# hpcaitech/CachedEmbedding

Hardware: AMD Instinct MI355X
Metric: embedding lookups/sec (cache op + EmbeddingBag fwd + bwd/SGD), Criteo-1TB table @1% cache (higher is better)
Workload: dtype f32

## Files before the change

### cachedembedding_amd/_lib.py

```python
from __future__ import annotations

import ctypes
import os
from ctypes import POINTER, Structure, c_char_p, c_double, c_float, c_int, c_int32, c_int64, c_size_t, c_uint64, c_void_p
from pathlib import Path

import torch

_PKG = Path(__file__).resolve().parent
LIB_PATH = Path(os.environ["CE_LIBRARY"]) if os.environ.get("CE_LIBRARY") else _PKG / "libce_hip.so"

CE_OK = 0
CE_ERR_INVALID = 1
CE_ERR_HIP = 2
CE_ERR_CAPACITY = 3
CE_ERR_NOMEM = 4
CE_ERR_UNSUPPORTED = 5
CE_ERR_RANGE = 6
CE_EVICT_DATASET = 0
CE_EVICT_LFU = 1
CE_MODE_SUM = 0
CE_MODE_MEAN = 1
CE_ACT_F32 = 0
CE_ACT_BF16 = 1
CE_ACT_F16 = 2
CE_TRANSPORT_ZEROCOPY = 0
CE_TRANSPORT_STAGED = 1
CE_TRANSPORT_WORKER = 2
CE_CALL_PREPARE = 0
CE_CALL_PRELOAD = 1
CE_CALL_FLUSH = 2


class CeCacheConfig(Structure):
    _fields_ = [
        ("num_embeddings", c_int64),
        ("cuda_row_num", c_int64),
        ("embedding_dim", c_int32),
        ("evict_strategy", c_int32),
        ("transport", c_int32),
        ("protect_depth", c_int32),
        ("max_ids_per_call", c_int64),
        ("host_weight", c_void_p),
        ("host_weight_dev", c_void_p),
        ("cache_weight", c_void_p),
        ("idx_map", c_void_p),
        ("inverted_cached_idx", c_void_p),
        ("cached_idx_map", c_void_p),
        ("freq_cnter", c_void_p),
        ("workspace", c_void_p),
        ("workspace_bytes", c_size_t),
    ]


class CeCallStats(Structure):
    _fields_ = [
        ("seq", c_int64),
        ("n_ids", c_int64),
        ("n_unique", c_int64),
        ("n_miss", c_int64),
        ("n_evict", c_int64),
        ("miss_lookups", c_int64),
        ("n_free_after", c_int64),
        ("status", c_int32),
        ("kind", c_int32),
    ]


_BAG_COMMON = [c_void_p, c_int32, c_int64, c_int32, c_void_p, c_int32, c_int64]
SIGNATURES = {
    "ce_version": (c_int, []),
    "ce_cpu_budget": (c_int32, []),
    "ce_last_error": (c_char_p, []),
    "ce_stream_create_cu_mask": (c_int, [c_void_p, c_int32, POINTER(c_void_p)]),
    "ce_stream_destroy": (c_int, [c_void_p]),
    "ce_host_alloc": (c_int, [c_size_t, c_int, POINTER(c_void_p), POINTER(c_void_p)]),
    "ce_host_free": (c_int, [c_void_p]),
    "ce_host_register": (c_int, [c_void_p, c_size_t, POINTER(c_void_p)]),
    "ce_host_unregister": (c_int, [c_void_p]),
    "ce_host_fill_uniform": (c_int, [c_void_p, c_int64, c_float, c_float, c_uint64, c_int]),
    "ce_host_fill_uniform_rows": (c_int, [c_void_p, c_int64, c_int32, c_float, c_float, c_uint64, c_void_p, c_void_p]),
    "ce_host_rows_gather": (c_int, [c_void_p, c_int64, c_int32, c_void_p, c_int64, c_void_p, c_void_p]),
    "ce_box_probe": (c_int, [c_void_p, c_size_t, c_int32, POINTER(c_double), POINTER(c_double), c_void_p]),
    "ce_probe_rows": (c_int, [c_void_p, c_int64, c_int32, c_int64, c_int32, POINTER(c_double), POINTER(c_double), c_void_p]),
    "ce_bag_forward": (c_int, [c_void_p, c_int64, c_int32, c_void_p, c_int64, c_void_p, c_int32, c_int64,
                               c_int32, c_void_p, c_int32, c_int64, c_void_p, c_void_p]),
    "ce_bag_backward_dense": (c_int, [c_void_p, c_int64, c_int32, c_void_p, c_int64, c_void_p, c_int32, c_int64,
                                      c_int32, c_void_p, c_int32, c_int64, c_void_p, c_void_p]),
    "ce_bag_backward_dense_presorted": (c_int, [c_void_p, c_int64, c_int32, c_void_p, c_int64, c_void_p, c_int32, c_int64,
                                      c_int32, c_void_p, c_int32, c_int64, c_void_p, c_void_p, c_void_p]),
    "ce_bag_backward_rows": (c_int, [c_void_p, c_void_p, c_int32, c_int64, c_void_p, c_int32, c_int64, c_int32, c_void_p,
                                     c_int32, c_int64, c_void_p, c_void_p]),
    "ce_bag_backward_sgd": (c_int, [c_void_p, c_int64, c_int32, c_void_p, c_int64, c_void_p, c_int32, c_int64,
                                    c_int32, c_void_p, c_int32, c_int64, c_void_p, c_float, c_void_p]),
    "ce_bag_presort_len": (c_int64, [c_int64]),
    "ce_bag_presort": (c_int, [c_void_p, c_int64, c_int64, c_void_p, c_void_p]),
    "ce_bag_backward_sgd_presorted": (c_int, [c_void_p, c_int64, c_int32, c_void_p, c_int64, c_void_p, c_int32,
                                              c_int64, c_int32, c_void_p, c_int32, c_int64, c_void_p, c_float,
                                              c_void_p, c_void_p]),
    "ce_bag_presort_window": (c_int, [c_void_p, c_int64, c_int64, c_int64, c_void_p, c_void_p]),
    "ce_bag_presort_window_src": (c_int, [c_void_p, c_int64, c_int64, c_int64, c_void_p, c_int32, c_int64, c_int64,
                                          c_int32, c_int64, c_void_p, c_void_p]),
    "ce_bag_forward_src_keys": (c_int, [c_void_p, c_int64, c_int32, c_int64, c_void_p, c_void_p, c_void_p]),
    "ce_bag_backward_sgd_presorted_src": (c_int, [c_void_p, c_int64, c_int32, c_int64, c_void_p, c_float, c_void_p,
                                                  c_void_p]),
    "ce_bag_presort_window_src_excl": (c_int, [c_void_p, c_int64, c_int64, c_int64, c_void_p, c_int32, c_int64,
                                               c_int64, c_int32, c_int64, c_void_p, c_void_p, c_void_p, c_void_p]),
    "ce_bag_backward_sgd_presorted_src_excl": (c_int, [c_void_p, c_int64, c_int32, c_int64, c_void_p, c_float,
                                                       c_void_p, c_void_p, c_void_p]),
    "ce_bag_backward_dense_presorted_src": (c_int, [c_void_p, c_int64, c_int32, c_int64, c_void_p, c_void_p,
                                                    c_void_p]),
    "ce_bag_backward_sgd_sorted_workspace": (c_size_t, [c_int64, c_int64]),
    "ce_bag_backward_sgd_sorted": (c_int, [c_void_p, c_int64, c_int32, c_void_p, c_int64, c_void_p, c_int32,
                                           c_int64, c_int32, c_void_p, c_int32, c_int64, c_void_p, c_float,
                                           c_void_p, c_size_t, c_void_p]),
    "ce_bag_backward_rowwise_adagrad_workspace": (c_size_t, [c_int64, c_int32]),
    "ce_bag_backward_rowwise_adagrad": (c_int, [c_void_p, c_int64, c_int32, c_void_p, c_int64, c_void_p, c_int32,
                                                c_int64, c_int32, c_void_p, c_int32, c_int64, c_void_p, c_void_p,
                                                c_void_p, c_void_p, c_int64, c_float, c_float, c_void_p, c_size_t,
                                                c_void_p]),
    "ce_bag_backward_rowwise_adagrad_src": (c_int, [c_void_p, c_int64, c_int32, c_int64, c_void_p, c_void_p, c_void_p,
                                                    c_void_p, c_int64, c_float, c_float, c_void_p, c_size_t,
                                                    c_void_p]),
    "ce_bag_forward_act": (c_int, [c_void_p, c_int64, c_int32, c_void_p, c_int64, c_void_p, c_int32, c_int64,
                                   c_int32, c_void_p, c_int32, c_int64, c_void_p, c_int32, c_void_p]),
    "ce_bag_forward_src_keys_act": (c_int, [c_void_p, c_int64, c_int32, c_int64, c_void_p, c_void_p, c_int32,
                                            c_void_p]),
    "ce_bag_backward_dense_act": (c_int, [c_void_p, c_int64, c_int32, c_void_p, c_int64, c_void_p, c_int32, c_int64,
                                          c_int32, c_void_p, c_int32, c_int64, c_void_p, c_int32, c_void_p,
                                          c_void_p]),
    "ce_bag_backward_sgd_act": (c_int, [c_void_p, c_int64, c_int32, c_void_p, c_int64, c_void_p, c_int32, c_int64,
                                        c_int32, c_void_p, c_int32, c_int64, c_void_p, c_int32, c_float, c_void_p,
                                        c_void_p]),
    "ce_bag_backward_sgd_src_act": (c_int, [c_void_p, c_int64, c_int32, c_int64, c_void_p, c_int32, c_float, c_void_p,
                                            c_void_p, c_void_p]),
    "ce_bag_backward_dense_src_act": (c_int, [c_void_p, c_int64, c_int32, c_int64, c_void_p, c_int32, c_void_p,
                                              c_void_p]),
    "ce_bag_backward_rowwise_adagrad_act": (c_int, [c_void_p, c_int64, c_int32, c_void_p, c_int64, c_void_p, c_int32,
                                                    c_int64, c_int32, c_void_p, c_int32, c_int64, c_void_p, c_int32,
                                                    c_void_p, c_void_p, c_void_p, c_int64, c_float, c_float,
                                                    c_void_p, c_size_t, c_void_p]),
    "ce_bag_backward_rowwise_adagrad_src_act": (c_int, [c_void_p, c_int64, c_int32, c_int64, c_void_p, c_int32,
                                                        c_void_p, c_void_p, c_void_p, c_int64, c_float, c_float,
                                                        c_void_p, c_size_t, c_void_p]),
    "ce_cache_workspace_bytes": (c_size_t, [c_int64, c_int64, c_int64, c_int32]),
    "ce_cache_create": (c_int, [POINTER(CeCacheConfig), c_void_p, POINTER(c_void_p)]),
    "ce_cache_destroy": (c_int, [c_void_p]),
    "ce_cache_preload": (c_int, [c_void_p, c_void_p, c_void_p, c_int64, c_void_p]),
    "ce_cache_set_freq_bound": (c_int, [c_void_p, c_int64]),
    "ce_cache_prepare_ids": (c_int, [c_void_p, c_void_p, c_int64, c_void_p, c_void_p]),
    "ce_cache_prepare_ids_keys": (c_int, [c_void_p, c_void_p, c_int64, c_int64, c_void_p, c_int32, c_void_p, c_int32,
                                          c_int64, c_int64, c_int32, c_int64, c_void_p, c_void_p]),
    "ce_cache_prepare_ids_begin": (c_int, [c_void_p, c_void_p, c_int64, c_int64, c_void_p, c_int32, c_void_p, c_int32,
                                           c_int64, c_int64, c_int32, c_int64, c_void_p, c_void_p]),
    "ce_cache_prepare_ids_finish": (c_int, [c_void_p, c_void_p]),
    "ce_cache_prepare_ids_padded": (c_int, [c_void_p, c_void_p, c_int64, c_void_p, c_void_p]),
    "ce_cache_prepare_ids_begin_padded": (c_int, [c_void_p, c_void_p, c_int64, c_void_p, c_void_p]),
    "ce_cache_set_deferred_rows": (c_int, [c_void_p, c_int32]),
    "ce_cache_rows_ticket": (c_int64, [c_void_p]),
    "ce_cache_wait_rows": (c_int, [c_void_p, c_int64, c_void_p]),
    "ce_cache_last_stats": (c_int, [c_void_p, POINTER(CeCallStats)]),
    "ce_cache_totals": (c_int, [c_void_p, POINTER(c_int64), POINTER(c_int64), POINTER(c_int64),
                                POINTER(c_int64), POINTER(c_int64)]),
    "ce_cache_history": (c_int64, [c_void_p, c_int64, POINTER(CeCallStats), c_int64]),
    "ce_cache_lookup_slots": (c_int, [c_void_p, c_void_p, c_int64, c_void_p, c_void_p]),
    "ce_cache_flush": (c_int, [c_void_p, c_void_p]),
    "ce_cache_set_protect_depth": (c_int, [c_void_p, c_int32]),
    "ce_cache_set_transport": (c_int, [c_void_p, c_int32]),
    "ce_cache_get_transport": (c_int32, [c_void_p]),
    "ce_cache_set_cache_weight": (c_int, [c_void_p, c_void_p]),
    "ce_cache_graph_replayed": (c_int, [c_void_p, c_int64, c_int64, c_void_p]),
    "ce_cache_set_buffer_rows": (c_int, [c_void_p, c_int64]),
    "ce_cache_set_profiling": (c_int, [c_void_p, c_int32]),
    "ce_cache_phase_count": (c_int32, []),
    "ce_cache_phase_name": (c_char_p, [c_int32]),
    "ce_cache_phase_times": (c_int, [c_void_p, POINTER(c_double), c_int32, POINTER(c_int64), c_int32]),
    "ce_cache_writeback_wait": (c_int, [c_void_p]),
    "ce_cache_swap_stats": (c_int, [c_void_p, POINTER(c_double), POINTER(c_int64)]),
    "ce_cache_failures": (c_int, [c_void_p, POINTER(c_int64), POINTER(c_int32), POINTER(c_int64)]),
    "ce_cache_free_rows": (c_int, [c_void_p, POINTER(c_int64)]),
    "ce_bucketize_workspace": (c_size_t, [c_int64, c_int32]),
    "ce_bucketize_rows": (c_int, [c_void_p, c_int64, c_void_p, c_int32, c_void_p, c_void_p, c_void_p, c_void_p,
                                  c_size_t, c_void_p]),
    "ce_dedupe_bucket_rows": (c_int, [c_void_p, c_int64, c_void_p, c_int64, c_int32, c_void_p, c_void_p,
                                      c_void_p, c_void_p, c_void_p, c_void_p, c_void_p]),
    "ce_dedupe_bucket_rows_padded": (c_int, [c_void_p, c_int64, c_void_p, c_int64, c_int32, c_int64, c_void_p, c_void_p,
                                             c_void_p, c_void_p, c_void_p, c_void_p, c_void_p, c_void_p]),
    "ce_dedupe_bucket_rows_padded_window": (c_int, [c_void_p, c_int64, c_int64, c_void_p, c_int64, c_int32, c_int64,
                                                    c_void_p, c_void_p, c_void_p, c_void_p, c_void_p, c_void_p,
                                                    c_void_p, c_void_p]),
    "ce_exchange_local_index": (c_int, [c_void_p, c_int64, c_int64, c_void_p, c_int64, c_int64, c_int64, c_int64,
                                        c_void_p, c_void_p]),
    "ce_split_classify": (c_int, [c_void_p, c_int32, c_int32, c_int64, c_int64, c_void_p, c_int64, c_void_p, c_void_p,
                                  c_void_p]),
    "ce_split_places": (c_int, [c_void_p, c_void_p, c_int32, c_int32, c_int64, c_int32, c_void_p, c_void_p, c_void_p,
                                c_void_p, c_void_p, c_void_p]),
    "ce_exchange_local_index_split": (c_int, [c_void_p, c_int64, c_int64, c_void_p, c_void_p, c_void_p, c_int64, c_int64,
                                              c_int64, c_int64, c_int64, c_void_p, c_int32, c_int64, c_int64, c_int64,
                                              c_void_p, c_void_p, c_void_p]),
    "ce_bag_forward_max": (c_int, [c_void_p, c_int64, c_int32, c_void_p, c_int64, c_void_p, c_int32, c_int64, c_int32,
                                   c_int64, c_void_p, c_void_p, c_void_p]),
    "ce_bag_backward_max": (c_int, [c_void_p, c_int64, c_int32, c_void_p, c_int64, c_int64, c_int64, c_void_p, c_void_p,
                                    c_float, c_void_p]),
    "ce_bag_backward_psw": (c_int, [c_void_p, c_int64, c_int32, c_void_p, c_int64, c_void_p, c_int32, c_int64, c_int32,
                                    c_int64, c_void_p, c_void_p, c_void_p]),
    "ce_rows_renorm_workspace": (c_size_t, [c_int64]),
    "ce_rows_renorm": (c_int, [c_void_p, c_int64, c_int32, c_void_p, c_int64, c_float, c_float, c_void_p, c_size_t,
                               c_void_p]),
    "ce_rows_axpy": (c_int, [c_void_p, c_int64, c_int32, c_void_p, c_int64, c_void_p, c_float, c_void_p]),
}


class CeError(RuntimeError):
    def __init__(self, code: int, msg: str):
        super().__init__(f"libce_hip error {code}: {msg}")
        self.code = code


def _load() -> ctypes.CDLL:
    if not LIB_PATH.exists():
        raise ImportError(
            f"{LIB_PATH} is missing: the HIP extension has not been built. Run "
            "`python -c 'import __graft_entry__ as g; g.build()'` (needs hipcc). There is no CPU fallback.")
    lib = ctypes.CDLL(str(LIB_PATH), mode=os.RTLD_NOW | os.RTLD_LOCAL)
    for name, (res, args) in SIGNATURES.items():
        fn = getattr(lib, name)
        fn.restype = res
        fn.argtypes = args
    return lib


lib = _load()


def last_error() -> str:
    m = lib.ce_last_error()
    return m.decode("utf-8", "replace") if m else ""


def check(rc: int) -> None:
    if rc != CE_OK:
        raise CeError(rc, last_error())


def require_gpu() -> None:
    if not torch.cuda.is_available():
        raise RuntimeError("cachedembedding_amd needs a HIP device (MI355X); no GPU is visible and there is "
                           "no CPU fallback for the product path")


_RAW_STREAM = getattr(torch._C, "_cuda_getCurrentRawStream", None)


def stream_ptr() -> int:
    if _RAW_STREAM is not None:
        return _RAW_STREAM(torch.cuda.current_device())
    return torch.cuda.current_stream().cuda_stream


ACT_DTYPES = {torch.float32: CE_ACT_F32, torch.bfloat16: CE_ACT_BF16, torch.float16: CE_ACT_F16}


def act_code(dtype) -> int:
    if dtype is None:
        return CE_ACT_F32
    try:
        return ACT_DTYPES[dtype]
    except (KeyError, TypeError):
        raise NotImplementedError(f"output_dtype={dtype!r}: torch.float32, torch.bfloat16 and torch.float16 are "
                                  "implemented") from None


def ptr(t) -> int:
    return 0 if t is None else t.data_ptr()
```

### cachedembedding_amd/cache_mgr.py

```python
from __future__ import annotations

import ctypes
import math
import weakref
from enum import Enum
from typing import List, Optional

import numpy as np
import torch

from . import _lib
from ._lib import CeCacheConfig, CeCallStats, check, lib, ptr, stream_ptr


class EvictionStrategy(Enum):
    LFU = 1
    DATASET = 2


class _PinnedBlock:

    def __init__(self, host_ptr: int):
        self._fin = weakref.finalize(self, _PinnedBlock._free, host_ptr)

# ... 284 lines not shown
                self.wait_rows()
            self._strict_check()
        return out

    def graph_replayed(self, n_calls: int, ids_per_call: int) -> None:
        with torch.cuda.device(self.device):
            check(lib.ce_cache_graph_replayed(self._handle, int(n_calls), int(ids_per_call), stream_ptr()))

    def _id_to_cached_cuda_id(self, ids: torch.Tensor) -> torch.Tensor:
        flat = ids.reshape(-1).long().contiguous()
        slots = torch.empty_like(flat)
        check(lib.ce_cache_lookup_slots(self._handle, ptr(flat), flat.numel(), ptr(slots), stream_ptr()))
        return slots.view(ids.shape)

    @torch.no_grad()
    def flush(self):
        with torch.cuda.device(self.device):
            check(lib.ce_cache_flush(self._handle, stream_ptr()))
            st = CeCallStats()
            check(lib.ce_cache_last_stats(self._handle, ctypes.byref(st)))
        self._pull_history()
        assert self.cuda_available_row_num == self.cuda_row_num

    def sync_stats(self) -> CeCallStats:
        st = CeCallStats()
        rc = lib.ce_cache_last_stats(self._handle, ctypes.byref(st))
        self._pull_history()
        if rc not in (_lib.CE_OK, _lib.CE_ERR_CAPACITY, _lib.CE_ERR_RANGE):
            check(rc)
        return st

    def _pull_history(self):
        cap = 4096
        buf = (CeCallStats * cap)()
        while True:
            n = lib.ce_cache_history(self._handle, self._hist_seen + 1, buf, cap)
            for i in range(n):
                r = buf[i]
                self._hist_seen = max(self._hist_seen, r.seq)
                if r.kind != _lib.CE_CALL_PREPARE:
                    continue
                self.num_hits_history.append(int(r.n_unique - r.n_miss))
                self.num_miss_history.append(int(r.n_miss))
                self.num_write_back_history.append(int(r.n_evict) if r.status == _lib.CE_OK else 0)
            if n < cap:
                break

    def totals(self):
        a, b, c, d, e = (ctypes.c_int64() for _ in range(5))
        check(lib.ce_cache_totals(self._handle, ctypes.byref(a), ctypes.byref(b), ctypes.byref(c), ctypes.byref(d),
                                  ctypes.byref(e)))
        return dict(cpu_to_cuda_numel=a.value, cuda_to_cpu_numel=b.value, cache_miss=c.value,
                    total_cache=d.value, calls=e.value)

    def print_comm_stats(self):
        self.sync_stats()
        t = self.totals()
        esz = 4
        msg = (f"CUDA->CPU {t['cuda_to_cpu_numel'] * esz / 1e6:.2f} MB, CPU->CUDA "
               f"{t['cpu_to_cuda_numel'] * esz / 1e6:.2f} MB, cache miss {t['cache_miss']} / {t['total_cache']} "
               f"lookups ({100.0 * t['cache_miss'] / max(1, t['total_cache']):.2f} %)")
        wb = self.writeback_stats()
        if wb["jobs"]:
            row_b = self.embedding_dim * esz
            def rate(nbytes, busy_s):
                return f"{nbytes / busy_s / 1e9:.1f} GB/s" if busy_s > 0 else "a rate no worker thread timed"
            msg += (f"; swap workers: out {wb['jobs']} jobs {wb['rows'] * row_b / 1e6:.2f} MB at "
                    f"{rate(wb['rows'] * row_b, wb['out_busy_s'])}, in {wb['in_jobs']} jobs "
                    f"{wb['in_rows'] * row_b / 1e6:.2f} MB at {rate(wb['in_rows'] * row_b, wb['in_busy_s'])}")
        print(msg)
        return msg

    def set_protect_depth(self, depth: int):
        check(lib.ce_cache_set_protect_depth(self._handle, int(depth)))

    def set_async_copy(self, flag: bool):
        self._async_copy = bool(flag)
        self.set_transport("staged" if flag else "zerocopy")

    _TRANSPORTS = {"zerocopy": _lib.CE_TRANSPORT_ZEROCOPY, "staged": _lib.CE_TRANSPORT_STAGED,
                   "worker": _lib.CE_TRANSPORT_WORKER}

    def set_transport(self, name: str):
        with torch.cuda.device(self.device):
            rc = lib.ce_cache_set_transport(self._handle, self._TRANSPORTS[name])
            if rc == _lib.CE_ERR_UNSUPPORTED and name == "worker":
                import warnings
                warnings.warn(f"worker transport unavailable ({_lib.last_error()}); using zerocopy")
                name = "zerocopy"
                rc = lib.ce_cache_set_transport(self._handle, self._TRANSPORTS[name])
            check(rc)
        self._transport = self._TRANSPORTS[name]

    def reserve_tail(self, rows: int) -> torch.Tensor:
        rows = int(rows)
        C, D = self.cuda_row_num, self.embedding_dim
        full = getattr(self, "_cache_full", None)
        if full is None or full.shape[0] < C + rows:
            with torch.cuda.device(self.device):
                torch.cuda.synchronize(self.device)
                full = torch.empty(C + rows, D, device=self.device, dtype=torch.float32)
                full[:C].copy_(self.cuda_cached_weight.data)
                full[C:].zero_()
                check(lib.ce_cache_set_cache_weight(self._handle, full.data_ptr()))
            self.cuda_cached_weight.data = full[:C]
            self._cache_full = full
        return self._cache_full[C:C + rows]

    @property
    def cache_with_tail(self) -> torch.Tensor:
        return self._cache_full

    @property
    def transport_name(self) -> str:
        code = lib.ce_cache_get_transport(self._handle)
        return {v: k for k, v in self._TRANSPORTS.items()}.get(code, "zerocopy")

    def set_profiling(self, on: bool = True):
        check(lib.ce_cache_set_profiling(self._handle, int(bool(on))))

    def phase_times(self, reset: bool = False) -> dict:
        n = lib.ce_cache_phase_count()
        buf = (ctypes.c_double * n)()
        calls = ctypes.c_int64()
        check(lib.ce_cache_phase_times(self._handle, buf, n, ctypes.byref(calls), int(reset)))
        out = {lib.ce_cache_phase_name(i).decode(): buf[i] for i in range(n)}
        out["calls"] = calls.value
        return out

    def writeback_wait(self):
        check(lib.ce_cache_writeback_wait(self._handle))

    def set_deferred_rows(self, on: bool = True):
        check(lib.ce_cache_set_deferred_rows(self._handle, int(bool(on))))
        self._deferred_rows = bool(on)

    def rows_ticket(self) -> int:
        return int(lib.ce_cache_rows_ticket(self._handle))

    def wait_rows(self, ticket: int = 0):
        if torch.cuda.current_device() == self.device.index:
            check(lib.ce_cache_wait_rows(self._handle, int(ticket), stream_ptr()))
        else:
            with torch.cuda.device(self.device):
                check(lib.ce_cache_wait_rows(self._handle, int(ticket), stream_ptr()))

    def writeback_stats(self) -> dict:
        sec = (ctypes.c_double * 6)()
        cnt = (ctypes.c_int64 * 4)()
        check(lib.ce_cache_swap_stats(self._handle, sec, cnt))
        return dict(out_wait_s=sec[0], out_busy_s=sec[1], in_wait_s=sec[2], in_busy_s=sec[3], in_gather_s=sec[4],
                    rows=cnt[0], jobs=cnt[1], in_rows=cnt[2], in_jobs=cnt[3], in_jobs_before_writeback_landed=int(sec[5]))

    def raise_on_failed_calls(self):
        n, st, sq = ctypes.c_int64(), ctypes.c_int32(), ctypes.c_int64()
        check(lib.ce_cache_failures(self._handle, ctypes.byref(n), ctypes.byref(st), ctypes.byref(sq)))
        if n.value > self._failures_seen:
            self._failures_seen = n.value
            if st.value == _lib.CE_ERR_CAPACITY:
                raise AssertionError(
                    f"cache op #{sq.value} needed more unique rows than the {self.cuda_row_num} rows available on "
                    "CUDA (with an overlapped window: unique(window k U window k+1)). Please increase cuda_row_num "
                    "or decrease the training batch size.")
            if st.value == _lib.CE_ERR_RANGE:
                raise IndexError(f"cache op #{sq.value}: an id is outside [0, {self.num_embeddings}) -- every slot of "
                                 "that call is -1.  (Since API 4 an id of -1 is a bad id on prepare_ids / "
                                 "ce_cache_prepare_ids too; padded id lists go through prepare_ids(..., padded=True) / "
                                 "ce_cache_prepare_ids_padded.)")
            raise _lib.CeError(st.value, f"cache op #{sq.value} failed")

    def acknowledge_failures(self) -> int:
        n, st, sq = ctypes.c_int64(), ctypes.c_int32(), ctypes.c_int64()
        self.sync_stats()
        check(lib.ce_cache_failures(self._handle, ctypes.byref(n), ctypes.byref(st), ctypes.byref(sq)))
        self._failures_seen = n.value
        return n.value

    def cuda_weight_data(self, slot: int) -> torch.Tensor:
        return self.cuda_cached_weight.data[slot]

    def cpu_weight_data(self, row_idx: int) -> torch.Tensor:
        return self.weight[row_idx]
```

### cachedembedding_amd/csrc/ce_cache.hip

```cpp
#include <sched.h>
#include <stdlib.h>
#include <string.h>
#include <sys/prctl.h>

#include <algorithm>
#include <atomic>
#include <chrono>
#include <condition_variable>
#include <functional>
#include <mutex>
#include <thread>
#include <vector>

#include "ce_common.h"

#include "ce_cache_index.h"
#include "ce_cache_select.h"
#include "ce_cache_rows.h"
#include "ce_cache_fused.h"
#include "ce_cache_worker.h"


struct ce_cache {
  ce_cache_config_t cfg;
  ce::Layout L;
  char* ws;
  ce::Ctl* ctl;
  uint32_t* bitmap;
  int32_t *blk_unique, *blk_miss, *coarse, *miss_list, *slot_epoch, *victims, *blk_free, *free_list;
  int32_t* miss_list_b[2];
  int32_t* free_list_b[2];
  ce::ChainWords* chain;
  unsigned long long *lb_emit, *lb_remap;
  unsigned lb_tag;
  ce::FrontWords* front;
  int32_t *fine_cnt, *coarse_cnt;
  long long front_calls;
  bool front_cleanup_pending;
  unsigned long long* keys;
  uint32_t* hist;
  ce_call_stats_t* ring;
  ce_call_stats_t* ring_dev;
  hipEvent_t ev;
  float* stage;
  int32_t* stage_idx;
  long long seq;
  long long drained;
  std::vector<ce_call_stats_t> history;
  int64_t cpu_to_cuda_numel, cuda_to_cpu_numel, cache_miss, total_cache;
  int vec;
  int rowlen, g_log2, slot_bits, word_bits;
  int host_threads;
  float* stage_dev;
  float* stage_host;
  int32_t* list_host;
  ce::Ctl* ctl_host;
  int64_t stage_rows;
  int64_t list_rows;
  int64_t buffer_rows;
  ce::RowPool* pool;
  ce::SwapEngine* wb;
  unsigned long long* evt_keys[2];
  int32_t* evt_pos[2];
  uint32_t evt_mask;
  float* stage2;
  int32_t* stage_idx2;
  float* in_stage;
  long long hist_base;
  ce::PhaseProf* prof;
  uint64_t freq_bound;
  uint64_t graph_freq_limit;
  bool freq_bound_known;
  long long n_failed;
  int last_fail_status;
  long long last_fail_seq;
  bool free_zero;
  long long free_reset_seq;
  bool deferred_rows;
  struct Pending {
    bool active = false;
    int64_t n = 0;
    int64_t* slots_out = nullptr;
    hipStream_t s = nullptr;
    bool worker = false, capturing = false, has_tail = false;
    long long in_job = 0, seq_arg = 0;
    int cap_groups = 1, swap_threads = 256, pslot = 0, pmark = 0;
    bool chained = false;
    long long call = 0;
    int parity = 0;
    bool sel_pending = false;
    hipStream_t sel_s = nullptr;
    int64_t sel_n = 0;
    bool sel_steady = false;
    long long sel_out_job = 0;
    int sel_wbuf = 0, sel_n_vblocks = 0;
    const void* prof = nullptr;
    struct {
      int64_t n_batches, nnz_per_batch;
      int32_t src_keys;
      const void* offsets;
      int32_t offsets_are_i64;
      int64_t offsets_batch_stride, num_bags;
      int32_t include_last_offset;
      int64_t hook_features;
      uint64_t* keys_out;
    } tail;
  } pend;
};

using namespace ce;

static int ensure_writeback(ce_cache* h);

static void drain(ce_cache* h) {
  while (h->drained < h->seq) {
    const long long s = h->drained + 1;
    const ce_call_stats_t& r = h->ring[s % kRing];
    if (r.seq != s) break;
    if (h->history.empty()) h->hist_base = s;
    h->history.push_back(r);
    if (h->history.size() > (size_t)2 * kHistoryKeep) {
      h->history.erase(h->history.begin(), h->history.end() - kHistoryKeep);
      h->hist_base = h->history.front().seq;
    }
    if (r.status != CE_OK) {
      h->n_failed += 1;
      h->last_fail_status = r.status;
      h->last_fail_seq = s;
      h->free_zero = false;
      h->free_reset_seq = h->seq;
    } else if (r.kind == CE_CALL_PREPARE && s > h->free_reset_seq) {
      h->free_zero = r.n_free_after == 0;
    }
    if (r.status == CE_OK && r.kind != CE_CALL_PRELOAD) {
      h->cpu_to_cuda_numel += r.n_miss * h->cfg.embedding_dim;
      h->cuda_to_cpu_numel += r.n_evict * h->cfg.embedding_dim;
      h->cache_miss += r.miss_lookups;
      h->total_cache += r.n_ids;
      if (h->wb && h->wb->chained && r.kind == CE_CALL_PREPARE) {
        std::lock_guard<std::mutex> g(h->wb->m);
        h->wb->in_rows += r.n_miss;
      }
    }
    h->drained = s;
  }
}

static hipEvent_t last_rows_event(ce_cache* h) {
  if (!h->wb || !h->wb->chained || h->wb->chain_calls == 0) return nullptr;
  return h->wb->ev_rows[h->wb->chain_calls % SwapEngine::kRowsRing];
}
static int join_rows(ce_cache* h, hipStream_t s) {
  if (hipEvent_t ev = last_rows_event(h)) CE_HIP_CHECK(hipStreamWaitEvent(s, ev, 0));
  return CE_OK;
}

static int sync_and_drain(ce_cache* h) {
  CE_HIP_CHECK(hipEventSynchronize(h->ev));
  if (hipEvent_t ev = last_rows_event(h)) CE_HIP_CHECK(hipEventSynchronize(ev));
  drain(h);
  return CE_OK;
}

extern "C" size_t ce_cache_workspace_bytes(int64_t num_embeddings, int64_t cuda_row_num, int64_t max_ids_per_call,
                                           int32_t embedding_dim) {
  if (num_embeddings <= 0 || cuda_row_num <= 0 || embedding_dim <= 0) return 0;
  return make_layout(num_embeddings, cuda_row_num, max_ids_per_call, embedding_dim).total;
}

extern "C" int ce_cache_create(const ce_cache_config_t* cfg, ce_stream_t stream, ce_cache_t** out) {
  CE_REQUIRE(cfg && out, CE_ERR_INVALID, "null config");
  CE_REQUIRE(cfg->num_embeddings > 0 && cfg->num_embeddings < (int64_t)INT32_MAX, CE_ERR_UNSUPPORTED,
             "num_embeddings must be in (0, 2^31)");
  if (cfg->cuda_row_num == 0) {
    set_error("cuda_row_num == 0 is not implemented (NotImplementedError upstream, A.1)");
    return CE_ERR_UNSUPPORTED;
  }
  CE_REQUIRE(cfg->cuda_row_num > 0 && cfg->cuda_row_num <= cfg->num_embeddings, CE_ERR_INVALID,
             "cuda_row_num must be in (0, num_embeddings]");
  CE_REQUIRE(cfg->embedding_dim > 0, CE_ERR_INVALID, "embedding_dim must be positive");
  CE_REQUIRE(cfg->evict_strategy == CE_EVICT_DATASET || cfg->evict_strategy == CE_EVICT_LFU, CE_ERR_INVALID,
             "unknown eviction strategy");
  CE_REQUIRE(cfg->cache_weight && cfg->inverted_cached_idx && cfg->cached_idx_map && cfg->workspace,
             CE_ERR_INVALID, "null device array");
  CE_REQUIRE((((uintptr_t)cfg->inverted_cached_idx) & 15) == 0, CE_ERR_INVALID,
             "inverted_cached_idx must be 16-byte aligned");
  CE_REQUIRE(cfg->evict_strategy != CE_EVICT_LFU || cfg->freq_cnter, CE_ERR_INVALID, "LFU needs freq_cnter");
  CE_REQUIRE(cfg->host_weight && cfg->host_weight_dev, CE_ERR_INVALID, "null host table");
  Layout L = make_layout(cfg->num_embeddings, cfg->cuda_row_num, cfg->max_ids_per_call, cfg->embedding_dim);
  CE_REQUIRE(cfg->workspace_bytes >= L.total, CE_ERR_INVALID, "workspace too small: need %zu bytes", L.total);
  CE_REQUIRE((((uintptr_t)cfg->workspace) & 255) == 0, CE_ERR_INVALID, "workspace must be 256-byte aligned");

  ce_cache* h = new ce_cache();
  h->cfg = *cfg;
  h->L = L;
  h->ws = (char*)cfg->workspace;
  h->ctl = (Ctl*)(h->ws + L.ctl);
  h->bitmap = (uint32_t*)(h->ws + L.bitmap);
  h->blk_unique = (int32_t*)(h->ws + L.blk_unique);
  h->blk_miss = (int32_t*)(h->ws + L.blk_miss);
  h->coarse = (int32_t*)(h->ws + L.coarse);
  h->miss_list = (int32_t*)(h->ws + L.miss_list);
  h->slot_epoch = (int32_t*)(h->ws + L.slot_epoch);
  h->keys = (unsigned long long*)(h->ws + L.keys);
  h->hist = (uint32_t*)(h->ws + L.hist);
  h->victims = (int32_t*)(h->ws + L.victims);
  h->blk_free = (int32_t*)(h->ws + L.blk_free);
  h->free_list = (int32_t*)(h->ws + L.free_list);
  h->miss_list_b[0] = h->miss_list;
  h->miss_list_b[1] = (int32_t*)(h->ws + L.miss_list2);
  h->free_list_b[0] = h->free_list;
  h->free_list_b[1] = (int32_t*)(h->ws + L.free_list2);
  h->chain = (ChainWords*)(h->ws + L.chain);
  h->lb_emit = (unsigned long long*)(h->ws + L.lb_emit);
  h->lb_remap = (unsigned long long*)(h->ws + L.lb_remap);
  h->lb_tag = 0;
  h->front = (FrontWords*)(h->ws + L.front);
  h->fine_cnt = (int32_t*)(h->ws + L.fine_cnt);
  h->coarse_cnt = (int32_t*)(h->ws + L.coarse_cnt);
  h->front_calls = 0;
  h->front_cleanup_pending = false;
  h->seq = h->drained = 0;
  h->cpu_to_cuda_numel = h->cuda_to_cpu_numel = h->cache_miss = h->total_cache = 0;
  const int D = cfg->embedding_dim;
  auto al16 = [](const void* q) { return (((uintptr_t)q) & 15) == 0; };
  h->vec = (D % 4 == 0) && al16(cfg->cache_weight) && al16(cfg->host_weight_dev);
  h->rowlen = h->vec ? D / 4 : D;
  int g = 1, gl2 = 0;
  while (g < h->rowlen && g < 64) { g <<= 1; ++gl2; }
  h->g_log2 = gl2;
  int sb = 1;
  while ((1ll << sb) < cfg->cuda_row_num) ++sb;
  h->slot_bits = sb;
  int wb = 1;
  while ((1ll << wb) < cdiv(cfg->num_embeddings, 32)) ++wb;
  h->word_bits = wb;
  h->host_threads = (int)std::max(1u, std::min(64u, std::thread::hardware_concurrency()));
  h->stage_dev = nullptr;
  h->stage_host = nullptr;
  h->list_host = nullptr;
  h->ctl_host = nullptr;
  h->stage_rows = 0;
  h->list_rows = 0;
  h->buffer_rows = 0;
  h->pool = nullptr;
  h->wb = nullptr;
  h->hist_base = 1;
  h->prof = nullptr;
  h->freq_bound = 0;
  h->graph_freq_limit = ~0ull;
  h->freq_bound_known = true;
  h->n_failed = 0;
  h->last_fail_status = CE_OK;
  h->last_fail_seq = 0;
  h->free_zero = false;
  h->free_reset_seq = 0;
  h->deferred_rows = false;
  h->stage2 = (float*)(h->ws + L.stage2);
  h->stage_idx2 = (int32_t*)(h->ws + L.stage_idx2);
  h->in_stage = (float*)(h->ws + L.in_stage);

  hipStream_t s = (hipStream_t)stream;
  void* ring_host = nullptr;
  if (hipHostMalloc(&ring_host, sizeof(ce_call_stats_t) * kRing, hipHostMallocMapped) != hipSuccess) {
    delete h;
    set_error("hipHostMalloc(stats ring) failed");
    return CE_ERR_HIP;
  }
  memset(ring_host, 0, sizeof(ce_call_stats_t) * kRing);
  h->ring = (ce_call_stats_t*)ring_host;
  void* ring_dev = nullptr;
  if (hipHostGetDevicePointer(&ring_dev, ring_host, 0) != hipSuccess) ring_dev = ring_host;
  h->ring_dev = (ce_call_stats_t*)ring_dev;
  h->stage = (float*)(h->ws + L.stage);
  h->stage_idx = (int32_t*)(h->ws + L.stage_idx);
  if (hipEventCreateWithFlags(&h->ev, hipEventDisableTiming) != hipSuccess) {
    (void)hipHostFree(ring_host);
    delete h;
    set_error("hipEventCreate failed");
    return CE_ERR_HIP;
  }
  const int64_t N = cfg->num_embeddings, C = cfg->cuda_row_num;
  (void)hipMemsetAsync(h->ws, 0, L.stage_idx, s);
  hipLaunchKernelGGL(k_fill_i32, dim3(grid_for(N, 256)), dim3(256), 0, s, cfg->inverted_cached_idx, N, -1);
  hipLaunchKernelGGL(k_fill_i32, dim3(grid_for(C, 256)), dim3(256), 0, s, cfg->cached_idx_map, C, -1);
  hipLaunchKernelGGL(k_fill_i32, dim3(grid_for(C, 256)), dim3(256), 0, s, h->slot_epoch, C, kEpochNever);
  if (cfg->freq_cnter)
    hipLaunchKernelGGL(k_fill_i64, dim3(grid_for(C, 256)), dim3(256), 0, s, cfg->freq_cnter, C, (int64_t)INT64_MAX);
  Ctl init{};
  init.n_free = C;
  (void)hipMemcpyAsync(h->ctl, &init, sizeof(Ctl), hipMemcpyHostToDevice, s);
  hipError_t e = hipStreamSynchronize(s);
  if (e == hipSuccess) e = hipGetLastError();
  if (e != hipSuccess) {
    set_error("cache state initialisation failed: %s", hipGetErrorString(e));
    (void)hipEventDestroy(h->ev);
    (void)hipHostFree(ring_host);
    delete h;
    return CE_ERR_HIP;
  }
  (void)hipEventRecord(h->ev, s);
  if (cfg->transport == CE_TRANSPORT_WORKER) {
    int rc = ensure_writeback(h);
    if (rc) {
      (void)hipEventDestroy(h->ev);
      (void)hipHostFree(ring_host);
      delete h;
      return rc;
    }
  }
  *out = h;
  return CE_OK;
}

extern "C" int ce_cache_destroy(ce_cache_t* h) {
  if (!h) return CE_OK;
  (void)hipEventSynchronize(h->ev);
  if (h->wb && h->wb->in_stream) (void)hipStreamSynchronize(h->wb->in_stream);
  delete h->wb;
  for (int b = 0; b < 2; ++b) {
    if (h->evt_keys[b]) (void)hipFree(h->evt_keys[b]);
    if (h->evt_pos[b]) (void)hipFree(h->evt_pos[b]);
  }
  delete h->pool;
  delete h->prof;
  (void)hipEventDestroy(h->ev);
  (void)hipHostFree(h->ring);
  if (h->stage_dev) (void)hipFree(h->stage_dev);
  if (h->stage_host) (void)hipHostFree(h->stage_host);
  if (h->list_host) (void)hipHostFree(h->list_host);
  if (h->ctl_host) (void)hipHostFree(h->ctl_host);
  delete h;
  return CE_OK;
}

static int before_call(ce_cache* h) {
  if (h->seq - h->drained >= kRing - 2) return sync_and_drain(h);
  drain(h);
  return CE_OK;
}

static int ensure_staging(ce_cache* h, int64_t rows, int64_t list_rows) {
  if (rows > h->stage_rows) {
    if (h->stage_dev) (void)hipFree(h->stage_dev);
    if (h->stage_host) (void)hipHostFree(h->stage_host);
    h->stage_dev = nullptr; h->stage_host = nullptr;
    h->stage_rows = 0;
    const size_t bytes = (size_t)rows * h->cfg.embedding_dim * sizeof(float);
    CE_HIP_CHECK(hipMalloc((void**)&h->stage_dev, bytes));
    CE_HIP_CHECK(hipHostMalloc((void**)&h->stage_host, bytes, hipHostMallocDefault));
    h->stage_rows = rows;
  }
  if (list_rows > h->list_rows) {
    if (h->list_host) (void)hipHostFree(h->list_host);
    h->list_host = nullptr;
    h->list_rows = 0;
    CE_HIP_CHECK(hipHostMalloc((void**)&h->list_host, (size_t)list_rows * sizeof(int32_t), hipHostMallocDefault));
    h->list_rows = list_rows;
  }
  return CE_OK;
}

static int cpu_budget() {
  long n = (long)std::max(1u, std::thread::hardware_concurrency());
  cpu_set_t set;
  if (sched_getaffinity(0, sizeof set, &set) == 0) n = std::min<long>(n, std::max(1, CPU_COUNT(&set)));
  if (FILE* f = fopen("/sys/fs/cgroup/cpu.max", "r")) {
    char q[32] = {0};
    long long per = 0;
    if (fscanf(f, "%31s %lld", q, &per) == 2 && strcmp(q, "max") != 0 && per > 0)
      n = std::min<long>(n, std::max<long long>(1, atoll(q) / per));
    fclose(f);
  } else {
    long long quota = -1, per = 0;
    if (FILE* g = fopen("/sys/fs/cgroup/cpu/cpu.cfs_quota_us", "r")) { if (fscanf(g, "%lld", &quota) != 1) quota = -1; fclose(g); }
    if (FILE* g = fopen("/sys/fs/cgroup/cpu/cpu.cfs_period_us", "r")) { if (fscanf(g, "%lld", &per) != 1) per = 0; fclose(g); }
    if (quota > 0 && per > 0) n = std::min<long>(n, std::max<long long>(1, quota / per));
  }
  return (int)std::max<long>(1, n);
}

extern "C" int32_t ce_cpu_budget(void) { return cpu_budget(); }

static RowPool* host_pool(ce_cache* h) {
  if (!h->pool) h->pool = new RowPool(std::max(1, std::min(h->host_threads, 32)));
  return h->pool;
}

static int ensure_writeback(ce_cache* h) {
  if (h->wb) return CE_OK;
  const Layout& L = h->L;
  SwapEngine* w = new SwapEngine();
  int rc = CE_OK;
  do {
    int can = 0;
    if (hipGetDevice(&w->device) != hipSuccess) { rc = CE_ERR_HIP; break; }
    (void)hipDeviceGetAttribute(&can, hipDeviceAttributeCanUseStreamWaitValue, w->device);
    if (!can) {
      delete w;
      set_error("the worker transport needs hipStreamWaitValue64, which this device does not support");
      return CE_ERR_UNSUPPORTED;
    }
    w->D = h->cfg.embedding_dim;
    w->stage_rows = L.stage_rows;
    w->table = h->cfg.host_weight;
    w->stage_dev[0] = h->stage;
    w->stage_dev[1] = h->stage2;
    w->idx_dev[0] = h->stage_idx;
    w->idx_dev[1] = h->stage_idx2;
    w->in_stage_dev = h->in_stage;
    {
      const char* e = getenv("CE_WORKER_ADMIT");
      w->chained = !(e && !strcmp(e, "sdma")) && h->cfg.host_weight_dev != nullptr;
    }
    {
      if (w->chained && !h->evt_keys[0]) {
        uint32_t places = 4096;
        while ((int64_t)places < 4 * L.stage_rows && places < (1u << 30)) places <<= 1;
        bool ok = (int64_t)places >= 4 * L.stage_rows;
        for (int b = 0; b < 2 && ok; ++b) {
          ok = hipMalloc((void**)&h->evt_keys[b], (size_t)places * 8) == hipSuccess &&
               hipMalloc((void**)&h->evt_pos[b], (size_t)places * 4) == hipSuccess &&
               hipMemset(h->evt_keys[b], 0, (size_t)places * 8) == hipSuccess;
        }
        if (ok) {
          h->evt_mask = places - 1;
        } else {
          (void)hipGetLastError();
          for (int b = 0; b < 2; ++b) {
            if (h->evt_keys[b]) (void)hipFree(h->evt_keys[b]);
            if (h->evt_pos[b]) (void)hipFree(h->evt_pos[b]);
            h->evt_keys[b] = nullptr;
            h->evt_pos[b] = nullptr;
          }
          rc = CE_ERR_NOMEM;
          break;
        }
      }
#ifdef CE_TEST_HOOKS
      if (const char* e = getenv("CE_WORKER_OUT_DELAY_US")) w->out_delay_us = std::max(0, atoi(e));
      if (const char* e = getenv("CE_WORKER_FAIL_IN_JOB")) w->fail_in_job = atoll(e);
#endif
      for (int b = 0; b < 2; ++b) {
        w->evt_keys[b] = h->evt_keys[b];
        w->evt_pos[b] = h->evt_pos[b];
      }
      w->evt_mask = h->evt_mask;
    }
    const size_t rows_bytes = (size_t)L.stage_rows * w->D * 4, idx_bytes = (size_t)L.stage_rows * 4;
    int prio_lo = 0, prio_hi = 0;
    (void)hipDeviceGetStreamPriorityRange(&prio_lo, &prio_hi);
    if (prio_lo == prio_hi) {
      delete w;
      set_error("the worker transport needs stream priorities (a hardware-queue pool of its own for the copy streams)");
      return CE_ERR_UNSUPPORTED;
    }
    if (hipStreamCreateWithPriority(&w->out_stream, hipStreamNonBlocking, prio_hi) != hipSuccess ||
        hipStreamCreateWithPriority(&w->out_stream2, hipStreamNonBlocking, prio_hi) != hipSuccess ||
        hipStreamCreateWithPriority(&w->in_stream, hipStreamNonBlocking, prio_hi) != hipSuccess) {
      rc = CE_ERR_HIP;
      break;
    }
    void* p = nullptr;
    void* pd = nullptr;
    if (hipHostMalloc(&p, sizeof(WbMail) * 3, hipHostMallocMapped) != hipSuccess) { rc = CE_ERR_NOMEM; break; }
    memset(p, 0, sizeof(WbMail) * 3);
    w->mail = (WbMail*)p;
    if (hipHostGetDevicePointer(&pd, p, 0) != hipSuccess) pd = p;
    w->mail_dev = (WbMail*)pd;
    if (hipHostMalloc(&p, 64, hipHostMallocMapped) != hipSuccess) { rc = CE_ERR_NOMEM; break; }
    memset(p, 0, 64);
    w->sig = (unsigned long long*)p;
    if (hipHostGetDevicePointer(&pd, p, 0) != hipSuccess) pd = p;
    w->sig_dev = (unsigned long long*)pd;
    if (hipHostMalloc(&p, idx_bytes, hipHostMallocMapped) != hipSuccess) { rc = CE_ERR_NOMEM; break; }
    w->miss_host = (int32_t*)p;
    if (hipHostGetDevicePointer(&pd, p, 0) != hipSuccess) pd = p;
    w->miss_host_dev = (int32_t*)pd;
    if (!w->chained &&
        hipHostMalloc((void**)&w->in_host, rows_bytes, hipHostMallocDefault) != hipSuccess) { rc = CE_ERR_NOMEM; break; }
    if (w->chained) {
      for (auto& ev : w->ev_miss)
        if (rc == CE_OK && hipEventCreateWithFlags(&ev, hipEventDisableTiming) != hipSuccess) rc = CE_ERR_HIP;
      for (auto& ev : w->ev_rows)
        if (rc == CE_OK && hipEventCreateWithFlags(&ev, hipEventDisableTiming) != hipSuccess) rc = CE_ERR_HIP;
      if (rc) break;
    }
    const unsigned evf = hipEventDisableTiming | hipEventBlockingSync;
    if (hipEventCreateWithFlags(&w->in_ev[0], evf) != hipSuccess ||
        hipEventCreateWithFlags(&w->in_ev[1], evf) != hipSuccess) { rc = CE_ERR_HIP; break; }
    for (int b = 0; b < 2 && rc == CE_OK; ++b) {
      if (hipEventCreateWithFlags(&w->out_ev[b], evf) != hipSuccess) rc = CE_ERR_HIP;
      else if (hipHostMalloc((void**)&w->rows_host[b], rows_bytes, hipHostMallocDefault) != hipSuccess) rc = CE_ERR_NOMEM;
      else if (hipHostMalloc((void**)&w->idx_host[b], idx_bytes, hipHostMallocDefault) != hipSuccess) rc = CE_ERR_NOMEM;
    }
    for (auto& ev : w->chunk_ev)
      if (rc == CE_OK && hipEventCreateWithFlags(&ev, hipEventDisableTiming) != hipSuccess) rc = CE_ERR_HIP;
    if (rc) break;
    static const int dflt = std::max(2, std::min(8, (cpu_budget() - 4) / 2));
    static const int out_threads = [] { const char* e = getenv("CE_WB_THREADS"); return e ? atoi(e) : dflt; }();
    static const int in_threads = [] { const char* e = getenv("CE_GATHER_THREADS"); return e ? atoi(e) : dflt; }();
    w->out_pool = new RowPool(std::max(1, std::min(out_threads, 64)));
    w->in_pool = new RowPool(std::max(1, std::min(in_threads, 64)));
    w->rowlen = h->rowlen;
    w->g_log2 = h->g_log2;
    w->vec = h->vec;
    w->out_thread = std::thread([w] { w->run_out(); });
    if (!w->chained) w->in_thread = std::thread([w] { w->run_in(); });
  } while (0);
  if (rc) {
    delete w;
    set_error("swap worker setup failed (pinned buffers / streams / events)");
    return rc;
  }
  w->deferred_rows = h->deferred_rows;
  h->wb = w;
  return CE_OK;
}

static int64_t staged_chunk(const ce_cache* h, int64_t rows) {
  return (h->buffer_rows > 0 && h->buffer_rows < rows) ? h->buffer_rows : rows;
}

extern "C" int ce_cache_set_freq_bound(ce_cache_t* h, int64_t bound) {
  CE_REQUIRE(h && bound >= 0, CE_ERR_INVALID, "bad bound");
  h->freq_bound = std::max<uint64_t>(h->freq_bound, (uint64_t)bound);
  h->freq_bound_known = true;
  return CE_OK;
}

extern "C" int ce_cache_preload(ce_cache_t* h, const int32_t* rows, const int64_t* freq_vals, int64_t n,
                                ce_stream_t stream) {
  CE_REQUIRE(h, CE_ERR_INVALID, "null handle");
  CE_REQUIRE(n >= 0 && n <= h->cfg.cuda_row_num, CE_ERR_INVALID, "preload count out of range");
  CE_REQUIRE(!h->pend.active, CE_ERR_INVALID, "a cache op begun with ce_cache_prepare_ids_begin has not been finished");
  if (n == 0) return CE_OK;
  if (freq_vals) h->freq_bound_known = false;
  int rc = before_call(h);
  if (rc) return rc;
  if (h->wb) {
    rc = h->wb->wait_out(h->wb->out_issued);
    if (rc) return rc;
  }
  hipStream_t s = (hipStream_t)stream;
  const ce_cache_config_t& c = h->cfg;
  rc = join_rows(h, s);
  if (rc) return rc;
  h->seq += 1;
  const int32_t epoch = (int32_t)(h->seq & 0x3fffffff);
  const int64_t groups_per_block = 256 >> h->g_log2;
  if (h->vec)
    hipLaunchKernelGGL((k_admit<f32x4>), dim3(grid_for(n, (int)groups_per_block * kSwapRows)), dim3(256), 0, s, rows,
                       (const int32_t*)nullptr, (const long long*)nullptr, (long long)n,
                       (const f32x4*)c.host_weight_dev, (f32x4*)c.cache_weight, h->rowlen, h->g_log2,
                       (const Ctl*)nullptr, 0ll);
  else
    hipLaunchKernelGGL((k_admit<float>), dim3(grid_for(n, (int)groups_per_block * kSwapRows)), dim3(256), 0, s, rows,
                       (const int32_t*)nullptr, (const long long*)nullptr, (long long)n,
                       (const float*)c.host_weight_dev, (float*)c.cache_weight, h->rowlen, h->g_log2,
                       (const Ctl*)nullptr, 0ll);
  hipLaunchKernelGGL(k_admit_maps, dim3(grid_for(n, 256)), dim3(256), 0, s, rows, (const int32_t*)nullptr,
                     (const long long*)nullptr, (long long)n, c.cached_idx_map, c.inverted_cached_idx,
                     c.freq_cnter, freq_vals, h->slot_epoch, kEpochNever, (Ctl*)nullptr,
                     (ce_call_stats_t*)nullptr, 0ll, (const unsigned long long*)nullptr, 0ll);
  (void)epoch;
  hipLaunchKernelGGL(k_preload_end, dim3(1), dim3(1), 0, s, (long long)n, h->ctl, h->ring_dev + (h->seq % kRing),
                     h->seq);
  CE_LAUNCH_CHECK();
  CE_HIP_CHECK(hipEventRecord(h->ev, s));
  return CE_OK;
}

static int staged_swap(ce_cache* h, hipStream_t s) {
  const ce_cache_config_t& c = h->cfg;
  const int D = c.embedding_dim;
  const size_t rowbytes = (size_t)D * sizeof(float);
  if (!h->ctl_host) CE_HIP_CHECK(hipHostMalloc((void**)&h->ctl_host, sizeof(Ctl), hipHostMallocDefault));
  CE_HIP_CHECK(hipMemcpyAsync(h->ctl_host, h->ctl, sizeof(Ctl), hipMemcpyDeviceToHost, s));
  CE_HIP_CHECK(hipStreamSynchronize(s));
  const Ctl ctl = *h->ctl_host;
  if (ctl.status != CE_OK) return CE_OK;
  const int64_t k = ctl.k_evict, m = ctl.n_miss;
  const int64_t big = std::max<int64_t>(std::max(k, m), 1);
  int rc = ensure_staging(h, staged_chunk(h, big), big);
  if (rc) return rc;
  const int gpb = 256 >> h->g_log2;
  if (k > 0) {
    int32_t* evicted_rows_dev = h->free_list;
    hipLaunchKernelGGL(k_evict_maps, dim3(grid_for(k, 256)), dim3(256), 0, s, h->victims, c.cached_idx_map,
                       c.inverted_cached_idx, evicted_rows_dev, h->ctl);
    CE_HIP_CHECK(hipMemcpyAsync(h->list_host, evicted_rows_dev, (size_t)k * 4, hipMemcpyDeviceToHost, s));
    const int64_t chunk = staged_chunk(h, k);
    for (int64_t off = 0; off < k; off += chunk) {
      const int64_t cnt = std::min(chunk, k - off);
      if (h->vec)
        hipLaunchKernelGGL((k_pack_rows<f32x4>), dim3(grid_for(cnt, gpb)), dim3(256), 0, s,
                           (const int32_t*)h->victims + off, (long long)cnt, (const f32x4*)c.cache_weight,
                           (f32x4*)h->stage_dev, h->rowlen, h->g_log2);
      else
        hipLaunchKernelGGL((k_pack_rows<float>), dim3(grid_for(cnt, gpb)), dim3(256), 0, s,
                           (const int32_t*)h->victims + off, (long long)cnt, (const float*)c.cache_weight,
                           (float*)h->stage_dev, h->rowlen, h->g_log2);
      CE_HIP_CHECK(hipMemcpyAsync(h->stage_host, h->stage_dev, (size_t)cnt * rowbytes, hipMemcpyDeviceToHost, s));
      CE_HIP_CHECK(hipStreamSynchronize(s));
      float* table = c.host_weight;
      const float* st = h->stage_host;
      const int32_t* rows = h->list_host + off;
      host_pool(h)->parallel(cnt, [=](int64_t lo, int64_t hi) {
        for (int64_t i = lo; i < hi; ++i) memcpy(table + (size_t)rows[i] * D, st + (size_t)i * D, rowbytes);
      });
    }
  }
  return CE_OK;
}

static int worker_selftest(ce_cache* h, hipStream_t s) {
  SwapEngine* w = h->wb;
  if (w->tested && w->tested_stream == s) return CE_OK;
  CE_HIP_CHECK(hipStreamSynchronize(s));
  unsigned long long* word = w->sig + 2;
  __atomic_store_n(word, 0ull, __ATOMIC_RELEASE);
  CE_HIP_CHECK(hipStreamWaitValue64(s, word, 1, hipStreamWaitValueGte, ~0ull));
  std::this_thread::sleep_for(std::chrono::milliseconds(2));
  hipError_t e = hipMemcpyAsync(w->rows_host[0], w->stage_dev[0], 64, hipMemcpyDeviceToHost, w->out_stream);
  if (e == hipSuccess) e = hipMemcpyAsync(w->rows_host[1], w->stage_dev[1], 64, hipMemcpyDeviceToHost, w->out_stream2);
  if (e == hipSuccess) e = hipMemcpyAsync(w->in_stage_dev, w->rows_host[0], 64, hipMemcpyHostToDevice, w->in_stream);
  bool done = e == hipSuccess;
  if (done) {
    for (hipStream_t st : {w->out_stream, w->out_stream2, w->in_stream})
      if (stream_wait_polite(st, 0.25) != hipSuccess) done = false;
  }
  __atomic_store_n(word, 1ull, __ATOMIC_RELEASE);
  CE_HIP_CHECK(hipStreamSynchronize(s));
  if (e != hipSuccess) {
    set_error("worker transport self-test: %s", hipGetErrorString(e));
    return CE_ERR_HIP;
  }
  if (!done) {
    set_error("worker transport self-test failed: copies on the library's copy streams do not run while the cache-op "
              "stream is parked in hipStreamWaitValue64 (they share a hardware queue with it: GPU_MAX_HW_QUEUES = %s)",
              getenv("GPU_MAX_HW_QUEUES") ? getenv("GPU_MAX_HW_QUEUES") : "unset");
    return CE_ERR_UNSUPPORTED;
  }
  w->tested = true;
  w->tested_stream = s;
  return CE_OK;
}

struct FrontTail {
  const int32_t* miss_tmp;
  const FrontWords* fw;
  uint32_t* bitmap;
  int32_t *fine, *coarse;
};
static FrontTail take_front_tail(ce_cache* h) {
  if (!h->front_cleanup_pending) return FrontTail{nullptr, nullptr, nullptr, nullptr, nullptr};
  h->front_cleanup_pending = false;
  return FrontTail{h->victims, h->front + (h->front_calls & 1), h->bitmap, h->fine_cnt, h->coarse_cnt};
}

struct SelArgs {
  hipStream_t s;
  int64_t n;
  bool worker, capturing, steady;
  long long out_job, seq_arg;
  int wbuf, n_vblocks, pslot;
  const void* prof_id;
  int32_t* free_list;
};

static int select_top_pass(ce_cache* h, int64_t n, bool capturing) {
  const ce_cache_config_t& c = h->cfg;
  const int64_t N = c.num_embeddings;
  int top_pass = kLevels - 1;
  if (c.evict_strategy != CE_EVICT_LFU) {
    top_pass = 0;
    while (top_pass < kLevels - 1 && ((uint64_t)(N - 1) >> (kDigitBits * (top_pass + 1))) != 0) ++top_pass;
  } else {
    uint64_t bound = h->freq_bound + (uint64_t)n;
    if (capturing) {
      bound = h->freq_bound + kGraphFreqHeadroom;
      h->graph_freq_limit = bound;
    } else {
      h->freq_bound = bound;
    }
    const int bits = 64 - __builtin_clzll(bound | 1ull) + h->slot_bits;
    top_pass = h->freq_bound_known ? std::min(kLevels - 1, std::max(0, (bits + kDigitBits - 1) / kDigitBits - 1))
                                   : kLevels - 1;
  }
  return top_pass;
}

static int select_and_stage(ce_cache* h, const SelArgs& a, int* pmark_io) {
  const ce_cache_config_t& c = h->cfg;
  const Layout& L = h->L;
  const int64_t N = c.num_embeddings, C = c.cuda_row_num, n = a.n;
  hipStream_t s = a.s;
  const bool worker = a.worker, capturing = a.capturing, steady = a.steady;
  const long long out_job = a.out_job, seq_arg = a.seq_arg;
  const int wbuf = a.wbuf, n_vblocks = a.n_vblocks, pslot = a.pslot;
  const int lfu = c.evict_strategy == CE_EVICT_LFU;
  const int gpb = 256 >> h->g_log2;
  ce_call_stats_t* const ring = h->ring_dev;
  PhaseProf* const prof = (h->prof && (const void*)h->prof == a.prof_id) ? h->prof : nullptr;
  int pmark = *pmark_io;
  int rc = CE_OK;
#define CE_PHASE() do { if (prof) (void)hipEventRecord(prof->ev[pslot][pmark++], s); } while (0)
  const int cgrid = grid_for(C, 256 * 4);
  const int top_pass = select_top_pass(h, n, capturing);
  const FrontTail ft = take_front_tail(h);
  hipLaunchKernelGGL(k_keys, dim3(std::min(cgrid, 512)), dim3(256), 0, s, c.cached_idx_map, c.freq_cnter, h->slot_epoch, C, N,
                     seq_arg, c.protect_depth, h->slot_bits, lfu, top_pass, h->keys, h->hist, h->ctl, ft.miss_tmp, ft.fw,
                     ft.bitmap, ft.fine, ft.coarse, (int)L.n_chunks);
  const int hgrid = (int)std::min<int64_t>(kNumCU, std::max<int64_t>(1, cdiv(C, 1024 * 4)));
  for (int pass = top_pass - 1; pass >= 0; --pass)
    hipLaunchKernelGGL(k_hist, dim3(hgrid), dim3(1024), 0, s, h->keys, C, pass, top_pass, h->hist, h->ctl);
  hipLaunchKernelGGL(k_victims, dim3((unsigned)n_vblocks), dim3(256), 0, s, h->keys, C, h->victims, L.list_cap, h->ctl,
                     (const uint32_t*)h->hist, top_pass, ring, seq_arg, steady ? h->blk_free : (int32_t*)nullptr);
  CE_PHASE();
  float* const stage_cur = (worker && wbuf) ? h->stage2 : h->stage;
  int32_t* const stage_idx_cur = (worker && wbuf) ? h->stage_idx2 : h->stage_idx;
  if (c.transport == CE_TRANSPORT_ZEROCOPY || worker) {
    const long long scap = (long long)L.stage_rows;
    const int sgrid = (int)std::min<int64_t>(512, std::max<int64_t>(1, cdiv(L.stage_rows, gpb)));
    WbMail* const mail = worker ? h->wb->mail_dev + wbuf : nullptr;
    const dim3 sg(sgrid + (steady ? n_vblocks : 0));
    const EvTable evt = (worker && h->wb->chained) ? EvTable{h->evt_keys[wbuf], h->evt_pos[wbuf], h->evt_mask}
                                                     : EvTable{nullptr, nullptr, 0u};
    if (h->vec) {
      hipLaunchKernelGGL((k_evict_stage<f32x4>), sg, dim3(256), 0, s, h->victims, c.cached_idx_map,
                         c.inverted_cached_idx, (const f32x4*)c.cache_weight, (f32x4*)stage_cur, stage_idx_cur, scap, h->rowlen, h->g_log2,
                         h->ctl, mail, out_job, sgrid, (const unsigned long long*)h->keys, C, (const int32_t*)h->blk_free,
                         a.free_list, evt, L.list_cap > L.stage_rows ? (f32x4*)c.host_weight_dev : (f32x4*)nullptr);
    } else {
      hipLaunchKernelGGL((k_evict_stage<float>), sg, dim3(256), 0, s, h->victims, c.cached_idx_map,
                         c.inverted_cached_idx, (const float*)c.cache_weight, (float*)stage_cur, stage_idx_cur, scap, h->rowlen, h->g_log2,
                         h->ctl, mail, out_job, sgrid, (const unsigned long long*)h->keys, C, (const int32_t*)h->blk_free,
                         a.free_list, evt, L.list_cap > L.stage_rows ? (float*)c.host_weight_dev : (float*)nullptr);
    }
    if (worker) {
      CE_HIP_CHECK(hipEventRecord(h->wb->out_ev[wbuf], s));
      h->wb->push_out();
    }
  } else {
    rc = staged_swap(h, s);
    if (rc) return rc;
  }
  CE_PHASE();
  if (steady) {
  } else if (C <= 16384) {
    hipLaunchKernelGGL(k_free_single, dim3(1), dim3(1024), 0, s, c.cached_idx_map, C, a.free_list, h->ctl);
  } else {
    hipLaunchKernelGGL(k_free_count, dim3((unsigned)L.n_slot_blocks), dim3(256), 0, s, c.cached_idx_map, C,
                       h->blk_free, h->ctl);
    hipLaunchKernelGGL(k_free_emit, dim3((unsigned)L.n_slot_blocks), dim3(256), 0, s, c.cached_idx_map, C,
                       h->blk_free, a.free_list, h->ctl);
  }
  CE_PHASE();
#undef CE_PHASE
  *pmark_io = pmark;
  (void)rc;
  return CE_OK;
}

struct KeysTail {
  int64_t n_batches, nnz_per_batch;
  int32_t src_keys;
  const void* offsets;
  int32_t offsets_are_i64;
  int64_t offsets_batch_stride, num_bags;
  int32_t include_last_offset;
  int64_t hook_features;
  uint64_t* keys_out;
};

struct MarkCfg {
  bool merge;
  int u, threads, blocks, hot_words;
};
static MarkCfg mark_cfg(const ce_cache* h, int64_t n) {
  const bool ranked = h->cfg.idx_map != nullptr;
  MarkCfg m;
  m.merge = !ranked;
  m.threads = ranked ? 512 : 256;
  m.hot_words = (int)std::min<int64_t>(h->L.bitmap_words, ranked ? 8192 : 2048);
  m.u = n >= 65536 ? 4 : 1;
  m.blocks = std::min(grid_for(n, m.threads * m.u), 256);
  return m;
}

constexpr int64_t kScanMaxIds = (1 << 23) - 1;

static void launch_front_kernels(ce_cache* h, const int64_t* ids, int64_t n, int64_t* slots_out, hipStream_t s,
                                 int allow_pad, bool steady, long long seq_arg, int32_t* miss_list, WbMail* mail_in,
                                 long long in_job, int32_t* miss_host, long long* n_admit_out, bool single_pass_ok) {
  const ce_cache_config_t& c = h->cfg;
  const Layout& L = h->L;
  const int64_t N = c.num_embeddings, C = c.cuda_row_num;
  if (h->front_cleanup_pending) {
    hipLaunchKernelGGL(k_front_cleanup, dim3(64), dim3(256), 0, s, (const int32_t*)h->victims,
                       (const FrontWords*)(h->front + (h->front_calls & 1)), h->bitmap, h->fine_cnt, h->coarse_cnt,
                       (int)L.n_chunks);
    h->front_cleanup_pending = false;
  }
  if (single_pass_ok && !mail_in && !miss_host && n < (int64_t)INT32_MAX && L.n_chunks <= kRankMaxChunks) {
    const long long fc = ++h->front_calls;
    FrontWords* const fw = h->front + (fc & 1);
    FrontWords* const fw_next = h->front + ((fc + 1) & 1);
    if (n > 0) {
      const int U = n >= 65536 ? 2 : 1;
      const int threads = (int)std::min<int64_t>(1024, std::max<int64_t>(64, cdiv(cdiv(n, U), 64) * 64));
      const dim3 tg((unsigned)cdiv(n, (int64_t)threads * U)), tb(threads);
#define CE_TOUCH(U_)                                                                                                \
  hipLaunchKernelGGL((k_touch<U_>), tg, tb, 0, s, ids, n, c.idx_map, c.inverted_cached_idx, N, h->bitmap, h->fine_cnt, \
                     h->coarse_cnt, h->slot_epoch, seq_arg, fw, h->victims, (unsigned)L.list_cap, slots_out, allow_pad)
      if (U == 2) CE_TOUCH(2); else CE_TOUCH(1);
#undef CE_TOUCH
    }
    const int rgrid = (int)std::min<int64_t>(kNumCU, std::max<int64_t>(1, cdiv(std::max(n, C), 4096)));
    hipLaunchKernelGGL(k_miss_rank, dim3(rgrid), dim3(256), (size_t)L.n_chunks * 4, s, (const int32_t*)h->victims, fw, fw_next,
                       (const uint32_t*)h->bitmap, (const int32_t*)h->fine_cnt, (const int32_t*)h->coarse_cnt,
                       (int)L.n_chunks, (unsigned)L.list_cap, miss_list, (const int32_t*)h->slot_epoch, C, h->hist, seq_arg, h->ctl, n, h->ring_dev,
                       (long long)L.stage_rows, steady ? 1 : 0, n_admit_out);
    h->front_cleanup_pending = true;
    return;
  }
  hipLaunchKernelGGL(k_begin, dim3(16), dim3(256), 0, s, h->ctl, h->coarse,
                     (int)(((L.n_chunks >> kCoarseShift) + 1) * 2 * kCoarsePad), h->hist, seq_arg);
  if (n > 0) {
    const MarkCfg mc = mark_cfg(h, n);
    const dim3 mg(mc.blocks), mb(mc.threads);
#define CE_MARK(M, U_)                                                                                             \
  hipLaunchKernelGGL((k_mark<M, U_>), mg, mb, mc.hot_words * 4, s, ids, n, c.idx_map, c.inverted_cached_idx, N,    \
                     h->word_bits, mc.hot_words, h->bitmap, h->ctl, slots_out, allow_pad)
    if (mc.merge) { if (mc.u == 4) CE_MARK(true, 4); else CE_MARK(true, 1); }
    else { if (mc.u == 4) CE_MARK(false, 4); else CE_MARK(false, 1); }
#undef CE_MARK
  }
  hipLaunchKernelGGL(k_count, dim3((unsigned)L.n_chunks), dim3(256), 0, s, (const uint4*)h->bitmap,
                     c.inverted_cached_idx, N, h->blk_unique, h->blk_miss, h->coarse);
  hipLaunchKernelGGL(k_emit, dim3((unsigned)cdiv(L.n_chunks, kEmitSub)), dim3(256), 0, s, (uint4*)h->bitmap, c.inverted_cached_idx, N,
                     h->blk_miss, h->coarse, (int)L.n_chunks, miss_list, h->slot_epoch, seq_arg, h->ctl, C, n, h->ring_dev,
                     mail_in, in_job, (long long)L.stage_rows, miss_host, steady ? 1 : 0, n_admit_out);
}

static int prepare_ids_second_half(ce_cache* h);
static int chained_second_half(ce_cache* h);
static int launch_slots_keys(ce_cache* h);

static int chained_first_half(ce_cache* h, const int64_t* ids, int64_t n, int64_t* slots_out, hipStream_t s,
                              int allow_pad, const KeysTail* tail, int split) {
  SwapEngine* const w = h->wb;
  const Layout& L = h->L;
  const long long out_job = w->out_issued + 1;
  const int wbuf = (int)(out_job & 1);
  int rc = w->wait_out(out_job - 2);
  if (rc) return rc;
  const long long call = ++w->chain_calls;
  const int parity = (int)(call & 1);
  const bool steady = h->free_zero;
  const long long seq_arg = (long long)h->seq;
  PhaseProf* const prof = h->prof;
  const int pslot = (int)(h->seq % kProfDepth);
  int pmark = 0;
  if (prof) {
    prof->collect(pslot);
    prof->chained[pslot] = true;
    (void)hipEventRecord(prof->ev[pslot][pmark++], s);
  }
  launch_front_kernels(h, ids, n, slots_out, s, allow_pad, steady, seq_arg, h->miss_list_b[parity], (WbMail*)nullptr, 0ll,
                       (int32_t*)nullptr, &h->chain->n_admit[parity], true);
  CE_HIP_CHECK(hipEventRecord(w->ev_miss[parity], s));
  CE_HIP_CHECK(hipStreamWaitEvent(w->in_stream, w->ev_miss[parity], 0));
  if (prof) (void)hipEventRecord(prof->adm0[pslot], w->in_stream);
  {
    const int blocks = n <= 600000 ? 32 : 20;
    const long long prev = out_job - 1;
    const int pb = (int)(prev & 1);
    bool landed;
    {
      std::lock_guard<std::mutex> g(w->m);
      landed = w->out_done >= prev;
      w->in_jobs += 1;
      if (!landed) w->in_probed += 1;
    }
    const bool has_prev = prev >= w->probe_floor && !landed;
    const unsigned long long* ek = has_prev ? h->evt_keys[pb] : nullptr;
    const long long* n_ptr = &h->chain->n_admit[parity];
    if (h->vec)
      hipLaunchKernelGGL((k_admit_probe<f32x4>), dim3(blocks), dim3(1024), 0, w->in_stream, h->miss_list_b[parity], n_ptr,
                         (const f32x4*)h->cfg.host_weight_dev, (f32x4*)h->in_stage, h->rowlen, h->g_log2, ek,
                         (const int32_t*)h->evt_pos[pb], h->evt_mask, (uint32_t)prev,
                         (const f32x4*)(pb ? h->stage2 : h->stage));
    else
      hipLaunchKernelGGL((k_admit_probe<float>), dim3(blocks), dim3(1024), 0, w->in_stream, h->miss_list_b[parity], n_ptr,
                         (const float*)h->cfg.host_weight_dev, (float*)h->in_stage, h->rowlen, h->g_log2, ek,
                         (const int32_t*)h->evt_pos[pb], h->evt_mask, (uint32_t)prev,
                         (const float*)(pb ? h->stage2 : h->stage));
  }
  if (prof) (void)hipEventRecord(prof->ev[pslot][pmark++], s);
  ce_cache::Pending& x = h->pend;
  x.n = n; x.slots_out = slots_out; x.s = s; x.worker = true; x.capturing = false; x.has_tail = tail != nullptr;
  x.in_job = 0; x.seq_arg = seq_arg; x.pslot = pslot; x.pmark = pmark; x.prof = prof;
  x.chained = true; x.call = call; x.parity = parity;
  x.sel_pending = true;
  x.sel_s = s; x.sel_n = n; x.sel_steady = steady; x.sel_out_job = out_job; x.sel_wbuf = wbuf;
  x.sel_n_vblocks = (int)cdiv(h->cfg.cuda_row_num, 4096);
  if (tail)
    x.tail = {tail->n_batches, tail->nnz_per_batch, tail->src_keys, tail->offsets, tail->offsets_are_i64,
              tail->offsets_batch_stride, tail->num_bags, tail->include_last_offset, tail->hook_features, tail->keys_out};
  (void)L;
  if (split) {
    x.active = true;
    CE_LAUNCH_CHECK();
    return CE_OK;
  }
  return chained_second_half(h);
}

static int chained_second_half(ce_cache* h) {
  ce_cache::Pending& x = h->pend;
  x.active = false;
  x.sel_pending = false;
  SwapEngine* const w = h->wb;
  const ce_cache_config_t& c = h->cfg;
  const Layout& L = h->L;
  hipStream_t s = x.s;
  const int parity = x.parity, wbuf = x.sel_wbuf, pslot = x.pslot;
  const long long call = x.call, out_job = x.sel_out_job;
  PhaseProf* const prof = (h->prof && (const void*)h->prof == x.prof) ? h->prof : nullptr;
  if (prof) {
    (void)hipEventRecord(prof->resume[pslot], s);
    prof->resumed[pslot] = true;
  }
  if (call > 1) CE_HIP_CHECK(hipStreamWaitEvent(s, w->ev_rows[(call - 1) % SwapEngine::kRowsRing], 0));
  hipEvent_t sel_done = w->out_ev[wbuf];
  if (x.sel_steady && x.sel_n <= kScanMaxIds) {
    const int64_t N = c.num_embeddings, C = c.cuda_row_num;
    const int lfu = c.evict_strategy == CE_EVICT_LFU;
    const int top_pass = select_top_pass(h, x.sel_n, false);
    const FrontTail ft = take_front_tail(h);
    hipLaunchKernelGGL(k_keys, dim3(std::min(grid_for(C, 256 * 4), 512)), dim3(256), 0, s, c.cached_idx_map, c.freq_cnter,
                       h->slot_epoch, C, N, x.seq_arg, c.protect_depth, h->slot_bits, lfu, top_pass, h->keys, h->hist, h->ctl,
                       ft.miss_tmp, ft.fw, ft.bitmap, ft.fine, ft.coarse, (int)L.n_chunks);
    const int hgrid = (int)std::min<int64_t>(kNumCU, std::max<int64_t>(1, cdiv(C, 1024 * 4)));
    for (int pass = top_pass - 1; pass >= 0; --pass)
      hipLaunchKernelGGL(k_hist, dim3(hgrid), dim3(1024), 0, s, h->keys, C, pass, top_pass, h->hist, h->ctl);
    if (prof) (void)hipEventRecord(prof->ev[pslot][x.pmark++], s);
    StageArgs a;
    a.cached_idx_map = c.cached_idx_map;
    a.inverted = c.inverted_cached_idx;
    a.freq = c.freq_cnter;
    a.slot_epoch = h->slot_epoch;
    a.C = C;
    a.seq_arg = x.seq_arg;
    a.top_pass = top_pass;
    a.keys = h->keys;
    a.hist = h->hist;
    a.ctl = h->ctl;
    a.lb = h->lb_remap;
    h->lb_tag = (h->lb_tag + 1) & 0xffffu;
    a.tag = h->lb_tag;
    a.free_list = h->free_list_b[parity];
    a.miss_list = h->miss_list_b[parity];
    a.ring = h->ring_dev;
    a.n_unpack_out = &h->chain->n_unpack[parity];
    a.cache = c.cache_weight;
    a.stage = wbuf ? h->stage2 : h->stage;
    a.stage_rows_idx = wbuf ? h->stage_idx2 : h->stage_idx;
    a.scap = (long long)L.stage_rows;
    a.rowlen = h->rowlen;
    a.g_log2 = h->g_log2;
    a.vec = h->vec;
    a.mail = w->mail_dev + wbuf;
    a.job = out_job;
    a.evt = EvTable{h->evt_keys[wbuf], h->evt_pos[wbuf], h->evt_mask};
    a.host_overflow = L.list_cap > L.stage_rows ? (void*)c.host_weight_dev : nullptr;
    hipLaunchKernelGGL(k_rank_victims, dim3((unsigned)cdiv(C, kRemapSlots)), dim3(256), 0, s, a);
    {
      const int gpb = 256 >> h->g_log2;
      const int sgrid = (int)std::min<int64_t>(x.sel_n <= 600000 ? 256 : 512,
                                               std::max<int64_t>(1, cdiv(L.stage_rows, gpb * kStageRowsInFlight)));
      hipLaunchKernelGGL(k_stage_maps, dim3(sgrid), dim3(256), 0, s, a);
    }
    CE_HIP_CHECK(hipEventRecord(w->out_ev[wbuf], s));
    w->push_out();
    if (prof)
      for (int j = 0; j < 2; ++j) (void)hipEventRecord(prof->ev[pslot][x.pmark++], s);
  } else {
    SelArgs sel{s, x.sel_n, true, false, x.sel_steady, out_job, x.seq_arg, wbuf, x.sel_n_vblocks, pslot, x.prof,
                h->free_list_b[parity]};
    int rc0 = select_and_stage(h, sel, &x.pmark);
    if (rc0) return rc0;
    hipLaunchKernelGGL(k_admit_maps, dim3(grid_for(L.list_cap, 256)), dim3(256), 0, s, h->miss_list_b[parity],
                       h->free_list_b[parity], (const long long*)&h->ctl->n_miss, 0ll, c.cached_idx_map,
                       c.inverted_cached_idx, c.freq_cnter, (const int64_t*)nullptr, h->slot_epoch, 0, h->ctl,
                       h->ring_dev, x.seq_arg, (const unsigned long long*)nullptr, 0ll, &h->chain->n_unpack[parity]);
    CE_HIP_CHECK(hipEventRecord(w->ev_miss[parity], s));
    sel_done = w->ev_miss[parity];
  }
  CE_HIP_CHECK(hipStreamWaitEvent(w->in_stream, sel_done, 0));
  {
    const int gpb = 256 >> h->g_log2;
    const int ugrid = (int)std::min<int64_t>(x.sel_n <= 600000 ? 128 : 512, std::max<int64_t>(1, cdiv(L.stage_rows, gpb)));
    const long long prev = out_job - 1;
    const int pb = (int)(prev & 1);
    const unsigned long long* ek = prev >= w->probe_floor ? h->evt_keys[pb] : nullptr;
    const bool tail_possible = L.list_cap > L.stage_rows;
    if (h->vec)
      hipLaunchKernelGGL((k_unpack_chained<f32x4>), dim3(ugrid), dim3(256), 0, w->in_stream, h->free_list_b[parity],
                         (const long long*)&h->chain->n_unpack[parity], (long long)L.stage_rows,
                         (const f32x4*)h->in_stage, (f32x4*)c.cache_weight, h->rowlen, h->g_log2,
                         (const int32_t*)h->miss_list_b[parity],
                         tail_possible ? (const f32x4*)c.host_weight_dev : (const f32x4*)nullptr, ek,
                         (const int32_t*)h->evt_pos[pb], h->evt_mask, (uint32_t)prev,
                         (const f32x4*)(pb ? h->stage2 : h->stage));
    else
      hipLaunchKernelGGL((k_unpack_chained<float>), dim3(ugrid), dim3(256), 0, w->in_stream, h->free_list_b[parity],
                         (const long long*)&h->chain->n_unpack[parity], (long long)L.stage_rows,
                         (const float*)h->in_stage, (float*)c.cache_weight, h->rowlen, h->g_log2,
                         (const int32_t*)h->miss_list_b[parity],
                         tail_possible ? (const float*)c.host_weight_dev : (const float*)nullptr, ek,
                         (const int32_t*)h->evt_pos[pb], h->evt_mask, (uint32_t)prev,
                         (const float*)(pb ? h->stage2 : h->stage));
  }
  if (prof) (void)hipEventRecord(prof->adm1[pslot], w->in_stream);
  hipEvent_t rows = w->ev_rows[call % SwapEngine::kRowsRing];
  CE_HIP_CHECK(hipEventRecord(rows, w->in_stream));
  if (prof) (void)hipEventRecord(prof->ev[pslot][x.pmark++], s);
  int rc = launch_slots_keys(h);
  if (rc) return rc;
  if (prof) prof->pending[pslot] = true;
  CE_LAUNCH_CHECK();
  if (!w->deferred_rows) CE_HIP_CHECK(hipStreamWaitEvent(s, rows, 0));
  CE_HIP_CHECK(hipEventRecord(h->ev, s));
  return CE_OK;
}

static int prepare_ids_impl(ce_cache_t* h, const int64_t* ids, int64_t n, int64_t* slots_out, ce_stream_t stream,
                            int allow_pad, const KeysTail* tail = nullptr, int split = 0) {
  CE_REQUIRE(h, CE_ERR_INVALID, "null handle");
  CE_REQUIRE(!h->pend.active, CE_ERR_INVALID, "a cache op begun with ce_cache_prepare_ids_begin has not been finished");
  CE_REQUIRE(n >= 0 && n <= std::max<int64_t>(h->cfg.max_ids_per_call, 0), CE_ERR_INVALID,
             "n=%lld exceeds max_ids_per_call=%lld", (long long)n, (long long)h->cfg.max_ids_per_call);
  CE_REQUIRE(n == 0 || (ids && slots_out), CE_ERR_INVALID, "null ids/slots");
  hipStream_t s = (hipStream_t)stream;
  hipStreamCaptureStatus cap_st = hipStreamCaptureStatusNone;
  if (s != nullptr) CE_HIP_CHECK(hipStreamIsCapturing(s, &cap_st));
  const bool capturing = cap_st == hipStreamCaptureStatusActive;
  if (capturing) {
    CE_REQUIRE(h->cfg.transport == CE_TRANSPORT_ZEROCOPY, CE_ERR_UNSUPPORTED,
               "only the zero-copy transport can be captured in a hipGraph (the others hand rows to host threads)");
    CE_REQUIRE(!h->prof, CE_ERR_UNSUPPORTED, "switch the phase timers off before capturing a cache op");
    CE_REQUIRE(!split, CE_ERR_UNSUPPORTED, "a cache op in two halves cannot be captured in a hipGraph");
  }
  int rc = capturing ? CE_OK : before_call(h);
  if (rc) return rc;
  const ce_cache_config_t& c = h->cfg;
  const Layout& L = h->L;
  const int64_t N = c.num_embeddings, C = c.cuda_row_num;
  bool worker = c.transport == CE_TRANSPORT_WORKER;
  if (worker) {
    rc = ensure_writeback(h);
    if (rc) return rc;
    if (h->wb->chained) {
      rc = h->wb->check();
      if (rc) return rc;
      h->seq += 1;
      return chained_first_half(h, ids, n, slots_out, s, allow_pad, tail, split);
    }
  }
  if (!capturing) h->seq += 1;
  const long long seq_arg = capturing ? 0ll : (long long)h->seq;
  ce_call_stats_t* const ring = h->ring_dev;
  const int swap_blocks = c.protect_depth > 0 ? 32 : 512;
  const int swap_threads = 256;
  const int cap_groups = (int)std::min<int64_t>(swap_blocks, std::max<int64_t>(1, cdiv(L.list_cap, (swap_threads >> h->g_log2) * kSwapRows)));

  long long out_job = 0, in_job = 0;
  int wbuf = 0;
  if (worker) {
    rc = worker_selftest(h, s);
    if (rc == CE_ERR_UNSUPPORTED) {
      fprintf(stderr, "[libce_hip] %s -- falling back to the zero-copy transport\n", ce_last_error());
      rc = h->wb->wait_out(h->wb->out_issued);
      if (rc) return rc;
      h->cfg.transport = CE_TRANSPORT_ZEROCOPY;
      worker = false;
    } else if (rc) {
      return rc;
    }
  }
  if (worker) {
    {
      int prio = 0, prio_lo = 0, prio_hi = 0;
      (void)hipDeviceGetStreamPriorityRange(&prio_lo, &prio_hi);
      if (s != nullptr && prio_hi != prio_lo && hipStreamGetPriority(s, &prio) == hipSuccess)
        CE_REQUIRE(prio != prio_hi, CE_ERR_UNSUPPORTED,
                   "the worker transport's host-gather admission cannot run its cache op on a highest-priority stream "
                   "(its copy streams use that priority to stay out of the parked stream's hardware queue)");
    }
    out_job = h->wb->out_issued + 1;
    in_job = h->wb->in_issued + 1;
    wbuf = (int)(out_job & 1);
    rc = h->wb->wait_out(out_job - 2);
    if (rc == CE_OK) rc = h->wb->wait_in(in_job - 2);
    if (rc) return rc;
  }
  const bool steady = h->free_zero && !capturing && (c.transport == CE_TRANSPORT_ZEROCOPY || worker);
  const int n_vblocks = (int)cdiv(C, 4096);
  PhaseProf* const prof = h->prof;
  const int pslot = (int)(h->seq % kProfDepth);
  int pmark = 0;
  if (prof) prof->collect(pslot);
#define CE_PHASE() do { if (prof) (void)hipEventRecord(prof->ev[pslot][pmark++], s); } while (0)
  CE_PHASE();
  launch_front_kernels(h, ids, n, slots_out, s, allow_pad, steady, seq_arg, h->miss_list,
                       worker ? h->wb->mail_dev + 2 : (WbMail*)nullptr, in_job,
                       worker ? h->wb->miss_host_dev : (int32_t*)nullptr, (long long*)nullptr, !capturing);
  if (worker) {
    CE_HIP_CHECK(hipEventRecord(h->wb->in_ev[in_job & 1], s));
    h->wb->push_in(out_job - 1);
  }
  CE_PHASE();
  SelArgs sel{s, n, worker, capturing, steady, out_job, seq_arg, wbuf, n_vblocks, pslot, (const void*)prof, h->free_list};
  const bool defer_sel = split && worker;
  if (!defer_sel) {
    rc = select_and_stage(h, sel, &pmark);
    if (rc) return rc;
  }
#undef CE_PHASE
  ce_cache::Pending& x = h->pend;
  x.n = n; x.slots_out = slots_out; x.s = s; x.worker = worker; x.capturing = capturing; x.has_tail = tail != nullptr;
  x.in_job = in_job; x.seq_arg = seq_arg; x.cap_groups = cap_groups; x.swap_threads = swap_threads; x.pslot = pslot;
  x.pmark = pmark;
  x.prof = prof;
  x.chained = false;
  x.sel_pending = defer_sel;
  x.sel_s = s; x.sel_n = n; x.sel_steady = steady; x.sel_out_job = out_job; x.sel_wbuf = wbuf; x.sel_n_vblocks = n_vblocks;
  if (tail)
    x.tail = {tail->n_batches, tail->nnz_per_batch, tail->src_keys, tail->offsets, tail->offsets_are_i64,
              tail->offsets_batch_stride, tail->num_bags, tail->include_last_offset, tail->hook_features, tail->keys_out};
  if (split) {
    x.active = true;
    CE_LAUNCH_CHECK();
    return CE_OK;
  }
  return prepare_ids_second_half(h);
}

static int launch_slots_keys(ce_cache* h) {
  ce_cache::Pending& x = h->pend;
  const ce_cache_config_t& c = h->cfg;
  const int64_t C = c.cuda_row_num, n = x.n;
  int64_t* const slots_out = x.slots_out;
  hipStream_t s = x.s;
  const ce_stream_t stream = (ce_stream_t)s;
  const int lfu = c.evict_strategy == CE_EVICT_LFU;
  PhaseProf* const prof = (h->prof && (const void*)h->prof == x.prof) ? h->prof : nullptr;
  const decltype(x.tail)* const tail = x.has_tail ? &x.tail : nullptr;
  int rc = CE_OK;
  if (n > 0 && lfu) {
    hipLaunchKernelGGL(k_slots_lfu, dim3(std::min(grid_for(n, 8192), kMaxBlocks)), dim3(1024), 0, s, slots_out, n,
                       c.inverted_cached_idx, c.freq_cnter, (const Ctl*)h->ctl);
    if (tail) {
      rc = tail->src_keys
               ? ce_bag_presort_window_src(slots_out, tail->nnz_per_batch, tail->n_batches, C, tail->offsets,
                                           tail->offsets_are_i64, tail->offsets_batch_stride, tail->num_bags,
                                           tail->include_last_offset, tail->hook_features, tail->keys_out, stream)
               : ce_bag_presort_window(slots_out, tail->nnz_per_batch, tail->n_batches, C, tail->keys_out, stream);
      if (rc) return rc;
    }
  } else if (n > 0 && tail) {
    rc = presort_window_from_rows(slots_out, tail->nnz_per_batch, tail->n_batches, C, c.inverted_cached_idx,
                                  &h->ctl->status, tail->src_keys, tail->offsets, tail->offsets_are_i64,
                                  tail->offsets_batch_stride, tail->num_bags, tail->include_last_offset,
                                  tail->hook_features, tail->keys_out, s);
    if (rc) return rc;
  } else if (n > 0) {
    hipLaunchKernelGGL(k_slots, dim3(grid_for(n, 256 * 4)), dim3(256), 0, s, slots_out, n, c.inverted_cached_idx,
                       (const Ctl*)h->ctl);
  }
  if (prof) (void)hipEventRecord(prof->ev[x.pslot][x.pmark++], s);
  return CE_OK;
}

static int prepare_ids_second_half(ce_cache* h) {
  ce_cache::Pending& x = h->pend;
  if (x.chained) return chained_second_half(h);
  x.active = false;
  if (x.sel_pending) {
    x.sel_pending = false;
    SelArgs sel{x.sel_s, x.sel_n, x.worker, x.capturing, x.sel_steady, x.sel_out_job, x.seq_arg, x.sel_wbuf, x.sel_n_vblocks,
                x.pslot, x.prof, h->free_list};
    if (h->prof && (const void*)h->prof == x.prof) {
      (void)hipEventRecord(h->prof->resume[x.pslot], x.sel_s);
      h->prof->resumed[x.pslot] = true;
    }
    int rc0 = select_and_stage(h, sel, &x.pmark);
    if (rc0) return rc0;
  }
  const ce_cache_config_t& c = h->cfg;
  const Layout& L = h->L;
  const int64_t n = x.n;
  hipStream_t s = x.s;
  const bool worker = x.worker, capturing = x.capturing;
  const long long in_job = x.in_job;
  const int cap_groups = x.cap_groups, gpb = 256 >> h->g_log2;
  const dim3 swap_block(x.swap_threads);
  PhaseProf* const prof = (h->prof && (const void*)h->prof == x.prof) ? h->prof : nullptr;
  const int pslot = x.pslot;
  int rc = CE_OK;
  if (worker) {
    const long long scap = (long long)L.stage_rows;
    CE_HIP_CHECK(hipStreamWaitValue64(s, h->wb->sig, (uint64_t)in_job, hipStreamWaitValueGte, ~0ull));
    const int ugrid = (int)std::min<int64_t>(1024, std::max<int64_t>(1, cdiv(L.stage_rows, gpb)));
    if (h->vec) {
      hipLaunchKernelGGL((k_unpack_admitted<f32x4>), dim3(ugrid), dim3(256), 0, s, h->free_list,
                         (const long long*)&h->ctl->n_miss, scap, (const f32x4*)h->in_stage, (f32x4*)c.cache_weight,
                         h->rowlen, h->g_log2, h->ctl, (const unsigned long long*)(h->wb->sig_dev + 1),
                         in_job, (const int32_t*)h->miss_list,
                         L.list_cap > L.stage_rows ? (const f32x4*)c.host_weight_dev : (const f32x4*)nullptr);
    } else {
      hipLaunchKernelGGL((k_unpack_admitted<float>), dim3(ugrid), dim3(256), 0, s, h->free_list,
                         (const long long*)&h->ctl->n_miss, scap, (const float*)h->in_stage, (float*)c.cache_weight,
                         h->rowlen, h->g_log2, h->ctl, (const unsigned long long*)(h->wb->sig_dev + 1),
                         in_job, (const int32_t*)h->miss_list,
                         L.list_cap > L.stage_rows ? (const float*)c.host_weight_dev : (const float*)nullptr);
    }
  } else if (c.transport == CE_TRANSPORT_ZEROCOPY) {
    const long long scap = (long long)L.stage_rows;
    const int swap_rows = n <= 131072 ? 4 : kSwapRows;
    const int wb_groups = c.protect_depth > 0 ? std::max(1, cap_groups / 2) : cap_groups;
#define CE_SWAP(VT, R)                                                                                          \
  hipLaunchKernelGGL((k_swap<VT, R>), dim3(wb_groups + cap_groups), swap_block, 0, s, h->stage_idx,             \
                     (const VT*)h->stage, scap, wb_groups, h->miss_list, h->free_list,                           \
                     (const long long*)&h->ctl->n_miss,                                                          \
                     (VT*)c.host_weight_dev, (VT*)c.cache_weight, h->rowlen, h->g_log2, (const Ctl*)h->ctl)
    if (h->vec) {
      if (swap_rows == 4) CE_SWAP(f32x4, 4); else CE_SWAP(f32x4, 16);
    } else {
      CE_SWAP(float, 16);
    }
#undef CE_SWAP
  } else {
    const Ctl ctl = *h->ctl_host;
    const int64_t m = (ctl.status == CE_OK) ? ctl.n_miss : 0;
    if (m > 0) {
      const int D = c.embedding_dim;
      const size_t rowbytes = (size_t)D * sizeof(float);
      CE_HIP_CHECK(hipMemcpyAsync(h->list_host, h->miss_list, (size_t)m * 4, hipMemcpyDeviceToHost, s));
      CE_HIP_CHECK(hipStreamSynchronize(s));
      const float* table = c.host_weight;
      float* st = h->stage_host;
      const int64_t chunk = staged_chunk(h, m);
      for (int64_t off = 0; off < m; off += chunk) {
        const int64_t cnt = std::min(chunk, m - off);
        if (off > 0) CE_HIP_CHECK(hipStreamSynchronize(s));
        const int32_t* rows = h->list_host + off;
        host_pool(h)->parallel(cnt, [=](int64_t lo, int64_t hi) {
          for (int64_t i = lo; i < hi; ++i) memcpy(st + (size_t)i * D, table + (size_t)rows[i] * D, rowbytes);
        });
        CE_HIP_CHECK(hipMemcpyAsync(h->stage_dev, h->stage_host, (size_t)cnt * rowbytes, hipMemcpyHostToDevice, s));
        if (h->vec)
          hipLaunchKernelGGL((k_unpack_rows<f32x4>), dim3(grid_for(cnt, gpb)), dim3(256), 0, s,
                             (const int32_t*)h->free_list + off, (long long)cnt, (const f32x4*)h->stage_dev,
                             (f32x4*)c.cache_weight, h->rowlen, h->g_log2);
        else
          hipLaunchKernelGGL((k_unpack_rows<float>), dim3(grid_for(cnt, gpb)), dim3(256), 0, s,
                             (const int32_t*)h->free_list + off, (long long)cnt, (const float*)h->stage_dev,
                             (float*)c.cache_weight, h->rowlen, h->g_log2);
      }
    }
  }
  hipLaunchKernelGGL(k_admit_maps, dim3(grid_for(L.list_cap, 256)), dim3(256), 0, s, h->miss_list, h->free_list,
                     (const long long*)&h->ctl->n_miss, 0ll, c.cached_idx_map, c.inverted_cached_idx,
                     c.freq_cnter, (const int64_t*)nullptr, h->slot_epoch, 0, h->ctl, h->ring_dev,
                     x.seq_arg, x.worker ? (const unsigned long long*)(h->wb->sig_dev + 1) : nullptr, x.in_job);
  if (prof) (void)hipEventRecord(prof->ev[pslot][x.pmark++], s);
  rc = launch_slots_keys(h);
  if (rc) return rc;
  if (prof) prof->pending[pslot] = true;
  CE_LAUNCH_CHECK();
  if (!capturing) CE_HIP_CHECK(hipEventRecord(h->ev, s));
  return CE_OK;
}

extern "C" int ce_cache_prepare_ids(ce_cache_t* h, const int64_t* ids, int64_t n, int64_t* slots_out,
                                    ce_stream_t stream) {
  return prepare_ids_impl(h, ids, n, slots_out, stream, 0);
}

extern "C" int ce_cache_prepare_ids_keys(ce_cache_t* h, const int64_t* ids, int64_t n_batches, int64_t nnz_per_batch,
                                         int64_t* slots_out, int32_t src_keys, const void* offsets,
                                         int32_t offsets_are_i64, int64_t offsets_batch_stride, int64_t num_bags,
                                         int32_t include_last_offset, int64_t hook_features, uint64_t* keys_out,
                                         ce_stream_t stream) {
  CE_REQUIRE(n_batches > 0 && nnz_per_batch > 0 && keys_out, CE_ERR_INVALID, "bad window shape / null keys_out");
  KeysTail t{n_batches, nnz_per_batch, src_keys, offsets, offsets_are_i64, offsets_batch_stride, num_bags,
             include_last_offset, hook_features, keys_out};
  return prepare_ids_impl(h, ids, n_batches * nnz_per_batch, slots_out, stream, 0, &t);
}

extern "C" int ce_cache_prepare_ids_begin(ce_cache_t* h, const int64_t* ids, int64_t n_batches, int64_t nnz_per_batch,
                                          int64_t* slots_out, int32_t src_keys, const void* offsets,
                                          int32_t offsets_are_i64, int64_t offsets_batch_stride, int64_t num_bags,
                                          int32_t include_last_offset, int64_t hook_features, uint64_t* keys_out,
                                          ce_stream_t stream) {
  CE_REQUIRE(n_batches > 0 && nnz_per_batch > 0, CE_ERR_INVALID, "bad window shape");
  if (!keys_out) return prepare_ids_impl(h, ids, n_batches * nnz_per_batch, slots_out, stream, 0, nullptr, 1);
  KeysTail t{n_batches, nnz_per_batch, src_keys, offsets, offsets_are_i64, offsets_batch_stride, num_bags,
             include_last_offset, hook_features, keys_out};
  return prepare_ids_impl(h, ids, n_batches * nnz_per_batch, slots_out, stream, 0, &t, 1);
}

extern "C" int ce_cache_prepare_ids_finish(ce_cache_t* h, ce_stream_t stream) {
  CE_REQUIRE(h, CE_ERR_INVALID, "null handle");
  CE_REQUIRE(h->pend.active, CE_ERR_INVALID, "no cache op has been begun");
  CE_REQUIRE((hipStream_t)stream == h->pend.s, CE_ERR_INVALID, "finish the cache op on the stream it was begun on");
  return prepare_ids_second_half(h);
}

extern "C" int ce_cache_prepare_ids_padded(ce_cache_t* h, const int64_t* ids, int64_t n, int64_t* slots_out,
                                           ce_stream_t stream) {
  return prepare_ids_impl(h, ids, n, slots_out, stream, 1);
}

extern "C" int ce_cache_prepare_ids_begin_padded(ce_cache_t* h, const int64_t* ids, int64_t n, int64_t* slots_out,
                                                 ce_stream_t stream) {
  return prepare_ids_impl(h, ids, n, slots_out, stream, 1, nullptr, 1);
}

extern "C" int ce_cache_set_deferred_rows(ce_cache_t* h, int32_t on) {
  CE_REQUIRE(h, CE_ERR_INVALID, "null handle");
  CE_REQUIRE(!h->pend.active, CE_ERR_INVALID, "a cache op begun with ce_cache_prepare_ids_begin has not been finished");
  h->deferred_rows = on != 0;
  if (h->wb) h->wb->deferred_rows = h->deferred_rows;
  return CE_OK;
}

extern "C" int64_t ce_cache_rows_ticket(ce_cache_t* h) { return (h && h->wb && h->wb->chained) ? h->wb->chain_calls : 0; }

extern "C" int ce_cache_wait_rows(ce_cache_t* h, int64_t ticket, ce_stream_t stream) {
  CE_REQUIRE(h, CE_ERR_INVALID, "null handle");
  if (!h->wb || !h->wb->chained || h->wb->chain_calls == 0) return CE_OK;
  SwapEngine* const w = h->wb;
  long long t = (ticket <= 0 || ticket > w->chain_calls) ? w->chain_calls : ticket;
  if (t <= w->chain_calls - SwapEngine::kRowsRing) t = w->chain_calls - SwapEngine::kRowsRing + 1;
  CE_HIP_CHECK(hipStreamWaitEvent((hipStream_t)stream, w->ev_rows[t % SwapEngine::kRowsRing], 0));
  return CE_OK;
}

extern "C" int ce_cache_graph_replayed(ce_cache_t* h, int64_t n_calls, int64_t ids_per_call, ce_stream_t stream) {
  CE_REQUIRE(h && n_calls >= 0 && ids_per_call >= 0, CE_ERR_INVALID, "bad arguments");
  if (n_calls == 0) return CE_OK;
  CE_REQUIRE(n_calls <= kRing / 4, CE_ERR_INVALID, "report at most %d replayed calls at a time", kRing / 4);
  if (h->seq + n_calls - h->drained >= kRing / 2) {
    const int rc = sync_and_drain(h);
    if (rc) return rc;
  } else {
    drain(h);
  }
  h->seq += n_calls;
  CE_HIP_CHECK(hipEventRecord(h->ev, (hipStream_t)stream));
  if (h->cfg.evict_strategy == CE_EVICT_LFU) {
    h->freq_bound += (uint64_t)n_calls * (uint64_t)ids_per_call;
    CE_REQUIRE(h->freq_bound <= h->graph_freq_limit, CE_ERR_UNSUPPORTED,
               "the captured cache op's LFU key width is used up: capture it again");
  }
  return CE_OK;
}

extern "C" int ce_cache_last_stats(ce_cache_t* h, ce_call_stats_t* out) {
  CE_REQUIRE(h, CE_ERR_INVALID, "null handle");
  int rc = sync_and_drain(h);
  if (rc) return rc;
  if (h->history.empty()) {
    if (out) memset(out, 0, sizeof(*out));
    return CE_OK;
  }
  const ce_call_stats_t& r = h->history.back();
// ... 189 lines not shown
```

### cachedembedding_amd/csrc/ce_cache_index.h

```cpp
#pragma once

namespace ce {

constexpr int kChunkShift = 15;
constexpr int kChunkRows = 1 << kChunkShift;
constexpr int kCoarseShift = 6;
constexpr int kCoarsePad = 32;
constexpr int kSlotsPerBlock = 1024;
constexpr int kRing = 1024;
constexpr unsigned long long kGraphFreqHeadroom = 1ull << 31;
constexpr int kDigitBits = 11;
constexpr int kBins = 1 << kDigitBits;
constexpr int kLevels = 6;
constexpr int kHistWords = kLevels * kBins;
constexpr int32_t kEpochNever = -(1 << 30);
constexpr int64_t kHistoryKeep = 1 << 16;

struct Ctl {
  long long n_free;
  long long n_unique;
  long long n_miss;
  long long k_evict;
  long long miss_lookups;
  unsigned long long sel_prefix;
// ... 228 lines not shown
      idx[k][j] = b ? __ffs(b) - 1 : -1;
      b &= b - 1;
    }
  }
#pragma unroll
  for (int k = 0; k < 4; ++k)
#pragma unroll
    for (int j = 0; j < 5; ++j) val[k][j] = idx[k][j] >= 0 ? inverted[row0 + 32 * k + idx[k][j]] : 0;
#pragma unroll
  for (int k = 0; k < 4; ++k) {
    mm[k] = 0;
#pragma unroll
    for (int j = 0; j < 5; ++j) {
      if (idx[k][j] < 0) continue;
      if (val[k][j] < 0) mm[k] |= 1u << idx[k][j];
      else slot_epoch[val[k][j]] = epoch;
    }
    if (dense[k]) mm[k] = miss_mask_stamp(inverted, row0 + 32 * k, wds[k], N, slot_epoch, epoch);
  }
}

template <bool MERGE, int U>
__device__ __forceinline__ void mark_pass(const int64_t* __restrict__ ids, int64_t n,
                                          const int32_t* __restrict__ idx_map, const int32_t* __restrict__ inverted,
                                          int64_t N, int word_bits, int hot_words, uint32_t* hot, uint32_t* bitmap,
                                          int64_t* rows_out, int allow_pad, int* cold_out, bool* bad_out) {
  for (int w = threadIdx.x; w < hot_words; w += blockDim.x) hot[w] = 0;
  __syncthreads();
  const int lane = threadIdx.x & 63;
  const int64_t stride = (int64_t)gridDim.x * blockDim.x * U;
  int cold = 0;
  bool bad = false;
  for (int64_t i0 = ((int64_t)blockIdx.x * blockDim.x + (threadIdx.x & ~63)) * U; i0 < n; i0 += stride) {
    int32_t row[U], inv[U];
    uint32_t cur[U];
    bool valid[U];
#pragma unroll
    for (int u = 0; u < U; ++u) {
      const int64_t i = i0 + u * 64 + lane;
      valid[u] = i < n;
      row[u] = 0;
      if (valid[u]) {
        const int64_t id = ids[i];
        if ((unsigned long long)id >= (unsigned long long)N) {
          if (!(allow_pad && id == -1)) bad = true;
          valid[u] = false;
          rows_out[i] = -1;
        } else {
          row[u] = idx_map ? idx_map[id] : (int32_t)id;
        }
      }
    }
#pragma unroll
    for (int u = 0; u < U; ++u) {
      const int64_t i = i0 + u * 64 + lane;
      inv[u] = 0;
      cur[u] = ~0u;
      if (valid[u]) {
        rows_out[i] = row[u];
        inv[u] = inverted[row[u]];
        const int word = row[u] >> 5;
        if (word < hot_words) atomicOr(&hot[word], 1u << (row[u] & 31));
        else cur[u] = *(volatile uint32_t*)(bitmap + word);
      }
    }
#pragma unroll
    for (int u = 0; u < U; ++u) {
      const int word = row[u] >> 5;
      const int bidx = row[u] & 31;
      const bool need = valid[u] && (cur[u] & (1u << bidx)) == 0;
      if (valid[u]) cold += inv[u] < 0;
      if (!MERGE) {
        if (need) atomicOr(bitmap + word, 1u << bidx);
      } else if (__any(need)) {
        unsigned long long pm = __ballot(need);
        if (!need) pm = 0;
        for (int b = 0; b < word_bits; ++b) {
          const unsigned long long m = __ballot((word >> b) & 1);
          pm &= ((word >> b) & 1) ? m : ~m;
        }
        uint32_t orbits = 0;
#pragma unroll
        for (int b = 0; b < 32; ++b) {
          const unsigned long long m = __ballot(need && bidx == b);
          if (m & pm) orbits |= (1u << b);
        }
        if (need && (__ffsll((long long)pm) - 1) == lane) atomicOr(bitmap + word, orbits);
      }
    }
  }
  __syncthreads();
  for (int w0 = threadIdx.x; w0 < hot_words; w0 += (int)blockDim.x * 8) {
    uint32_t v[8], cur[8];
#pragma unroll
    for (int q = 0; q < 8; ++q) {
      const int w = w0 + q * (int)blockDim.x;
      v[q] = w < hot_words ? hot[w] : 0u;
    }
#pragma unroll
    for (int q = 0; q < 8; ++q) cur[q] = v[q] ? *(volatile uint32_t*)(bitmap + w0 + q * (int)blockDim.x) : ~0u;
#pragma unroll
    for (int q = 0; q < 8; ++q)
      if (v[q] && (cur[q] & v[q]) != v[q]) atomicOr(bitmap + w0 + q * (int)blockDim.x, v[q]);
  }
  *cold_out += cold;
  *bad_out = *bad_out || bad;
}

template <bool MERGE, int U>
__global__ __launch_bounds__(1024) void k_mark(const int64_t* __restrict__ ids, int64_t n,
                                              const int32_t* __restrict__ idx_map,
                                              const int32_t* __restrict__ inverted, int64_t N, int word_bits,
                                              int hot_words, uint32_t* bitmap, Ctl* ctl, int64_t* rows_out,
                                              int allow_pad) {
  extern __shared__ uint32_t hot[];
  int cold = 0;
  bool bad = false;
  mark_pass<MERGE, U>(ids, n, idx_map, inverted, N, word_bits, hot_words, hot, bitmap, rows_out, allow_pad, &cold, &bad);
  if (bad) ctl->status = CE_ERR_RANGE;
  cold = wave_sum(cold);
  if ((threadIdx.x & 63) == 0 && cold) atomicAdd((unsigned long long*)&ctl->miss_lookups, (unsigned long long)cold);
}

__global__ __launch_bounds__(256) void k_count(const uint4* __restrict__ bitmap4,
                                               const int32_t* __restrict__ inverted, int64_t N,
                                               int32_t* blk_unique, int32_t* blk_miss, int32_t* coarse) {
  const int64_t v = (int64_t)blockIdx.x * 256 + threadIdx.x;
  const uint4 q = bitmap4[v];
  const uint32_t wds[4] = {q.x, q.y, q.z, q.w};
  int u = 0, m = 0;
#pragma unroll
  for (int k = 0; k < 4; ++k) {
    if (!wds[k]) continue;
    u += __popc(wds[k]);
    m += __popc(miss_mask(inverted, v * 128 + k * 32, wds[k], N));
  }
  __shared__ int su[4], sm[4];
  u = wave_sum(u);
  m = wave_sum(m);
  if ((threadIdx.x & 63) == 0) {
    su[threadIdx.x >> 6] = u;
    sm[threadIdx.x >> 6] = m;
  }
  __syncthreads();
  if (threadIdx.x == 0) {
    const int tu = su[0] + su[1] + su[2] + su[3], tm = sm[0] + sm[1] + sm[2] + sm[3];
    blk_unique[blockIdx.x] = tu;
    blk_miss[blockIdx.x] = tm;
    if (tu) atomicAdd(&coarse[(2 * (blockIdx.x >> kCoarseShift)) * kCoarsePad], tu);
    if (tm) atomicAdd(&coarse[(2 * (blockIdx.x >> kCoarseShift) + 1) * kCoarsePad], tm);
  }
}

constexpr int kEmitSub = 1;
__global__ __launch_bounds__(256) void k_emit(uint4* bitmap4, const int32_t* __restrict__ inverted, int64_t N,
                                              const int32_t* __restrict__ blk_miss, const int32_t* __restrict__ coarse,
                                              int n_chunks, int32_t* miss_list, int32_t* slot_epoch, long long seq_arg,
                                              Ctl* ctl, int64_t C, int64_t n_ids, ce_call_stats_t* ring,
                                              WbMail* mail_in, long long job, long long in_cap, int32_t* miss_host,
                                              int assume_free0, long long* n_admit_out = nullptr) {
  const long long seq_ = call_seq(ctl, seq_arg);
  const int32_t epoch = call_epoch(seq_);
  ce_call_stats_t* const ring_slot = ring + (seq_ % kRing);
  __shared__ long long red[2 + kEmitSub][4];
  __shared__ int wsub[kEmitSub][4];
  const int lane = threadIdx.x & 63, wv = threadIdx.x >> 6;
  const int bid = (int)blockIdx.x, G = (int)gridDim.x;
  const int st_in = __hip_atomic_load(&ctl->status, __ATOMIC_RELAXED, __HIP_MEMORY_SCOPE_AGENT);
  int chunk[kEmitSub];
  uint4 q[kEmitSub];
#pragma unroll
  for (int j = 0; j < kEmitSub; ++j) {
    chunk[j] = bid + j * G;
    q[j] = make_uint4(0, 0, 0, 0);
    if (chunk[j] < n_chunks) q[j] = bitmap4[(int64_t)chunk[j] * 256 + threadIdx.x];
  }
  const int n_coarse = (n_chunks >> kCoarseShift) + 1;
  long long tu_p = 0, tm_p = 0, base_p[kEmitSub];
#pragma unroll
  for (int j = 0; j < kEmitSub; ++j) base_p[j] = 0;
  for (int g = threadIdx.x; g < n_coarse; g += 256) {
    const int cu = coarse[(2 * g) * kCoarsePad], cm = coarse[(2 * g + 1) * kCoarsePad];
    tu_p += cu;
    tm_p += cm;
#pragma unroll
    for (int j = 0; j < kEmitSub; ++j)
      if (g < (chunk[j] >> kCoarseShift)) base_p[j] += cm;
  }
#pragma unroll
  for (int j = 0; j < kEmitSub; ++j) {
    const int i = ((chunk[j] >> kCoarseShift) << kCoarseShift) + (int)(threadIdx.x & 63);
    if ((int)(threadIdx.x >> 6) == j && i < chunk[j] && chunk[j] < n_chunks) base_p[j] += blk_miss[i];
  }
#pragma unroll
  for (int d = 32; d >= 1; d >>= 1) {
    tu_p += __shfl_xor(tu_p, d);
    tm_p += __shfl_xor(tm_p, d);
#pragma unroll
    for (int j = 0; j < kEmitSub; ++j) base_p[j] += __shfl_xor(base_p[j], d);
  }
  if (lane == 0) {
    red[0][wv] = tu_p;
    red[1][wv] = tm_p;
#pragma unroll
    for (int j = 0; j < kEmitSub; ++j) red[2 + j][wv] = base_p[j];
  }
  __syncthreads();
  const long long tu = red[0][0] + red[0][1] + red[0][2] + red[0][3];
  const long long tm = red[1][0] + red[1][1] + red[1][2] + red[1][3];
  const bool stale = assume_free0 && ctl->n_free_start != 0;
  const bool ok = st_in == CE_OK && tu <= C && !stale;
  if (bid == 0 && threadIdx.x == 0) {
    int status = st_in;
    if (status == CE_OK && tu > C) status = CE_ERR_CAPACITY;
    if (status == CE_OK && stale) status = CE_ERR_HIP;
    long long k = 0;
    if (status == CE_OK) {
      k = tm - ctl->n_free;
      if (k < 0) k = 0;
      ctl->n_free = ctl->n_free + k - tm;
    }
    __hip_atomic_store(&ctl->status, status, __ATOMIC_RELAXED, __HIP_MEMORY_SCOPE_AGENT);
    ctl->n_unique = tu;
    ctl->n_miss = tm;
    ctl->k_evict = k;
    ctl->sel_krem = k;
    ring_slot->n_ids = n_ids;
    ring_slot->n_unique = tu;
    ring_slot->n_miss = tm;
    ring_slot->n_evict = k;
    ring_slot->miss_lookups = (status == CE_OK) ? ctl->miss_lookups : 0;
    ring_slot->n_free_after = ctl->n_free;
    ring_slot->status = status;
    ring_slot->kind = CE_CALL_PREPARE;
    if (mail_in) {
      const long long mrows = (status == CE_OK) ? tm : 0;
      mail_in->count = mrows < in_cap ? mrows : in_cap;
      mail_in->job = job;
    }
    if (n_admit_out) {
      const long long mrows = (status == CE_OK) ? tm : 0;
      *n_admit_out = mrows < in_cap ? mrows : in_cap;
    }
  }
  uint32_t mm[kEmitSub][4];
  int m[kEmitSub], inc[kEmitSub];
#pragma unroll
  for (int j = 0; j < kEmitSub; ++j) {
    m[j] = 0;
    const uint32_t wds[4] = {q[j].x, q[j].y, q[j].z, q[j].w};
    const int64_t v = (int64_t)chunk[j] * 256 + threadIdx.x;
#pragma unroll
    for (int k = 0; k < 4; ++k) {
      mm[j][k] = 0;
      if (ok && wds[k]) {
        mm[j][k] = miss_mask_stamp(inverted, v * 128 + k * 32, wds[k], N, slot_epoch, epoch);
        m[j] += __popc(mm[j][k]);
      }
    }
    inc[j] = wave_incl_scan(m[j], lane);
    if (lane == 63) wsub[j][wv] = inc[j];
  }
  __syncthreads();
  if (ok) {
#pragma unroll
    for (int j = 0; j < kEmitSub; ++j) {
      if (chunk[j] >= n_chunks) continue;
      int pos = (int)(red[2 + j][0] + red[2 + j][1] + red[2 + j][2] + red[2 + j][3]) + inc[j] - m[j];
      for (int k = 0; k < wv; ++k) pos += wsub[j][k];
      const int64_t v = (int64_t)chunk[j] * 256 + threadIdx.x;
#pragma unroll
      for (int k = 0; k < 4; ++k) {
        uint32_t bits = mm[j][k];
        const int64_t row0 = v * 128 + k * 32;
        while (bits) {
          const int b = __ffs(bits) - 1;
          bits &= bits - 1;
          if (miss_host && pos < in_cap) miss_host[pos] = (int32_t)(row0 + b);
          miss_list[pos++] = (int32_t)(row0 + b);
        }
      }
    }
  }
#pragma unroll
  for (int j = 0; j < kEmitSub; ++j)
    if (chunk[j] < n_chunks && (q[j].x | q[j].y | q[j].z | q[j].w))
      bitmap4[(int64_t)chunk[j] * 256 + threadIdx.x] = make_uint4(0, 0, 0, 0);
}

}
```

### cachedembedding_amd/csrc/ce_cache_rows.h

```cpp
#pragma once

namespace ce {

template <typename VT>
__device__ __forceinline__ void copy_row(const VT* __restrict__ src, VT* __restrict__ dst, int rowlen, int gl, int G) {
  for (int c = gl; c < rowlen; c += G) dst[c] = src[c];
}

constexpr int kSwapRows = 16;

template <typename VT>
__global__ __launch_bounds__(1024) void k_evict(const int32_t* __restrict__ victims, int32_t* cached_idx_map,
                                               int32_t* inverted, const VT* __restrict__ cache, VT* host,
                                               long long first, int rowlen, int g_log2, const Ctl* ctl) {
  const long long k = (ctl->status == CE_OK) ? ctl->k_evict : 0;
  if (k <= first) return;
  const int G = 1 << g_log2;
  const int gl = threadIdx.x & (G - 1);
  const int64_t gstride = ((int64_t)gridDim.x * blockDim.x) >> g_log2;
  if (!host) return;
  for (int64_t i = first + (((int64_t)blockIdx.x * blockDim.x + threadIdx.x) >> g_log2) * kSwapRows; i < k;
       i += gstride * kSwapRows) {
    if (rowlen <= G) {
      VT v[kSwapRows];
// ... 257 lines not shown
  for (int i = threadIdx.x; i < (int)blockIdx.x; i += 256) part += blk_free[i];
  part = wave_sum(part);
  if ((threadIdx.x & 63) == 0) wsum4[threadIdx.x >> 6] = part;
  __syncthreads();
  const long long before = (long long)wsum4[0] + wsum4[1] + wsum4[2] + wsum4[3];
  if (before >= need) return;
  const int64_t s0 = ((int64_t)blockIdx.x * 256 + threadIdx.x) * 4;
  int fl[4];
  int f = 0;
#pragma unroll
  for (int t = 0; t < 4; ++t) {
    fl[t] = (s0 + t < C) && (cached_idx_map[s0 + t] < 0);
    f += fl[t];
  }
  int tot;
  long long pos = block_excl_scan_256(f, &tot) + before;
#pragma unroll
  for (int t = 0; t < 4; ++t) {
    if (fl[t]) {
      if (pos < need) free_list[pos] = (int32_t)(s0 + t);
      ++pos;
    }
  }
}

__global__ __launch_bounds__(1024) void k_free_single(const int32_t* __restrict__ cached_idx_map, int64_t C,
                                                      int32_t* free_list, const Ctl* ctl) {
  if (ctl->status != CE_OK || ctl->n_miss == 0) return;
  const long long need = ctl->n_miss;
  __shared__ int wtot[16];
  __shared__ long long base_s;
  if (threadIdx.x == 0) base_s = 0;
  __syncthreads();
  const int lane = threadIdx.x & 63, w = threadIdx.x >> 6;
  for (int64_t s0 = 0; s0 < C; s0 += 4096) {
    const long long base = base_s;
    if (base >= need) break;
    const int64_t i0 = s0 + (int64_t)threadIdx.x * 4;
    int fl[4], f = 0;
#pragma unroll
    for (int t = 0; t < 4; ++t) {
      fl[t] = (i0 + t < C) && (cached_idx_map[i0 + t] < 0);
      f += fl[t];
    }
    const int inc = wave_incl_scan(f, lane);
    if (lane == 63) wtot[w] = inc;
    __syncthreads();
    int pre = 0, tot = 0;
    for (int k = 0; k < 16; ++k) {
      if (k < w) pre += wtot[k];
      tot += wtot[k];
    }
    long long pos = base + pre + inc - f;
#pragma unroll
    for (int t = 0; t < 4; ++t) {
      if (fl[t]) {
        if (pos < need) free_list[pos] = (int32_t)(i0 + t);
        ++pos;
      }
    }
    __syncthreads();
    if (threadIdx.x == 0) base_s = base + tot;
    __syncthreads();
  }
}

template <typename VT, int R>
__device__ __forceinline__ void admit_rows(const int32_t* __restrict__ rows, const int32_t* __restrict__ slots,
                                           const long long* n_ptr, long long n_imm, const VT* __restrict__ host,
                                           VT* cache, int rowlen, int g_log2, const Ctl* ctl, int block, int nblocks,
                                           long long first = 0) {
  if (ctl && ctl->status != CE_OK) return;
  const long long n = n_ptr ? *n_ptr : n_imm;
  const int G = 1 << g_log2;
  const int gl = threadIdx.x & (G - 1);
  const int64_t gstride = ((int64_t)nblocks * blockDim.x) >> g_log2;
  for (int64_t i = first + (((int64_t)block * blockDim.x + threadIdx.x) >> g_log2) * R; i < n; i += gstride * R) {
    if (rowlen <= G) {
      VT v[R];
      int64_t dst[R];
#pragma unroll
      for (int t = 0; t < R; ++t) {
        dst[t] = -1;
        if (i + t < n) {
          const int64_t row = rows ? rows[i + t] : i + t;
          dst[t] = slots ? slots[i + t] : i + t;
          if (gl < rowlen) v[t] = host[row * rowlen + gl];
        }
      }
#pragma unroll
      for (int t = 0; t < R; ++t)
        if (dst[t] >= 0 && gl < rowlen) cache[dst[t] * rowlen + gl] = v[t];
    } else {
      for (int t = 0; t < R && i + t < n; ++t) {
        const int64_t row = rows ? rows[i + t] : i + t;
        const int64_t slot = slots ? slots[i + t] : i + t;
        copy_row(host + row * rowlen, cache + slot * rowlen, rowlen, gl, G);
      }
    }
  }
}

template <typename VT, int R = kSwapRows>
__global__ __launch_bounds__(1024) void k_admit(const int32_t* __restrict__ rows, const int32_t* __restrict__ slots,
                                               const long long* n_ptr, long long n_imm,
                                               const VT* __restrict__ host, VT* cache, int rowlen, int g_log2,
                                               const Ctl* ctl, long long first) {
  admit_rows<VT, R>(rows, slots, n_ptr, n_imm, host, cache, rowlen, g_log2, ctl, (int)blockIdx.x,
                    (int)gridDim.x, first);
}

template <typename VT, int R = kSwapRows>
__global__ __launch_bounds__(1024) void k_admit_probe(const int32_t* __restrict__ rows, const long long* n_ptr,
                                                     const VT* __restrict__ host, VT* dst, int rowlen, int g_log2,
                                                     const unsigned long long* __restrict__ evt_keys,
                                                     const int32_t* __restrict__ evt_pos, uint32_t evt_mask,
                                                     uint32_t tag, const VT* __restrict__ prev_stage) {
  const long long n = *n_ptr;
  const int G = 1 << g_log2;
  const int gl = threadIdx.x & (G - 1);
  const int64_t gstride = ((int64_t)gridDim.x * blockDim.x) >> g_log2;
  for (int64_t i = (((int64_t)blockIdx.x * blockDim.x + threadIdx.x) >> g_log2) * R; i < n; i += gstride * R) {
    if (rowlen <= G) {
      VT v[R];
#pragma unroll
      for (int t = 0; t < R; ++t) {
        if (i + t < n) {
          const int32_t row = rows[i + t];
          const int32_t p = evt_keys ? evt_find(evt_keys, evt_pos, evt_mask, tag, row) : -1;
          const VT* src = p >= 0 ? prev_stage + (int64_t)p * rowlen : host + (int64_t)row * rowlen;
          if (gl < rowlen) v[t] = src[gl];
        }
      }
#pragma unroll
      for (int t = 0; t < R; ++t)
        if (i + t < n && gl < rowlen) dst[(i + t) * rowlen + gl] = v[t];
    } else {
      for (int t = 0; t < R && i + t < n; ++t) {
        const int32_t row = rows[i + t];
        const int32_t p = evt_keys ? evt_find(evt_keys, evt_pos, evt_mask, tag, row) : -1;
        copy_row(p >= 0 ? prev_stage + (int64_t)p * rowlen : host + (int64_t)row * rowlen, dst + (i + t) * rowlen,
                 rowlen, gl, G);
      }
    }
  }
}

template <typename VT>
__global__ __launch_bounds__(256) void k_unpack_admitted(const int32_t* __restrict__ slots, const long long* n_ptr,
                                                         long long cap, const VT* __restrict__ in_stage, VT* cache,
                                                         int rowlen, int g_log2, Ctl* ctl,
                                                         const unsigned long long* fail_word, long long job,
                                                         const int32_t* __restrict__ rows,
                                                         const VT* __restrict__ host_overflow) {
  const bool ok = ctl->status == CE_OK;
  if (blockIdx.x == 0 && threadIdx.x == 0) {
    ctl->lost = *(volatile const unsigned long long*)fail_word == (unsigned long long)job;
  }
  if (!ok) return;
  long long n = *n_ptr;
  const int G = 1 << g_log2;
  const int gl = threadIdx.x & (G - 1);
  const int64_t gstride = ((int64_t)gridDim.x * blockDim.x) >> g_log2;
  if (host_overflow && n > cap) {
    for (int64_t i = cap + (((int64_t)blockIdx.x * blockDim.x + threadIdx.x) >> g_log2); i < n; i += gstride)
      copy_row(host_overflow + (int64_t)rows[i] * rowlen, cache + (int64_t)slots[i] * rowlen, rowlen, gl, G);
  }
  if (n > cap) n = cap;
  constexpr int R = kStageRowsInFlight;
  for (int64_t i = (((int64_t)blockIdx.x * blockDim.x + threadIdx.x) >> g_log2) * R; i < n; i += gstride * R) {
    if (rowlen <= G) {
      int32_t slot[R];
      VT v[R];
#pragma unroll
      for (int t = 0; t < R; ++t) {
        slot[t] = i + t < n ? slots[i + t] : -1;
        if (slot[t] >= 0 && gl < rowlen) v[t] = in_stage[(i + t) * rowlen + gl];
      }
#pragma unroll
      for (int t = 0; t < R; ++t)
        if (slot[t] >= 0 && gl < rowlen) cache[(int64_t)slot[t] * rowlen + gl] = v[t];
    } else {
      for (int t = 0; t < R && i + t < n; ++t)
        copy_row(in_stage + (i + t) * rowlen, cache + (int64_t)slots[i + t] * rowlen, rowlen, gl, G);
    }
  }
}

template <typename VT, int R>
__global__ __launch_bounds__(1024) void k_swap(const int32_t* __restrict__ stage_rows_idx,
                                              const VT* __restrict__ stage, long long cap, int wb_blocks,
                                              const int32_t* __restrict__ rows, const int32_t* __restrict__ slots,
                                              const long long* n_ptr, VT* host, VT* cache, int rowlen, int g_log2,
                                              const Ctl* ctl) {
  if ((int)blockIdx.x < wb_blocks)
    writeback_rows<VT, R>(stage_rows_idx, stage, host, cap, rowlen, g_log2, ctl, (int)blockIdx.x, wb_blocks);
  else
    admit_rows<VT, R>(rows, slots, n_ptr, 0ll, (const VT*)host, cache, rowlen, g_log2, ctl,
                      (int)blockIdx.x - wb_blocks, (int)gridDim.x - wb_blocks);
}

__global__ __launch_bounds__(256) void k_admit_maps(const int32_t* __restrict__ rows,
                                                    const int32_t* __restrict__ slots, const long long* n_ptr,
                                                    long long n_imm, int32_t* cached_idx_map, int32_t* inverted,
                                                    int64_t* freq, const int64_t* freq_vals, int32_t* slot_epoch,
                                                    int32_t epoch_imm, Ctl* ctl, ce_call_stats_t* ring,
                                                    long long seq_arg, const unsigned long long* fail_word,
                                                    long long job, long long* n_unpack_out = nullptr) {
  const long long seq = ring ? call_seq(ctl, seq_arg) : 0;
  const int32_t epoch = ring ? call_epoch(seq) : epoch_imm;
  ce_call_stats_t* const ring_slot = ring ? ring + (seq % kRing) : nullptr;
  const bool lost = fail_word && ctl->lost != 0;
  if (ring_slot && blockIdx.x == 0 && threadIdx.x == 0) {
    if (n_unpack_out) *n_unpack_out = (ctl->status == CE_OK && n_ptr) ? *n_ptr : 0;
    if (lost && ctl->status == CE_OK) {
      ctl->n_free = ctl->n_free + ctl->n_miss;
      ring_slot->status = CE_ERR_HIP;
      ring_slot->n_free_after = ctl->n_free;
      __hip_atomic_store(&ctl->status, CE_ERR_HIP, __ATOMIC_RELAXED, __HIP_MEMORY_SCOPE_AGENT);
    }
    __threadfence_system();
    *(volatile long long*)&ring_slot->seq = seq;
  }
  if (lost) return;
  if (ctl && __hip_atomic_load(&ctl->status, __ATOMIC_RELAXED, __HIP_MEMORY_SCOPE_AGENT) != CE_OK) return;
  const long long n = n_ptr ? *n_ptr : n_imm;
  const int64_t stride = (int64_t)gridDim.x * blockDim.x;
  for (int64_t i = (int64_t)blockIdx.x * blockDim.x + threadIdx.x; i < n; i += stride) {
    const int32_t row = rows ? rows[i] : (int32_t)i;
    const int32_t slot = slots ? slots[i] : (int32_t)i;
    cached_idx_map[slot] = row;
    inverted[row] = slot;
    if (freq) freq[slot] = freq_vals ? freq_vals[i] : 0;
    slot_epoch[slot] = epoch;
  }
}

__global__ __launch_bounds__(256) void k_lookup(const int64_t* __restrict__ ids, int64_t n,
                                                const int32_t* __restrict__ idx_map,
                                                const int32_t* __restrict__ inverted, int64_t N, int64_t* slots_out) {
  const int64_t stride = (int64_t)gridDim.x * blockDim.x;
  for (int64_t i = (int64_t)blockIdx.x * blockDim.x + threadIdx.x; i < n; i += stride) {
    const int64_t id = ids[i];
    int64_t slot = -1;
    if ((unsigned long long)id < (unsigned long long)N) slot = inverted[idx_map ? idx_map[id] : (int32_t)id];
    slots_out[i] = slot;
  }
}

__global__ __launch_bounds__(256) void k_slots(int64_t* slots, int64_t n, const int32_t* __restrict__ inverted,
                                               const Ctl* ctl) {
  const bool failed = ctl->status != CE_OK;
  constexpr int U = 4;
  const int64_t stride = (int64_t)gridDim.x * blockDim.x * U;
  for (int64_t i0 = (int64_t)blockIdx.x * blockDim.x * U + threadIdx.x; i0 < n; i0 += stride) {
    int64_t row[U];
#pragma unroll
    for (int u = 0; u < U; ++u) {
      const int64_t i = i0 + (int64_t)u * blockDim.x;
      row[u] = i < n ? slots[i] : -1;
    }
#pragma unroll
    for (int u = 0; u < U; ++u) {
      const int64_t i = i0 + (int64_t)u * blockDim.x;
      if (i < n) slots[i] = (failed || row[u] < 0) ? -1 : (int64_t)inverted[row[u]];
    }
  }
}

constexpr int kSlotsHashBits = 13;
constexpr int kSlotsHash = 1 << kSlotsHashBits;
__global__ __launch_bounds__(1024) void k_slots_lfu(int64_t* slots, int64_t n, const int32_t* __restrict__ inverted,
                                                    int64_t* freq, const Ctl* ctl) {
  __shared__ int hkey[kSlotsHash];
  __shared__ int hcnt[kSlotsHash];
  for (int i = threadIdx.x; i < kSlotsHash; i += blockDim.x) { hkey[i] = -1; hcnt[i] = 0; }
  __syncthreads();
  const bool failed = ctl->status != CE_OK;
  const int64_t per_block = (n + gridDim.x - 1) / gridDim.x;
  const int64_t lo = (int64_t)blockIdx.x * per_block;
  const int64_t hi = lo + per_block < n ? lo + per_block : n;
  constexpr int U = 4;
  for (int64_t i0 = lo + threadIdx.x; i0 < hi; i0 += (int64_t)blockDim.x * U) {
    int64_t row[U];
    int slot[U];
#pragma unroll
    for (int u = 0; u < U; ++u) {
      const int64_t i = i0 + (int64_t)u * blockDim.x;
      row[u] = (i < hi && !failed) ? slots[i] : -1;
    }
#pragma unroll
    for (int u = 0; u < U; ++u) slot[u] = row[u] >= 0 ? inverted[row[u]] : -1;
#pragma unroll
    for (int u = 0; u < U; ++u) {
      const int64_t i = i0 + (int64_t)u * blockDim.x;
      if (i < hi) slots[i] = slot[u];
      if (slot[u] < 0) continue;
      unsigned h = ((unsigned)slot[u] * 2654435761u) >> (32 - kSlotsHashBits);
      bool done = false;
      for (int p = 0; p < 16 && !done; ++p) {
        const int old = atomicCAS(&hkey[h], -1, slot[u]);
        if (old == -1 || old == slot[u]) {
          atomicAdd(&hcnt[h], 1);
          done = true;
        } else {
          h = (h + 1) & (kSlotsHash - 1);
        }
      }
      if (!done) atomicAdd((unsigned long long*)&freq[slot[u]], 1ull);
    }
  }
  __syncthreads();
  for (int i = threadIdx.x; i < kSlotsHash; i += blockDim.x)
    if (hkey[i] >= 0) atomicAdd((unsigned long long*)&freq[hkey[i]], (unsigned long long)hcnt[i]);
}

template <typename VT>
__global__ __launch_bounds__(256) void k_flush_rows(const int32_t* __restrict__ cached_idx_map, int64_t C,
                                                    const VT* __restrict__ cache, VT* host, int rowlen,
                                                    int g_log2) {
  const int G = 1 << g_log2;
  const int gl = threadIdx.x & (G - 1);
  const int64_t gstride = ((int64_t)gridDim.x * blockDim.x) >> g_log2;
  for (int64_t s = ((int64_t)blockIdx.x * blockDim.x + threadIdx.x) >> g_log2; s < C; s += gstride) {
    const int32_t row = cached_idx_map[s];
    if (row >= 0) copy_row(cache + s * rowlen, host + (int64_t)row * rowlen, rowlen, gl, G);
  }
}

__global__ __launch_bounds__(256) void k_flush_maps(int32_t* cached_idx_map, int64_t C, int32_t* inverted,
                                                    int64_t* freq, int32_t* slot_epoch, Ctl* ctl) {
  const int64_t stride = (int64_t)gridDim.x * blockDim.x;
  int n = 0;
  for (int64_t s = (int64_t)blockIdx.x * blockDim.x + threadIdx.x; s < C; s += stride) {
    const int32_t row = cached_idx_map[s];
    if (row >= 0) {
      inverted[row] = -1;
// ... 72 lines not shown
```

### cachedembedding_amd/csrc/ce_cache_worker.h

```cpp
#pragma once

namespace ce {

class RowPool {
 public:
  explicit RowPool(int n) {
    cpu_set_t set;
    const bool near = near_gpu_cpus(&set);
    for (int i = 0; i < n; ++i)
      workers_.emplace_back([this, i, near, set] {
        if (near) (void)sched_setaffinity(0, sizeof set, &set);
        run(i);
      });
  }
  ~RowPool() {
    {
      std::lock_guard<std::mutex> g(m_);
      stop_ = true;
      ++gen_;
    }
    cv_.notify_all();
    for (auto& t : workers_) t.join();
  }
  void parallel(int64_t n, const std::function<void(int64_t, int64_t)>& fn) {
// ... 21 lines not shown
    std::unique_lock<std::mutex> g(m_);
    done_.wait(g, [this] { return pending_ == 0; });
  }
  int size() const { return (int)workers_.size(); }

 private:
  void run(int id) {
    unsigned long long seen = 0;
    for (;;) {
      const std::function<void(int64_t, int64_t)>* fn;
      int64_t n;
      int parts;
      {
        std::unique_lock<std::mutex> g(m_);
        cv_.wait(g, [&] { return gen_ != seen; });
        seen = gen_;
        if (stop_) return;
        fn = fn_;
        n = n_;
        parts = parts_;
      }
      if (id < parts) {
        const int64_t per = cdiv(n, parts);
        const int64_t lo = id * per, hi = std::min<int64_t>(n, lo + per);
        if (lo < hi) (*fn)(lo, hi);
        std::lock_guard<std::mutex> g(m_);
        if (--pending_ == 0) done_.notify_all();
      }
    }
  }
  std::vector<std::thread> workers_;
  std::mutex m_;
  std::condition_variable cv_, done_;
  const std::function<void(int64_t, int64_t)>* fn_ = nullptr;
  int64_t n_ = 0;
  int parts_ = 0, pending_ = 0;
  unsigned long long gen_ = 0;
  bool stop_ = false;
};

constexpr int kPhases = 6;
constexpr int kProfDepth = 8;
static const char* const kPhaseNames[kPhases] = {"unique_and_miss", "find_evict_ids", "evict_stage",
                                                  "free_slots", "admit_swap", "ids_to_slots"};
struct PhaseProf {
  hipEvent_t ev[kProfDepth][kPhases + 1];
  bool pending[kProfDepth];
  hipEvent_t resume[kProfDepth];
  bool resumed[kProfDepth];
  hipEvent_t adm0[kProfDepth], adm1[kProfDepth];
  bool chained[kProfDepth];
  double ms[kPhases];
  long long calls;
  PhaseProf() : calls(0) {
    for (int i = 0; i < kProfDepth; ++i) {
      pending[i] = false;
      resumed[i] = false;
      chained[i] = false;
      (void)hipEventCreate(&resume[i]);
      (void)hipEventCreate(&adm0[i]);
      (void)hipEventCreate(&adm1[i]);
      for (int j = 0; j <= kPhases; ++j) (void)hipEventCreate(&ev[i][j]);
    }
    for (int j = 0; j < kPhases; ++j) ms[j] = 0;
  }
  ~PhaseProf() {
    for (int i = 0; i < kProfDepth; ++i) {
      (void)hipEventDestroy(resume[i]);
      (void)hipEventDestroy(adm0[i]);
      (void)hipEventDestroy(adm1[i]);
      for (int j = 0; j <= kPhases; ++j) (void)hipEventDestroy(ev[i][j]);
    }
  }
  void collect(int i) {
    if (!pending[i]) return;
    if (hipEventSynchronize(ev[i][kPhases]) == hipSuccess &&
        (!chained[i] || hipEventSynchronize(adm1[i]) == hipSuccess)) {
      for (int j = 0; j < kPhases; ++j) {
        float t = 0;
        hipError_t e;
        if (chained[i] && j == 4) e = hipEventElapsedTime(&t, adm0[i], adm1[i]);
        else e = hipEventElapsedTime(&t, (j == 1 && resumed[i]) ? resume[i] : ev[i][j], ev[i][j + 1]);
        if (e == hipSuccess) ms[j] += t;
      }
      calls += 1;
    }
    pending[i] = false;
    resumed[i] = false;
    chained[i] = false;
  }
};

void row_copy_stream(float* dst, const float* src, size_t floats);
void row_copy_fence();

static double worker_timeout_s() {
  static const double v = [] { const char* e = getenv("CE_WORKER_TIMEOUT_S"); const double t = e ? atof(e) : 30.0; return t > 0 ? t : 30.0; }();
  return v;
}
static inline void tight_timer_slack() { (void)prctl(PR_SET_TIMERSLACK, 1000ul, 0ul, 0ul, 0ul); }

static inline hipError_t stream_wait_polite(hipStream_t st, double timeout_s = worker_timeout_s()) {
  const auto t0 = std::chrono::steady_clock::now();
  for (int spins = 0;; ++spins) {
    const hipError_t e = hipStreamQuery(st);
    if (e != hipErrorNotReady) return e;
    if (spins < 50) std::this_thread::yield();
    else std::this_thread::sleep_for(std::chrono::microseconds(15));
    if ((spins & 1023) == 1023 && std::chrono::duration<double>(std::chrono::steady_clock::now() - t0).count() > timeout_s)
      return hipErrorNotReady;
  }
}

static inline hipError_t event_wait_polite(hipEvent_t ev, double timeout_s = worker_timeout_s()) {
  const auto t0 = std::chrono::steady_clock::now();
  for (int spins = 0;; ++spins) {
    const hipError_t e = hipEventQuery(ev);
    if (e != hipErrorNotReady) return e;
    if (spins < 50) std::this_thread::yield();
    else std::this_thread::sleep_for(std::chrono::microseconds(15));
    if ((spins & 1023) == 1023 && std::chrono::duration<double>(std::chrono::steady_clock::now() - t0).count() > timeout_s)
      return hipErrorNotReady;
  }
}

static const bool g_trace = [] { const char* e = getenv("CE_WORKER_TRACE"); return e && atoi(e) != 0; }();
#define CE_TRACE(...)                                                                            \
  do {                                                                                           \
    if (ce::g_trace) {                                                                           \
      const double t_ = std::chrono::duration<double>(std::chrono::steady_clock::now().time_since_epoch()).count(); \
      fprintf(stderr, "[ce %.6f %p] ", t_, (void*)this);                                         \
      fprintf(stderr, __VA_ARGS__);                                                              \
      fputc('\n', stderr);                                                                       \
    }                                                                                            \
  } while (0)

struct SwapEngine {
  int device = 0;
  int64_t D = 0, stage_rows = 0;
  float* table = nullptr;
  hipStream_t out_stream = nullptr, out_stream2 = nullptr;
  hipEvent_t out_ev[2] = {nullptr, nullptr};
  static constexpr int kOutChunks = 8;
  hipEvent_t chunk_ev[kOutChunks + 1] = {nullptr};
  const float* stage_dev[2] = {nullptr, nullptr};
  const int32_t* idx_dev[2] = {nullptr, nullptr};
  float* rows_host[2] = {nullptr, nullptr};
  int32_t* idx_host[2] = {nullptr, nullptr};
  hipStream_t in_stream = nullptr;
  hipEvent_t in_ev[2] = {nullptr, nullptr};
  float* in_stage_dev = nullptr;
  float* in_host = nullptr;
  bool chained = false;
  hipEvent_t ev_miss[2] = {nullptr, nullptr};
  static constexpr int kRowsRing = 4;
  hipEvent_t ev_rows[kRowsRing] = {nullptr};
  long long chain_calls = 0;
  long long probe_floor = 1;
  bool deferred_rows = false;
  const unsigned long long* evt_keys[2] = {nullptr, nullptr};
  const int32_t* evt_pos[2] = {nullptr, nullptr};
  uint32_t evt_mask = 0;
  long long in_probed = 0;
#ifdef CE_TEST_HOOKS
  int out_delay_us = 0;
  long long fail_in_job = 0;
#endif
  int rowlen = 0, g_log2 = 0, vec = 0;
  int32_t* miss_host = nullptr;
  int32_t* miss_host_dev = nullptr;
  unsigned long long* sig = nullptr;
  unsigned long long* sig_dev = nullptr;
  WbMail* mail = nullptr;
  WbMail* mail_dev = nullptr;
  std::thread out_thread, in_thread;
  std::mutex m;
  std::condition_variable cv_job, cv_done;
  long long out_issued = 0, out_done = 0, in_issued = 0, in_done = 0;
  bool stop = false;
  int err = 0;
  char errmsg[256] = {0};
  RowPool* out_pool = nullptr;
  RowPool* in_pool = nullptr;
  double out_wait_s = 0, out_busy_s = 0, in_wait_s = 0, in_busy_s = 0, in_gather_s = 0;
  double out_wait0_s = 0;
  double out_copy_wait_s = 0, out_scatter_s = 0;
  long long out_rows = 0, out_jobs = 0, in_rows = 0, in_jobs = 0;

  void fail(const char* what, hipError_t e) {
    std::lock_guard<std::mutex> g(m);
    if (!err) {
      err = CE_ERR_HIP;
      snprintf(errmsg, sizeof errmsg, "swap worker: %s failed: %s", what, hipGetErrorString(e));
    }
  }
  bool failed() {
    std::lock_guard<std::mutex> g(m);
    return err != 0;
  }

  void run_out() {
    (void)hipSetDevice(device);
    bind_thread_near_gpu();
    tight_timer_slack();
    for (;;) {
      long long job;
      {
        std::unique_lock<std::mutex> g(m);
        cv_job.wait(g, [&] { return stop || out_done < out_issued; });
        if (out_done >= out_issued) return;
        job = out_done + 1;
      }
      const int b = (int)(job & 1);
      const auto t0 = std::chrono::steady_clock::now();
      CE_TRACE("out job %lld: waiting for its staging event", job);
      hipError_t e = hipEventSynchronize(out_ev[b]);
      if (e != hipSuccess) fail("hipEventSynchronize(out)", e);
      const auto t1 = std::chrono::steady_clock::now();
      long long k = mail[b].count;
      double copy_wait = 0, scatter = 0, wait0 = 0;
#ifdef CE_TEST_HOOKS
      if (out_delay_us > 0) std::this_thread::sleep_for(std::chrono::microseconds(out_delay_us));
#endif
      CE_TRACE("out job %lld: event done (%s), mail job %lld count %lld", job, hipGetErrorString(e), mail[b].job, k);
      if (mail[b].job != job || k < 0 || k > stage_rows) k = 0;
      if (k > 0 && !failed()) {
        e = hipMemcpyAsync(idx_host[b], idx_dev[b], (size_t)k * 4, hipMemcpyDeviceToHost, out_stream);
        const int64_t per = std::max<int64_t>(4096, cdiv(k, kOutChunks));
        int nch = 0;
        for (int64_t off = 0; off < k && e == hipSuccess; off += per, ++nch) {
          const int64_t cnt = std::min<int64_t>(per, k - off);
          hipStream_t cs = (nch & 1) ? out_stream2 : out_stream;
          e = hipMemcpyAsync(rows_host[b] + off * D, stage_dev[b] + off * D, (size_t)cnt * D * 4, hipMemcpyDeviceToHost, cs);
          if (e == hipSuccess) e = hipEventRecord(chunk_ev[nch], cs);
        }
        int c = 0;
        for (int64_t off = 0; off < k && e == hipSuccess; off += per, ++c) {
          const int64_t cnt = std::min<int64_t>(per, k - off);
          const auto tc0 = std::chrono::steady_clock::now();
          hipError_t e2 = event_wait_polite(chunk_ev[c]);
          const auto tc1 = std::chrono::steady_clock::now();
          copy_wait += std::chrono::duration<double>(tc1 - tc0).count();
          if (c == 0) wait0 = std::chrono::duration<double>(tc1 - tc0).count();
          if (e == hipSuccess) e = e2;
          if (e != hipSuccess) break;
          float* tb = table;
          const float* st = rows_host[b] + off * D;
          const int32_t* ri = idx_host[b] + off;
          const int64_t d = D;
          out_pool->parallel(cnt, [=](int64_t lo, int64_t hi) {
            for (int64_t i = lo; i < hi; ++i) {
              if (i + 8 < hi) __builtin_prefetch((const void*)((uintptr_t)(tb + (size_t)ri[i + 8] * d) ^ 2048u), 0, 0);
              row_copy_stream(tb + (size_t)ri[i] * d, st + (size_t)i * d, (size_t)d);
            }
            row_copy_fence();
          });
          scatter += std::chrono::duration<double>(std::chrono::steady_clock::now() - tc1).count();
        }
        if (e == hipSuccess) {
          e = stream_wait_polite(out_stream);
          if (e == hipSuccess) e = stream_wait_polite(out_stream2);
        }
        if (e != hipSuccess) fail(e == hipErrorNotReady ? "write-back copy timed out (CE_WORKER_TIMEOUT_S)" : "D2H copy", e);
      }
      const auto t2 = std::chrono::steady_clock::now();
      CE_TRACE("out job %lld: done", job);
      {
        std::lock_guard<std::mutex> g(m);
        out_done = job;
        out_wait_s += std::chrono::duration<double>(t1 - t0).count();
        out_busy_s += std::chrono::duration<double>(t2 - t1).count();
        out_copy_wait_s += copy_wait;
        out_wait0_s += wait0;
        out_scatter_s += scatter;
        out_rows += k;
        out_jobs += 1;
      }
      cv_done.notify_all();
    }
  }

  void run_in() {
    (void)hipSetDevice(device);
    bind_thread_near_gpu();
    tight_timer_slack();
    for (;;) {
      long long job, need_out;
      {
        std::unique_lock<std::mutex> g(m);
        cv_job.wait(g, [&] { return stop || in_done < in_issued; });
        if (in_done >= in_issued) return;
        job = in_done + 1;
        need_out = out_issued_at[job & 7];
      }
      const auto t0 = std::chrono::steady_clock::now();
      CE_TRACE("in job %lld: waiting for its miss-list event (needs out job %lld)", job, need_out);
      hipError_t e = hipEventSynchronize(in_ev[job & 1]);
      if (e != hipSuccess) fail("hipEventSynchronize(in)", e);
      CE_TRACE("in job %lld: event done (%s)", job, hipGetErrorString(e));
      {
        std::unique_lock<std::mutex> g(m);
        cv_done.wait(g, [&] { return out_done >= need_out || err != 0; });
      }
      const auto t1 = std::chrono::steady_clock::now();
      long long n = mail[2].count;
      CE_TRACE("in job %lld: earlier write-backs landed; mail job %lld count %lld", job, mail[2].job, n);
      if (mail[2].job != job || n < 0 || n > stage_rows) n = 0;
#ifdef CE_TEST_HOOKS
      if (fail_in_job > 0 && job == fail_in_job) fail("admission (injected: CE_WORKER_FAIL_IN_JOB)", hipErrorUnknown);
#endif
      if (n > 0 && !failed()) {
        const float* tb = table;
        float* st = in_host;
        float* dv = in_stage_dev;
        const int32_t* rows = miss_host;
        const int64_t d = D;
        hipStream_t cs = in_stream;
        constexpr int kAhead = 8;
        constexpr int64_t kPiece = 2048, kCopyPieces = 4;
        const int64_t npieces = cdiv(n, kPiece);
        std::atomic<int64_t> next{0};
        std::vector<std::atomic<unsigned char>> ready((size_t)npieces);
        for (auto& r : ready) r.store(0, std::memory_order_relaxed);
        const std::function<void(int64_t, int64_t)> work = [&](int64_t, int64_t) {
          for (;;) {
            const int64_t pc = next.fetch_add(1, std::memory_order_relaxed);
            if (pc >= npieces) break;
            const int64_t lo = pc * kPiece, hi = std::min<int64_t>(n, lo + kPiece);
            for (int64_t i = lo; i < hi; ++i) {
              if (i + kAhead < hi) {
                const char* q = (const char*)(tb + (size_t)rows[i + kAhead] * d);
                for (int64_t l = 0; l < d * 4; l += 64) __builtin_prefetch(q + l);
              }
              row_copy_stream(st + (size_t)i * d, tb + (size_t)rows[i] * d, (size_t)d);
            }
            row_copy_fence();
            ready[(size_t)pc].store(1, std::memory_order_release);
          }
        };
        const int helpers = (int)std::min<int64_t>(in_pool->size(), npieces);
        in_pool->start(helpers, helpers, work);
        int64_t cursor = 0;
        int idle = 0;
        while (cursor < npieces) {
          int64_t k = 0;
          while (cursor + k < npieces && ready[(size_t)(cursor + k)].load(std::memory_order_acquire)) ++k;
          if (k >= kCopyPieces || (k > 0 && cursor + k == npieces)) {
            const int64_t lo = cursor * kPiece, hi = std::min<int64_t>(n, (cursor + k) * kPiece);
            e = hipMemcpyAsync(dv + (size_t)lo * d, st + (size_t)lo * d, (size_t)(hi - lo) * d * 4,
                               hipMemcpyHostToDevice, cs);
            if (e != hipSuccess) { fail("hipMemcpyAsync(H2D)", e); break; }
            cursor += k;
            idle = 0;
          } else if (++idle < 64) {
            std::this_thread::yield();
          } else {
            std::this_thread::sleep_for(std::chrono::microseconds(10));
          }
        }
        in_pool->wait();
      }
      const auto tg = std::chrono::steady_clock::now();
      CE_TRACE("in job %lld: rows gathered, copies enqueued", job);
      e = stream_wait_polite(in_stream);
      if (e != hipSuccess) fail(e == hipErrorNotReady ? "admission timed out (CE_WORKER_TIMEOUT_S)" : "waiting for the H2D copies", e);
      if (n > 0 && failed()) __atomic_store_n(sig + 1, (unsigned long long)job, __ATOMIC_RELEASE);
      __atomic_store_n(sig, (unsigned long long)job, __ATOMIC_RELEASE);
      CE_TRACE("in job %lld: released the stream (%s)", job, hipGetErrorString(e));
      const auto t2 = std::chrono::steady_clock::now();
      {
        std::lock_guard<std::mutex> g(m);
        in_done = job;
        in_wait_s += std::chrono::duration<double>(t1 - t0).count();
        in_busy_s += std::chrono::duration<double>(t2 - t1).count();
        in_gather_s += std::chrono::duration<double>(tg - t1).count();
        in_rows += n;
        in_jobs += 1;
      }
      cv_done.notify_all();
    }
  }
  long long out_issued_at[8] = {0};
  hipStream_t tested_stream = nullptr;
  bool tested = false;

  int check() {
    std::lock_guard<std::mutex> g(m);
    if (err) {
      set_error("%s", errmsg);
      return err;
    }
    return CE_OK;
  }
  int give_up(const char* what) {
    {
      std::lock_guard<std::mutex> g(m);
      if (!err) {
        err = CE_ERR_HIP;
        snprintf(errmsg, sizeof errmsg, "swap worker: %s did not finish within %.0f s (CE_WORKER_TIMEOUT_S)", what,
                 2 * worker_timeout_s());
      }
    }
    if (sig) {
      __atomic_store_n(sig + 1, (unsigned long long)in_issued, __ATOMIC_RELEASE);
      __atomic_store_n(sig, ~0ull >> 1, __ATOMIC_RELEASE);
    }
    return check();
  }
  int wait_out(long long upto) {
    bool ok;
    {
      std::unique_lock<std::mutex> g(m);
      ok = cv_done.wait_for(g, std::chrono::duration<double>(2 * worker_timeout_s()),
                            [&] { return out_done >= upto || out_done >= out_issued; });
    }
    return ok ? check() : give_up("a write-back job");
  }
  int wait_in(long long upto) {
    bool ok;
    {
      std::unique_lock<std::mutex> g(m);
      ok = cv_done.wait_for(g, std::chrono::duration<double>(2 * worker_timeout_s()),
                            [&] { return in_done >= upto || in_done >= in_issued; });
    }
    return ok ? check() : give_up("an admission job");
  }
  void push_out() {
    {
      std::lock_guard<std::mutex> g(m);
      ++out_issued;
      CE_TRACE("push out job %lld", out_issued);
    }
    cv_job.notify_all();
  }
  void push_in(long long need_out) {
    {
      std::lock_guard<std::mutex> g(m);
      ++in_issued;
      out_issued_at[in_issued & 7] = need_out;
      CE_TRACE("push in job %lld (needs out %lld)", in_issued, need_out);
    }
    cv_job.notify_all();
  }

  ~SwapEngine() {
    {
      std::lock_guard<std::mutex> g(m);
      stop = true;
    }
    if (const char* e = getenv("CE_WORKER_PROFILE"))
      if (atoi(e) != 0 && in_jobs > 0)
        fprintf(stderr, "[libce_hip] admission worker: %lld jobs, %lld of them with the previous write-back still on its "
                "way (rows it evicted taken from its staging buffer)\n", in_jobs, in_probed);
    if (const char* e = getenv("CE_WORKER_PROFILE"))
      if (atoi(e) != 0 && out_jobs > 0)
        fprintf(stderr, "[libce_hip] write-back worker: %lld jobs, %.3f ms busy per job = %.3f waiting for copies + %.3f "
                "scattering + %.3f other; %.0f rows per job; first chunk's wait %.3f\n", out_jobs, out_busy_s / out_jobs * 1e3,
                out_copy_wait_s / out_jobs * 1e3, out_scatter_s / out_jobs * 1e3,
                (out_busy_s - out_copy_wait_s - out_scatter_s) / out_jobs * 1e3, (double)out_rows / out_jobs,
                out_wait0_s / out_jobs * 1e3);
    cv_job.notify_all();
    if (in_thread.joinable()) in_thread.join();
    if (out_thread.joinable()) out_thread.join();
    delete out_pool;
    delete in_pool;
    for (int b = 0; b < 2; ++b) {
      if (out_ev[b]) (void)hipEventDestroy(out_ev[b]);
      if (rows_host[b]) (void)hipHostFree(rows_host[b]);
      if (idx_host[b]) (void)hipHostFree(idx_host[b]);
    }
    for (int b = 0; b < 2; ++b)
      if (in_ev[b]) (void)hipEventDestroy(in_ev[b]);
    for (auto& ev : ev_miss)
      if (ev) (void)hipEventDestroy(ev);
    for (auto& ev : ev_rows)
      if (ev) (void)hipEventDestroy(ev);

    for (auto& ev : chunk_ev)
      if (ev) (void)hipEventDestroy(ev);
    if (in_host) (void)hipHostFree(in_host);
    if (miss_host) (void)hipHostFree(miss_host);
    if (sig) (void)hipHostFree(sig);
    if (mail) (void)hipHostFree(mail);
    if (out_stream) (void)hipStreamDestroy(out_stream);
    if (out_stream2) (void)hipStreamDestroy(out_stream2);
    if (in_stream) (void)hipStreamDestroy(in_stream);
  }
};

}
```

### include/ce_api.h

```cpp
#ifndef CE_API_H
#define CE_API_H

#include <stddef.h>
#include <stdint.h>

#ifdef __cplusplus
extern "C" {
#endif

#define CE_API_VERSION 6

#define CE_OK 0
#define CE_ERR_INVALID 1
#define CE_ERR_HIP 2
#define CE_ERR_CAPACITY 3
#define CE_ERR_NOMEM 4
#define CE_ERR_UNSUPPORTED 5
#define CE_ERR_RANGE 6

#define CE_EVICT_DATASET 0
#define CE_EVICT_LFU 1

#define CE_MODE_SUM 0
#define CE_MODE_MEAN 1
// ... 83 lines not shown
                                   int64_t num_bags, int32_t include_last_offset, int64_t hook_features,
                                   const int64_t* ids, uint64_t* keys_out, int64_t* seg_id_ranges,
                                   ce_stream_t stream);
int ce_bag_backward_sgd_presorted_src_excl(float* weight, int64_t num_rows, int32_t dim, int64_t nnz,
                                           const float* grad_out, float lr, const uint64_t* src_keys,
                                           const int64_t* seg_id_ranges, ce_stream_t stream);

size_t ce_bag_backward_sgd_sorted_workspace(int64_t num_rows, int64_t nnz);
int ce_bag_backward_sgd_sorted(float* weight, int64_t num_rows, int32_t dim,
                               const int64_t* indices, int64_t nnz,
                               const void* offsets, int32_t offsets_are_i64, int64_t num_bags,
                               int32_t include_last_offset, const float* per_sample_weights,
                               int32_t mode, int64_t hook_features, const float* grad_out, float lr,
                               void* workspace, size_t workspace_bytes, ce_stream_t stream);

size_t ce_bag_backward_rowwise_adagrad_workspace(int64_t num_rows, int32_t dim);
int ce_bag_backward_rowwise_adagrad(float* weight, int64_t num_rows, int32_t dim, const int64_t* indices, int64_t nnz,
                                    const void* offsets, int32_t offsets_are_i64, int64_t num_bags,
                                    int32_t include_last_offset, const float* per_sample_weights, int32_t mode,
                                    int64_t hook_features, const float* grad_out, const uint64_t* presorted,
                                    const int32_t* row_of_slot, float* momentum, int64_t momentum_rows, float lr,
                                    float eps, void* workspace, size_t workspace_bytes, ce_stream_t stream);
int ce_bag_backward_rowwise_adagrad_src(float* weight, int64_t num_rows, int32_t dim, int64_t nnz,
                                        const float* grad_out, const uint64_t* src_keys, const int32_t* row_of_slot,
                                        float* momentum, int64_t momentum_rows, float lr, float eps, void* workspace,
                                        size_t workspace_bytes, ce_stream_t stream);

int ce_bag_forward_act(const float* weight, int64_t num_rows, int32_t dim,
                       const int64_t* indices, int64_t nnz,
                       const void* offsets, int32_t offsets_are_i64, int64_t num_bags,
                       int32_t include_last_offset, const float* per_sample_weights,
                       int32_t mode, int64_t hook_features, void* out, int32_t act_dtype, ce_stream_t stream);
int ce_bag_forward_src_keys_act(const float* weight, int64_t num_rows, int32_t dim, int64_t nnz,
                                const uint64_t* src_keys, void* out, int32_t act_dtype, ce_stream_t stream);
int ce_bag_backward_dense_act(float* grad_weight, int64_t num_rows, int32_t dim,
                              const int64_t* indices, int64_t nnz,
                              const void* offsets, int32_t offsets_are_i64, int64_t num_bags,
                              int32_t include_last_offset, const float* per_sample_weights,
                              int32_t mode, int64_t hook_features, const void* grad_out, int32_t act_dtype,
                              const uint64_t* presorted_keys, ce_stream_t stream);
int ce_bag_backward_sgd_act(float* weight, int64_t num_rows, int32_t dim,
                            const int64_t* indices, int64_t nnz,
                            const void* offsets, int32_t offsets_are_i64, int64_t num_bags,
                            int32_t include_last_offset, const float* per_sample_weights,
                            int32_t mode, int64_t hook_features, const void* grad_out, int32_t act_dtype, float lr,
                            const uint64_t* presorted_keys, ce_stream_t stream);
int ce_bag_backward_sgd_src_act(float* weight, int64_t num_rows, int32_t dim, int64_t nnz,
                                const void* grad_out, int32_t act_dtype, float lr, const uint64_t* src_keys,
                                const int64_t* seg_id_ranges, ce_stream_t stream);
int ce_bag_backward_dense_src_act(float* grad_weight, int64_t num_rows, int32_t dim, int64_t nnz,
                                  const void* grad_out, int32_t act_dtype, const uint64_t* src_keys,
                                  ce_stream_t stream);
int ce_bag_backward_rowwise_adagrad_act(float* weight, int64_t num_rows, int32_t dim, const int64_t* indices,
                                        int64_t nnz, const void* offsets, int32_t offsets_are_i64, int64_t num_bags,
                                        int32_t include_last_offset, const float* per_sample_weights, int32_t mode,
                                        int64_t hook_features, const void* grad_out, int32_t act_dtype,
                                        const uint64_t* presorted, const int32_t* row_of_slot, float* momentum,
                                        int64_t momentum_rows, float lr, float eps, void* workspace,
                                        size_t workspace_bytes, ce_stream_t stream);
int ce_bag_backward_rowwise_adagrad_src_act(float* weight, int64_t num_rows, int32_t dim, int64_t nnz,
                                            const void* grad_out, int32_t act_dtype, const uint64_t* src_keys,
                                            const int32_t* row_of_slot, float* momentum, int64_t momentum_rows,
                                            float lr, float eps, void* workspace, size_t workspace_bytes,
                                            ce_stream_t stream);

typedef struct ce_cache_config {
  int64_t num_embeddings;
  int64_t cuda_row_num;
  int32_t embedding_dim;
  int32_t evict_strategy;
  int32_t transport;
  int32_t protect_depth;
  int64_t max_ids_per_call;
  float* host_weight;
  float* host_weight_dev;
  float* cache_weight;
  int32_t* idx_map;
  int32_t* inverted_cached_idx;
  int32_t* cached_idx_map;
  int64_t* freq_cnter;
  void* workspace;
  size_t workspace_bytes;
} ce_cache_config_t;

typedef struct ce_call_stats {
  int64_t seq;
  int64_t n_ids;
  int64_t n_unique;
  int64_t n_miss;
  int64_t n_evict;
  int64_t miss_lookups;
  int64_t n_free_after;
  int32_t status;
  int32_t kind;
} ce_call_stats_t;

#define CE_CALL_PREPARE 0
#define CE_CALL_PRELOAD 1
#define CE_CALL_FLUSH 2

size_t ce_cache_workspace_bytes(int64_t num_embeddings, int64_t cuda_row_num, int64_t max_ids_per_call,
                                int32_t embedding_dim);

int ce_cache_create(const ce_cache_config_t* cfg, ce_stream_t stream, ce_cache_t** out);
int ce_cache_destroy(ce_cache_t* h);

int ce_cache_preload(ce_cache_t* h, const int32_t* rows, const int64_t* freq_vals, int64_t n,
                     ce_stream_t stream);

int ce_cache_set_freq_bound(ce_cache_t* h, int64_t bound);

int ce_cache_prepare_ids(ce_cache_t* h, const int64_t* ids, int64_t n, int64_t* slots_out,
                         ce_stream_t stream);
int ce_cache_prepare_ids_keys(ce_cache_t* h, const int64_t* ids, int64_t n_batches, int64_t nnz_per_batch,
                              int64_t* slots_out, int32_t src_keys, const void* offsets, int32_t offsets_are_i64,
                              int64_t offsets_batch_stride, int64_t num_bags, int32_t include_last_offset,
                              int64_t hook_features, uint64_t* keys_out, ce_stream_t stream);
int ce_cache_prepare_ids_begin(ce_cache_t* h, const int64_t* ids, int64_t n_batches, int64_t nnz_per_batch,
                               int64_t* slots_out, int32_t src_keys, const void* offsets, int32_t offsets_are_i64,
                               int64_t offsets_batch_stride, int64_t num_bags, int32_t include_last_offset,
                               int64_t hook_features, uint64_t* keys_out, ce_stream_t stream);
int ce_cache_prepare_ids_finish(ce_cache_t* h, ce_stream_t stream);
int ce_cache_prepare_ids_padded(ce_cache_t* h, const int64_t* ids, int64_t n, int64_t* slots_out,
                                ce_stream_t stream);
int ce_cache_prepare_ids_begin_padded(ce_cache_t* h, const int64_t* ids, int64_t n, int64_t* slots_out,
                                      ce_stream_t stream);

int ce_cache_set_deferred_rows(ce_cache_t* h, int32_t on);
int64_t ce_cache_rows_ticket(ce_cache_t* h);
int ce_cache_wait_rows(ce_cache_t* h, int64_t ticket, ce_stream_t stream);

int ce_cache_last_stats(ce_cache_t* h, ce_call_stats_t* out);
int ce_cache_totals(ce_cache_t* h, int64_t* cpu_to_cuda_numel, int64_t* cuda_to_cpu_numel,
                    int64_t* cache_miss, int64_t* total_cache, int64_t* n_calls);
int ce_cache_failures(ce_cache_t* h, int64_t* n_failed, int32_t* last_status, int64_t* last_seq);
int64_t ce_cache_history(ce_cache_t* h, int64_t first_seq, ce_call_stats_t* out, int64_t cap);

int ce_cache_lookup_slots(ce_cache_t* h, const int64_t* ids, int64_t n, int64_t* slots_out,
                          ce_stream_t stream);

int ce_cache_flush(ce_cache_t* h, ce_stream_t stream);

int ce_cache_set_protect_depth(ce_cache_t* h, int32_t depth);
int ce_cache_set_transport(ce_cache_t* h, int32_t transport);
int32_t ce_cache_get_transport(ce_cache_t* h);
int ce_cache_set_cache_weight(ce_cache_t* h, float* cache_weight);
int ce_cache_graph_replayed(ce_cache_t* h, int64_t n_calls, int64_t ids_per_call, ce_stream_t stream);
int ce_cache_set_profiling(ce_cache_t* h, int32_t on);
int32_t ce_cache_phase_count(void);
const char* ce_cache_phase_name(int32_t i);
int ce_cache_phase_times(ce_cache_t* h, double* ms_out, int32_t cap, int64_t* calls, int32_t reset);
int ce_cache_writeback_wait(ce_cache_t* h);
int ce_cache_swap_stats(ce_cache_t* h, double* seconds6, int64_t* counts4);
int ce_cache_set_buffer_rows(ce_cache_t* h, int64_t rows);
int ce_cache_free_rows(ce_cache_t* h, int64_t* out);

size_t ce_bucketize_workspace(int64_t n, int32_t world);
int ce_bucketize_rows(const int64_t* ids, int64_t n, const int32_t* idx_map, int32_t world,
                      int64_t* local_rows_out, int64_t* perm_out, int64_t* counts_out,
                      void* workspace, size_t workspace_bytes, ce_stream_t stream);

int ce_dedupe_bucket_rows(const int64_t* ids, int64_t n, const int32_t* idx_map, int64_t num_rows,
                          int32_t world, int32_t* stamp, int32_t* slot_of_row, int32_t* scratch,
                          int64_t* local_rows_out, int64_t* pos_out, int64_t* counts_out, ce_stream_t stream);

int ce_dedupe_bucket_rows_padded(const int64_t* ids, int64_t n, const int32_t* idx_map, int64_t num_rows,
                                 int32_t world, int64_t capacity, int32_t* stamp, int32_t* slot_of_row,
                                 int32_t* scratch, int64_t* local_rows_out, int64_t* pos_out, int64_t* counts_out,
                                 int32_t* overflow_flag, ce_stream_t stream);

int ce_dedupe_bucket_rows_padded_window(const int64_t* ids, int64_t n, int64_t n_batches, const int32_t* idx_map,
                                        int64_t num_rows, int32_t world, int64_t capacity, int32_t* stamp,
                                        int32_t* slot_of_row, int32_t* scratch, int64_t* local_rows_out,
                                        int64_t* pos_out, int64_t* counts_out, int32_t* overflow_flag,
                                        ce_stream_t stream);

int ce_exchange_local_index(const int64_t* pos, int64_t n_per_batch, int64_t n_batches, const int64_t* slots,
                            int64_t slots_batch_stride, int64_t local_lo, int64_t local_hi, int64_t tail_base,
                            int64_t* index_out, ce_stream_t stream);

int ce_split_classify(const int64_t* serve, int32_t world, int32_t n_batches, int64_t capacity, int64_t n_local_rows,
                      const int64_t* prev, int64_t n_prev, uint64_t* mask, uint8_t* flags_out, ce_stream_t stream);

int ce_split_places(const int64_t* ids, const uint8_t* flags, int32_t n_batches, int32_t world, int64_t capacity,
                    int32_t skip_peer, const int32_t* caps, int32_t* place_fwd, int32_t* place_bwd,
                    int32_t* counts_out, int32_t* overflow_flag, ce_stream_t stream);

int ce_exchange_local_index_split(const int64_t* pos, int64_t n_per_batch, int64_t n_batches, const int64_t* slots,
                                  const int32_t* place_fwd, const int32_t* place_bwd, int64_t chunk_stride,
                                  int64_t local_lo, int64_t local_hi, int64_t tail_base, int64_t bwd_base,
                                  const int32_t* caps, int32_t world, int64_t n_early, int64_t n_urgent,
                                  int64_t n_deferred, int64_t* index_fwd, int64_t* index_bwd, ce_stream_t stream);

int ce_bag_forward_max(const float* weight, int64_t num_rows, int32_t dim, const int64_t* indices, int64_t nnz,
                       const void* offsets, int32_t offsets_are_i64, int64_t num_bags, int32_t include_last_offset,
                       int64_t hook_features, float* out, int32_t* max_pos, ce_stream_t stream);
int ce_bag_backward_max(float* dst, int64_t num_rows, int32_t dim, const int64_t* indices, int64_t nnz,
                        int64_t num_bags, int64_t hook_features, const float* grad_out, const int32_t* max_pos,
                        float alpha, ce_stream_t stream);
int ce_bag_backward_psw(const float* weight, int64_t num_rows, int32_t dim, const int64_t* indices, int64_t nnz,
                        const void* offsets, int32_t offsets_are_i64, int64_t num_bags, int32_t include_last_offset,
                        int64_t hook_features, const float* grad_out, float* grad_psw, ce_stream_t stream);
size_t ce_rows_renorm_workspace(int64_t num_rows);
int ce_rows_renorm(float* weight, int64_t num_rows, int32_t dim, const int64_t* indices, int64_t n, float max_norm,
                   float norm_type, void* workspace, size_t workspace_bytes, ce_stream_t stream);

int ce_rows_axpy(float* weight, int64_t num_rows, int32_t dim, const int64_t* index, int64_t n,
                 const float* src_rows, float alpha, ce_stream_t stream);

#ifdef __cplusplus
}
#endif
#endif
```

Measured before the change: 3.198 billion.

## Add switchable host-gather admission path that reads rows from previous eviction staging

Adds a runtime-selectable admission engine (kernel-chained zero-copy vs host-thread gather plus copy), with an auto mode gated by a compile-time constant that is currently false, so auto still picks the kernel path. The copy path no longer waits for the previous write-back to land: missed rows that the prior eviction still holds are tagged in the miss list, skipped by the host gather, and read from the previous staging buffer on device during unpack. This is meant to remove the serialization between write-back and admission. In exchange it adds hash probes in the emit and unpack kernels and a device-side wait on the event at the start of eviction for the copy path.

```diff
diff --git a/cachedembedding_amd/_lib.py b/cachedembedding_amd/_lib.py
--- a/cachedembedding_amd/_lib.py
+++ b/cachedembedding_amd/_lib.py
@@ -27,6 +27,9 @@
 CE_TRANSPORT_ZEROCOPY = 0
 CE_TRANSPORT_STAGED = 1
 CE_TRANSPORT_WORKER = 2
+CE_ADMIT_KERNEL = 0
+CE_ADMIT_COPY = 1
+CE_ADMIT_AUTO = 2
 CE_CALL_PREPARE = 0
 CE_CALL_PRELOAD = 1
 CE_CALL_FLUSH = 2
@@ -177,6 +180,8 @@
     "ce_cache_phase_times": (c_int, [c_void_p, POINTER(c_double), c_int32, POINTER(c_int64), c_int32]),
     "ce_cache_writeback_wait": (c_int, [c_void_p]),
     "ce_cache_swap_stats": (c_int, [c_void_p, POINTER(c_double), POINTER(c_int64)]),
+    "ce_cache_set_admission": (c_int, [c_void_p, c_int32]),
+    "ce_cache_admission_stats": (c_int, [c_void_p, POINTER(c_int64)]),
     "ce_cache_failures": (c_int, [c_void_p, POINTER(c_int64), POINTER(c_int32), POINTER(c_int64)]),
     "ce_cache_free_rows": (c_int, [c_void_p, POINTER(c_int64)]),
     "ce_bucketize_workspace": (c_size_t, [c_int64, c_int32]),
diff --git a/cachedembedding_amd/cache_mgr.py b/cachedembedding_amd/cache_mgr.py
--- a/cachedembedding_amd/cache_mgr.py
+++ b/cachedembedding_amd/cache_mgr.py
@@ -460,6 +460,17 @@
         return dict(out_wait_s=sec[0], out_busy_s=sec[1], in_wait_s=sec[2], in_busy_s=sec[3], in_gather_s=sec[4],
                     rows=cnt[0], jobs=cnt[1], in_rows=cnt[2], in_jobs=cnt[3], in_jobs_before_writeback_landed=int(sec[5]))
 
+    _ADMISSIONS = {"kernel": _lib.CE_ADMIT_KERNEL, "copy": _lib.CE_ADMIT_COPY, "auto": _lib.CE_ADMIT_AUTO}
+
+    def set_admission(self, mode: str = "auto"):
+        check(lib.ce_cache_set_admission(self._handle, self._ADMISSIONS[mode]))
+
+    def admission_stats(self) -> dict:
+        cnt = (ctypes.c_int64 * 4)()
+        check(lib.ce_cache_admission_stats(self._handle, cnt))
+        return dict(engine={v: k for k, v in self._ADMISSIONS.items()}[int(cnt[0])], copy_jobs=int(cnt[1]),
+                    jobs_before_writeback_landed=int(cnt[2]), rows_from_previous_staging=int(cnt[3]))
+
     def raise_on_failed_calls(self):
         n, st, sq = ctypes.c_int64(), ctypes.c_int32(), ctypes.c_int64()
         check(lib.ce_cache_failures(self._handle, ctypes.byref(n), ctypes.byref(st), ctypes.byref(sq)))
diff --git a/cachedembedding_amd/csrc/ce_cache.hip b/cachedembedding_amd/csrc/ce_cache.hip
--- a/cachedembedding_amd/csrc/ce_cache.hip
+++ b/cachedembedding_amd/csrc/ce_cache.hip
@@ -77,6 +77,7 @@
   bool free_zero;
   long long free_reset_seq;
   bool deferred_rows;
+  int admission;
   struct Pending {
     bool active = false;
     int64_t n = 0;
@@ -86,6 +87,8 @@
     long long in_job = 0, seq_arg = 0;
     int cap_groups = 1, swap_threads = 256, pslot = 0, pmark = 0;
     bool chained = false;
+    bool probe_prev = false;
+    long long prev_job = 0;
     long long call = 0;
     int parity = 0;
     bool sel_pending = false;
@@ -256,6 +259,7 @@
   h->free_zero = false;
   h->free_reset_seq = 0;
   h->deferred_rows = false;
+  h->admission = CE_ADMIT_AUTO;
   h->stage2 = (float*)(h->ws + L.stage2);
   h->stage_idx2 = (int32_t*)(h->ws + L.stage_idx2);
   h->in_stage = (float*)(h->ws + L.in_stage);
@@ -411,10 +415,12 @@
     w->in_stage_dev = h->in_stage;
     {
       const char* e = getenv("CE_WORKER_ADMIT");
-      w->chained = !(e && !strcmp(e, "sdma")) && h->cfg.host_weight_dev != nullptr;
+      if (e && (!strcmp(e, "sdma") || !strcmp(e, "copy"))) w->env_admit = 1;
+      else if (e && !strcmp(e, "kernel")) w->env_admit = 0;
+      w->chained = h->cfg.host_weight_dev != nullptr;
     }
     {
-      if (w->chained && !h->evt_keys[0]) {
+      if (!h->evt_keys[0]) {
         uint32_t places = 4096;
         while ((int64_t)places < 4 * L.stage_rows && places < (1u << 30)) places <<= 1;
         bool ok = (int64_t)places >= 4 * L.stage_rows;
@@ -477,9 +483,7 @@
     w->miss_host = (int32_t*)p;
     if (hipHostGetDevicePointer(&pd, p, 0) != hipSuccess) pd = p;
     w->miss_host_dev = (int32_t*)pd;
-    if (!w->chained &&
-        hipHostMalloc((void**)&w->in_host, rows_bytes, hipHostMallocDefault) != hipSuccess) { rc = CE_ERR_NOMEM; break; }
-    if (w->chained) {
+    {
       for (auto& ev : w->ev_miss)
         if (rc == CE_OK && hipEventCreateWithFlags(&ev, hipEventDisableTiming) != hipSuccess) rc = CE_ERR_HIP;
       for (auto& ev : w->ev_rows)
@@ -506,7 +510,6 @@
     w->g_log2 = h->g_log2;
     w->vec = h->vec;
     w->out_thread = std::thread([w] { w->run_out(); });
-    if (!w->chained) w->in_thread = std::thread([w] { w->run_in(); });
   } while (0);
   if (rc) {
     delete w;
@@ -515,6 +518,57 @@
   }
   w->deferred_rows = h->deferred_rows;
   h->wb = w;
+  return CE_OK;
+}
+
+constexpr bool kAutoCopyAdmission = false;
+constexpr int64_t kAutoCopyMinIds = 300000;
+constexpr int kAutoCopyMinCpus = 12;
+static bool admission_for_call(const ce_cache* h, int64_t n) {
+  if (!h->cfg.host_weight_dev) return false;
+  if (h->wb->env_admit >= 0) return h->wb->env_admit == 0;
+  if (h->admission == CE_ADMIT_KERNEL) return true;
+  if (h->admission == CE_ADMIT_COPY) return false;
+  return !(kAutoCopyAdmission && n >= kAutoCopyMinIds && cpu_budget() >= kAutoCopyMinCpus);
+}
+
+static int switch_admission(ce_cache* h, bool chained) {
+  SwapEngine* const w = h->wb;
+  int rc = w->wait_out(w->out_issued);
+  if (rc == CE_OK) rc = w->wait_in(w->in_issued);
+  if (rc) return rc;
+  CE_HIP_CHECK(hipEventSynchronize(h->ev));
+  if (hipEvent_t ev = last_rows_event(h)) CE_HIP_CHECK(hipEventSynchronize(ev));
+  drain(h);
+  w->probe_floor = w->out_issued + 1;
+  if (!chained) {
+    if (!w->in_host)
+      CE_HIP_CHECK(hipHostMalloc((void**)&w->in_host, (size_t)w->stage_rows * w->D * 4, hipHostMallocDefault));
+    if (!w->in_thread.joinable()) w->in_thread = std::thread([w] { w->run_in(); });
+  }
+  w->chained = chained;
+  return CE_OK;
+}
+
+extern "C" int ce_cache_set_admission(ce_cache_t* h, int32_t mode) {
+  CE_REQUIRE(h && (mode == CE_ADMIT_KERNEL || mode == CE_ADMIT_COPY || mode == CE_ADMIT_AUTO), CE_ERR_INVALID,
+             "bad admission mode");
+  CE_REQUIRE(!h->pend.active, CE_ERR_INVALID, "a cache op begun with ce_cache_prepare_ids_begin has not been finished");
+  h->admission = mode;
+  return CE_OK;
+}
+
+extern "C" int ce_cache_admission_stats(ce_cache_t* h, int64_t* counts4) {
+  CE_REQUIRE(h && counts4, CE_ERR_INVALID, "null argument");
+  for (int i = 0; i < 4; ++i) counts4[i] = 0;
+  counts4[0] = h->admission;
+  if (h->wb) {
+    std::lock_guard<std::mutex> g(h->wb->m);
+    counts4[0] = h->wb->chained ? CE_ADMIT_KERNEL : CE_ADMIT_COPY;
+    counts4[1] = h->wb->in_copy_jobs;
+    counts4[2] = h->wb->in_probed;
+    counts4[3] = h->wb->in_probed_rows;
+  }
   return CE_OK;
 }
 
@@ -705,6 +759,7 @@
   PhaseProf* const prof = (h->prof && (const void*)h->prof == a.prof_id) ? h->prof : nullptr;
   int pmark = *pmark_io;
   int rc = CE_OK;
+  if (worker && !h->wb->chained) CE_HIP_CHECK(hipStreamWaitEvent(s, h->ev, 0));
 #define CE_PHASE() do { if (prof) (void)hipEventRecord(prof->ev[pslot][pmark++], s); } while (0)
   const int cgrid = grid_for(C, 256 * 4);
   const int top_pass = select_top_pass(h, n, capturing);
@@ -725,8 +780,8 @@
     const int sgrid = (int)std::min<int64_t>(512, std::max<int64_t>(1, cdiv(L.stage_rows, gpb)));
     WbMail* const mail = worker ? h->wb->mail_dev + wbuf : nullptr;
     const dim3 sg(sgrid + (steady ? n_vblocks : 0));
-    const EvTable evt = (worker && h->wb->chained) ? EvTable{h->evt_keys[wbuf], h->evt_pos[wbuf], h->evt_mask}
-                                                     : EvTable{nullptr, nullptr, 0u};
+    const EvTable evt = worker ? EvTable{h->evt_keys[wbuf], h->evt_pos[wbuf], h->evt_mask}
+                               : EvTable{nullptr, nullptr, 0u};
     if (h->vec) {
       hipLaunchKernelGGL((k_evict_stage<f32x4>), sg, dim3(256), 0, s, h->victims, c.cached_idx_map,
                          c.inverted_cached_idx, (const f32x4*)c.cache_weight, (f32x4*)stage_cur, stage_idx_cur, scap, h->rowlen, h->g_log2,
@@ -793,7 +848,9 @@
 
 static void launch_front_kernels(ce_cache* h, const int64_t* ids, int64_t n, int64_t* slots_out, hipStream_t s,
                                  int allow_pad, bool steady, long long seq_arg, int32_t* miss_list, WbMail* mail_in,
-                                 long long in_job, int32_t* miss_host, long long* n_admit_out, bool single_pass_ok) {
+                                 long long in_job, int32_t* miss_host, long long* n_admit_out, bool single_pass_ok,
+                                 const unsigned long long* evt_keys = nullptr, const int32_t* evt_pos = nullptr,
+                                 uint32_t evt_tag = 0) {
   const ce_cache_config_t& c = h->cfg;
   const Layout& L = h->L;
   const int64_t N = c.num_embeddings, C = c.cuda_row_num;
@@ -841,7 +898,8 @@
                      c.inverted_cached_idx, N, h->blk_unique, h->blk_miss, h->coarse);
   hipLaunchKernelGGL(k_emit, dim3((unsigned)cdiv(L.n_chunks, kEmitSub)), dim3(256), 0, s, (uint4*)h->bitmap, c.inverted_cached_idx, N,
                      h->blk_miss, h->coarse, (int)L.n_chunks, miss_list, h->slot_epoch, seq_arg, h->ctl, C, n, h->ring_dev,
-                     mail_in, in_job, (long long)L.stage_rows, miss_host, steady ? 1 : 0, n_admit_out);
+                     mail_in, in_job, (long long)L.stage_rows, miss_host, steady ? 1 : 0, n_admit_out, evt_keys, evt_pos,
+                     h->evt_mask, evt_tag);
 }
 
 static int prepare_ids_second_half(ce_cache* h);
@@ -1063,6 +1121,11 @@
   if (worker) {
     rc = ensure_writeback(h);
     if (rc) return rc;
+    const bool want_chained = admission_for_call(h, n);
+    if (want_chained != h->wb->chained || (!want_chained && !h->wb->in_thread.joinable())) {
+      rc = switch_admission(h, want_chained);
+      if (rc) return rc;
+    }
     if (h->wb->chained) {
       rc = h->wb->check();
       if (rc) return rc;
@@ -1113,14 +1176,23 @@
   const int pslot = (int)(h->seq % kProfDepth);
   int pmark = 0;
   if (prof) prof->collect(pslot);
+  bool probe_prev = false;
+  if (worker) {
+    std::lock_guard<std::mutex> g(h->wb->m);
+    probe_prev = out_job - 1 >= h->wb->probe_floor && h->wb->out_done < out_job - 1;
+    if (probe_prev) h->wb->in_probed += 1;
+  }
+  const int pb = (int)((out_job - 1) & 1);
 #define CE_PHASE() do { if (prof) (void)hipEventRecord(prof->ev[pslot][pmark++], s); } while (0)
   CE_PHASE();
   launch_front_kernels(h, ids, n, slots_out, s, allow_pad, steady, seq_arg, h->miss_list,
                        worker ? h->wb->mail_dev + 2 : (WbMail*)nullptr, in_job,
-                       worker ? h->wb->miss_host_dev : (int32_t*)nullptr, (long long*)nullptr, !capturing);
+                       worker ? h->wb->miss_host_dev : (int32_t*)nullptr, (long long*)nullptr, !capturing,
+                       probe_prev ? h->evt_keys[pb] : nullptr, probe_prev ? h->evt_pos[pb] : nullptr,
+                       (uint32_t)(out_job - 1));
   if (worker) {
     CE_HIP_CHECK(hipEventRecord(h->wb->in_ev[in_job & 1], s));
-    h->wb->push_in(out_job - 1);
+    h->wb->push_in(out_job - 2);
   }
   CE_PHASE();
   SelArgs sel{s, n, worker, capturing, steady, out_job, seq_arg, wbuf, n_vblocks, pslot, (const void*)prof, h->free_list};
@@ -1136,6 +1208,8 @@
   x.pmark = pmark;
   x.prof = prof;
   x.chained = false;
+  x.probe_prev = probe_prev;
+  x.prev_job = out_job - 1;
   x.sel_pending = defer_sel;
   x.sel_s = s; x.sel_n = n; x.sel_steady = steady; x.sel_out_job = out_job; x.sel_wbuf = wbuf; x.sel_n_vblocks = n_vblocks;
   if (tail)
@@ -1215,18 +1289,24 @@
     const long long scap = (long long)L.stage_rows;
     CE_HIP_CHECK(hipStreamWaitValue64(s, h->wb->sig, (uint64_t)in_job, hipStreamWaitValueGte, ~0ull));
     const int ugrid = (int)std::min<int64_t>(1024, std::max<int64_t>(1, cdiv(L.stage_rows, gpb)));
+    const int pb = (int)(x.prev_job & 1);
+    const unsigned long long* ek = x.probe_prev ? h->evt_keys[pb] : nullptr;
     if (h->vec) {
       hipLaunchKernelGGL((k_unpack_admitted<f32x4>), dim3(ugrid), dim3(256), 0, s, h->free_list,
                          (const long long*)&h->ctl->n_miss, scap, (const f32x4*)h->in_stage, (f32x4*)c.cache_weight,
                          h->rowlen, h->g_log2, h->ctl, (const unsigned long long*)(h->wb->sig_dev + 1),
                          in_job, (const int32_t*)h->miss_list,
-                         L.list_cap > L.stage_rows ? (const f32x4*)c.host_weight_dev : (const f32x4*)nullptr);
+                         L.list_cap > L.stage_rows ? (const f32x4*)c.host_weight_dev : (const f32x4*)nullptr,
+                         ek, (const int32_t*)h->evt_pos[pb], h->evt_mask, (uint32_t)x.prev_job,
+                         (const f32x4*)(pb ? h->stage2 : h->stage));
     } else {
       hipLaunchKernelGGL((k_unpack_admitted<float>), dim3(ugrid), dim3(256), 0, s, h->free_list,
                          (const long long*)&h->ctl->n_miss, scap, (const float*)h->in_stage, (float*)c.cache_weight,
                          h->rowlen, h->g_log2, h->ctl, (const unsigned long long*)(h->wb->sig_dev + 1),
                          in_job, (const int32_t*)h->miss_list,
-                         L.list_cap > L.stage_rows ? (const float*)c.host_weight_dev : (const float*)nullptr);
+                         L.list_cap > L.stage_rows ? (const float*)c.host_weight_dev : (const float*)nullptr,
+                         ek, (const int32_t*)h->evt_pos[pb], h->evt_mask, (uint32_t)x.prev_job,
+                         (const float*)(pb ? h->stage2 : h->stage));
     }
   } else if (c.transport == CE_TRANSPORT_ZEROCOPY) {
     const long long scap = (long long)L.stage_rows;
diff --git a/cachedembedding_amd/csrc/ce_cache_index.h b/cachedembedding_amd/csrc/ce_cache_index.h
--- a/cachedembedding_amd/csrc/ce_cache_index.h
+++ b/cachedembedding_amd/csrc/ce_cache_index.h
@@ -404,13 +404,19 @@
   }
 }
 
+__device__ __forceinline__ int32_t evt_find(const unsigned long long* __restrict__ keys, const int32_t* __restrict__ pos,
+                                            uint32_t mask, uint32_t tag, int32_t row);
+constexpr uint32_t kMissCarried = 0x80000000u;
 constexpr int kEmitSub = 1;
 __global__ __launch_bounds__(256) void k_emit(uint4* bitmap4, const int32_t* __restrict__ inverted, int64_t N,
                                               const int32_t* __restrict__ blk_miss, const int32_t* __restrict__ coarse,
                                               int n_chunks, int32_t* miss_list, int32_t* slot_epoch, long long seq_arg,
                                               Ctl* ctl, int64_t C, int64_t n_ids, ce_call_stats_t* ring,
                                               WbMail* mail_in, long long job, long long in_cap, int32_t* miss_host,
-                                              int assume_free0, long long* n_admit_out = nullptr) {
+                                              int assume_free0, long long* n_admit_out = nullptr,
+                                              const unsigned long long* __restrict__ evt_keys = nullptr,
+                                              const int32_t* __restrict__ evt_pos = nullptr, uint32_t evt_mask = 0,
+                                              uint32_t evt_tag = 0) {
   const long long seq_ = call_seq(ctl, seq_arg);
   const int32_t epoch = call_epoch(seq_);
   ce_call_stats_t* const ring_slot = ring + (seq_ % kRing);
@@ -528,7 +534,11 @@
         while (bits) {
           const int b = __ffs(bits) - 1;
           bits &= bits - 1;
-          if (miss_host && pos < in_cap) miss_host[pos] = (int32_t)(row0 + b);
+          if (miss_host && pos < in_cap) {
+            const int32_t row = (int32_t)(row0 + b);
+            const bool carried = evt_keys && evt_find(evt_keys, evt_pos, evt_mask, evt_tag, row) >= 0;
+            miss_host[pos] = carried ? (int32_t)((uint32_t)row | kMissCarried) : row;
+          }
           miss_list[pos++] = (int32_t)(row0 + b);
         }
       }
diff --git a/cachedembedding_amd/csrc/ce_cache_rows.h b/cachedembedding_amd/csrc/ce_cache_rows.h
--- a/cachedembedding_amd/csrc/ce_cache_rows.h
+++ b/cachedembedding_amd/csrc/ce_cache_rows.h
@@ -433,7 +433,10 @@
                                                          int rowlen, int g_log2, Ctl* ctl,
                                                          const unsigned long long* fail_word, long long job,
                                                          const int32_t* __restrict__ rows,
-                                                         const VT* __restrict__ host_overflow) {
+                                                         const VT* __restrict__ host_overflow,
+                                                         const unsigned long long* __restrict__ evt_keys,
+                                                         const int32_t* __restrict__ evt_pos, uint32_t evt_mask,
+                                                         uint32_t tag, const VT* __restrict__ prev_stage) {
   const bool ok = ctl->status == CE_OK;
   if (blockIdx.x == 0 && threadIdx.x == 0) {
     ctl->lost = *(volatile const unsigned long long*)fail_word == (unsigned long long)job;
@@ -444,8 +447,12 @@
   const int gl = threadIdx.x & (G - 1);
   const int64_t gstride = ((int64_t)gridDim.x * blockDim.x) >> g_log2;
   if (host_overflow && n > cap) {
-    for (int64_t i = cap + (((int64_t)blockIdx.x * blockDim.x + threadIdx.x) >> g_log2); i < n; i += gstride)
-      copy_row(host_overflow + (int64_t)rows[i] * rowlen, cache + (int64_t)slots[i] * rowlen, rowlen, gl, G);
+    for (int64_t i = cap + (((int64_t)blockIdx.x * blockDim.x + threadIdx.x) >> g_log2); i < n; i += gstride) {
+      const int32_t row = rows[i];
+      const int32_t p = evt_keys ? evt_find(evt_keys, evt_pos, evt_mask, tag, row) : -1;
+      copy_row(p >= 0 ? prev_stage + (int64_t)p * rowlen : host_overflow + (int64_t)row * rowlen,
+               cache + (int64_t)slots[i] * rowlen, rowlen, gl, G);
+    }
   }
   if (n > cap) n = cap;
   constexpr int R = kStageRowsInFlight;
@@ -456,14 +463,20 @@
 #pragma unroll
       for (int t = 0; t < R; ++t) {
         slot[t] = i + t < n ? slots[i + t] : -1;
-        if (slot[t] >= 0 && gl < rowlen) v[t] = in_stage[(i + t) * rowlen + gl];
+        if (slot[t] < 0) continue;
+        const int32_t p = evt_keys ? evt_find(evt_keys, evt_pos, evt_mask, tag, rows[i + t]) : -1;
+        const VT* src = p >= 0 ? prev_stage + (int64_t)p * rowlen : in_stage + (i + t) * rowlen;
+        if (gl < rowlen) v[t] = src[gl];
       }
 #pragma unroll
       for (int t = 0; t < R; ++t)
         if (slot[t] >= 0 && gl < rowlen) cache[(int64_t)slot[t] * rowlen + gl] = v[t];
     } else {
-      for (int t = 0; t < R && i + t < n; ++t)
-        copy_row(in_stage + (i + t) * rowlen, cache + (int64_t)slots[i + t] * rowlen, rowlen, gl, G);
+      for (int t = 0; t < R && i + t < n; ++t) {
+        const int32_t p = evt_keys ? evt_find(evt_keys, evt_pos, evt_mask, tag, rows[i + t]) : -1;
+        copy_row(p >= 0 ? prev_stage + (int64_t)p * rowlen : in_stage + (i + t) * rowlen,
+                 cache + (int64_t)slots[i + t] * rowlen, rowlen, gl, G);
+      }
     }
   }
 }
diff --git a/cachedembedding_amd/csrc/ce_cache_worker.h b/cachedembedding_amd/csrc/ce_cache_worker.h
--- a/cachedembedding_amd/csrc/ce_cache_worker.h
+++ b/cachedembedding_amd/csrc/ce_cache_worker.h
@@ -197,6 +197,7 @@
   float* in_stage_dev = nullptr;
   float* in_host = nullptr;
   bool chained = false;
+  int env_admit = -1;
   hipEvent_t ev_miss[2] = {nullptr, nullptr};
   static constexpr int kRowsRing = 4;
   hipEvent_t ev_rows[kRowsRing] = {nullptr};
@@ -207,6 +208,8 @@
   const int32_t* evt_pos[2] = {nullptr, nullptr};
   uint32_t evt_mask = 0;
   long long in_probed = 0;
+  long long in_probed_rows = 0;
+  long long in_copy_jobs = 0;
 #ifdef CE_TEST_HOOKS
   int out_delay_us = 0;
   long long fail_in_job = 0;
@@ -229,6 +232,7 @@
   RowPool* in_pool = nullptr;
   double out_wait_s = 0, out_busy_s = 0, in_wait_s = 0, in_busy_s = 0, in_gather_s = 0;
   double out_wait0_s = 0;
+  double in_out_wait_s = 0;
   double out_copy_wait_s = 0, out_scatter_s = 0;
   long long out_rows = 0, out_jobs = 0, in_rows = 0, in_jobs = 0;
 
@@ -340,9 +344,10 @@
       }
       const auto t0 = std::chrono::steady_clock::now();
       CE_TRACE("in job %lld: waiting for its miss-list event (needs out job %lld)", job, need_out);
-      hipError_t e = hipEventSynchronize(in_ev[job & 1]);
-      if (e != hipSuccess) fail("hipEventSynchronize(in)", e);
+      hipError_t e = event_wait_polite(in_ev[job & 1]);
+      if (e != hipSuccess) fail("waiting for the miss list", e);
       CE_TRACE("in job %lld: event done (%s)", job, hipGetErrorString(e));
+      const auto tw = std::chrono::steady_clock::now();
       {
         std::unique_lock<std::mutex> g(m);
         cv_done.wait(g, [&] { return out_done >= need_out || err != 0; });
@@ -351,6 +356,7 @@
       long long n = mail[2].count;
       CE_TRACE("in job %lld: earlier write-backs landed; mail job %lld count %lld", job, mail[2].job, n);
       if (mail[2].job != job || n < 0 || n > stage_rows) n = 0;
+      long long n_carried = 0;
 #ifdef CE_TEST_HOOKS
       if (fail_in_job > 0 && job == fail_in_job) fail("admission (injected: CE_WORKER_FAIL_IN_JOB)", hipErrorUnknown);
 #endif
@@ -364,7 +370,7 @@
         constexpr int kAhead = 8;
         constexpr int64_t kPiece = 2048, kCopyPieces = 4;
         const int64_t npieces = cdiv(n, kPiece);
-        std::atomic<int64_t> next{0};
+        std::atomic<int64_t> next{0}, carried{0};
         std::vector<std::atomic<unsigned char>> ready((size_t)npieces);
         for (auto& r : ready) r.store(0, std::memory_order_relaxed);
         const std::function<void(int64_t, int64_t)> work = [&](int64_t, int64_t) {
@@ -372,14 +378,17 @@
             const int64_t pc = next.fetch_add(1, std::memory_order_relaxed);
             if (pc >= npieces) break;
             const int64_t lo = pc * kPiece, hi = std::min<int64_t>(n, lo + kPiece);
+            int64_t skipped = 0;
             for (int64_t i = lo; i < hi; ++i) {
-              if (i + kAhead < hi) {
+              if (i + kAhead < hi && rows[i + kAhead] >= 0) {
                 const char* q = (const char*)(tb + (size_t)rows[i + kAhead] * d);
                 for (int64_t l = 0; l < d * 4; l += 64) __builtin_prefetch(q + l);
               }
+              if (rows[i] < 0) { ++skipped; continue; }
               row_copy_stream(st + (size_t)i * d, tb + (size_t)rows[i] * d, (size_t)d);
             }
             row_copy_fence();
+            if (skipped) carried.fetch_add(skipped, std::memory_order_relaxed);
             ready[(size_t)pc].store(1, std::memory_order_release);
           }
         };
@@ -404,6 +413,7 @@
           }
         }
         in_pool->wait();
+        n_carried = carried.load(std::memory_order_relaxed);
       }
       const auto tg = std::chrono::steady_clock::now();
       CE_TRACE("in job %lld: rows gathered, copies enqueued", job);
@@ -417,10 +427,13 @@
         std::lock_guard<std::mutex> g(m);
         in_done = job;
         in_wait_s += std::chrono::duration<double>(t1 - t0).count();
+        in_out_wait_s += std::chrono::duration<double>(t1 - tw).count();
         in_busy_s += std::chrono::duration<double>(t2 - t1).count();
         in_gather_s += std::chrono::duration<double>(tg - t1).count();
         in_rows += n;
         in_jobs += 1;
+        in_copy_jobs += 1;
+        in_probed_rows += n_carried;
       }
       cv_done.notify_all();
     }
@@ -494,9 +507,16 @@
       stop = true;
     }
     if (const char* e = getenv("CE_WORKER_PROFILE"))
-      if (atoi(e) != 0 && in_jobs > 0)
+      if (atoi(e) != 0 && in_jobs > 0) {
         fprintf(stderr, "[libce_hip] admission worker: %lld jobs, %lld of them with the previous write-back still on its "
                 "way (rows it evicted taken from its staging buffer)\n", in_jobs, in_probed);
+        if (in_copy_jobs > 0)
+          fprintf(stderr, "[libce_hip] host-gather admission: %lld jobs, per job %.3f ms waiting for the miss list (%.3f of "
+                  "it for a write-back), %.3f busy = %.3f gathering + %.3f for the last copies; %.0f rows left to the "
+                  "previous staging buffer per job\n", in_copy_jobs, in_wait_s / in_copy_jobs * 1e3,
+                  in_out_wait_s / in_copy_jobs * 1e3, in_busy_s / in_copy_jobs * 1e3, in_gather_s / in_copy_jobs * 1e3,
+                  (in_busy_s - in_gather_s) / in_copy_jobs * 1e3, (double)in_probed_rows / in_copy_jobs);
+      }
     if (const char* e = getenv("CE_WORKER_PROFILE"))
       if (atoi(e) != 0 && out_jobs > 0)
         fprintf(stderr, "[libce_hip] write-back worker: %lld jobs, %.3f ms busy per job = %.3f waiting for copies + %.3f "
diff --git a/include/ce_api.h b/include/ce_api.h
--- a/include/ce_api.h
+++ b/include/ce_api.h
@@ -259,6 +259,12 @@
 int ce_cache_phase_times(ce_cache_t* h, double* ms_out, int32_t cap, int64_t* calls, int32_t reset);
 int ce_cache_writeback_wait(ce_cache_t* h);
 int ce_cache_swap_stats(ce_cache_t* h, double* seconds6, int64_t* counts4);
+
+#define CE_ADMIT_KERNEL 0
+#define CE_ADMIT_COPY 1
+#define CE_ADMIT_AUTO 2
+int ce_cache_set_admission(ce_cache_t* h, int32_t mode);
+int ce_cache_admission_stats(ce_cache_t* h, int64_t* counts4);
 int ce_cache_set_buffer_rows(ce_cache_t* h, int64_t rows);
 int ce_cache_free_rows(ce_cache_t* h, int64_t* out);
 
```

After: 3.161 billion. 1.2% lower.
